# ltronchin/Gan-track

Hardware: AMD Instinct MI355X
Metric: imgs/sec at 256^2 bs32/GPU StyleGAN2-ADA training (+ sec/kimg) (higher is better)
Workload: dtype fp16+fp32 (fp16 at the 4 highest resolutions, fp32 below; f32 accumulate); 1 GPU; StyleGAN2-ADA train iteration, 256x256 1-ch, c_dim 2, cbase 16384, map 8, Gmain+Dmain / Greg every 4 / Dreg every 16, ADA geometric p=0.2; global_batch=32, batch_gpu=32, resolution=256, parallelism=dp1

## Files before the change

### gan-track_amd/csrc/upfirdn2d.hip

```cpp
#include <cstdlib>

#include "sg2_common.h"

namespace sg2 {
namespace {

constexpr int kMaxTaps = 1024;

struct UpfParams {
    const void* x;
    void* y;
    const float* f;
    int N, C, H, W;
    int OH, OW;
    int64_t xs_n, xs_c, xs_h, xs_w;
    int64_t ys_n, ys_c, ys_h, ys_w;
    int fw, fh;
    int upx, upy, downx, downy, padx0, pady0;
    int flip;
    float gain;
    const float* out_scale;
    const void* noise;
    const float* bias;
    const void* residual;
    void* aux;
    float noise_gain, alpha, egain, clamp;
    int act, aux_mode, epi;
    const int* lim;
    int xcd;
};

constexpr int kZeroBand = 32;

__device__ __forceinline__ int floordiv(int a, int b) { return (a >= 0) ? a / b : -((-a + b - 1) / b); }

__device__ __forceinline__ void axis_taps(int o, int down, int pad0, int up, int& t0, int& i0) {
    const int z = o * down - pad0;
    int r = (-z) % up;
    if (r < 0) r += up;
    t0 = r;
    i0 = floordiv(z + r, up);
}

__device__ __forceinline__ void stage_filter(float* sf, const UpfParams& p) {
    const int n = p.fw * p.fh;
    for (int i = threadIdx.x; i < n; i += blockDim.x) {
        const int ty = i / p.fw, tx = i % p.fw;
        const int sy = p.flip ? ty : p.fh - 1 - ty;
        const int sx = p.flip ? tx : p.fw - 1 - tx;
        sf[i] = p.f[sy * p.fw + sx] * p.gain;
    }
    __syncthreads();
}

template <typename T>
__global__ __launch_bounds__(256) void upfirdn_generic(UpfParams p) {
    __shared__ float sf[kMaxTaps];
    stage_filter(sf, p);
    const T* x = (const T*)p.x;
    T* y = (T*)p.y;
    const int64_t total = (int64_t)p.N * p.C * p.OH * p.OW;
    for (int64_t idx = (int64_t)blockIdx.x * blockDim.x + threadIdx.x; idx < total;
         idx += (int64_t)gridDim.x * blockDim.x) {
        int64_t r = idx;
        const int ox = (int)(r % p.OW); r /= p.OW;
        const int oy = (int)(r % p.OH); r /= p.OH;
        const int c = (int)(r % p.C); r /= p.C;
        const int n = (int)r;
        if (p.lim) {
            const int ly = p.lim[0], lx = p.lim[1];
            if (oy >= ly + kZeroBand || ox >= lx + kZeroBand) continue;
            if (oy >= ly || ox >= lx) {
                y[n * p.ys_n + c * p.ys_c + (int64_t)oy * p.ys_h + (int64_t)ox * p.ys_w] = (T)0.f;
                continue;
            }
        }
        int ty0, iy0, tx0, ix0;
        axis_taps(oy, p.downy, p.pady0, p.upy, ty0, iy0);
        axis_taps(ox, p.downx, p.padx0, p.upx, tx0, ix0);
        const T* xb = x + n * p.xs_n + c * p.xs_c;
        float acc = 0.f;
        for (int ty = ty0, iy = iy0; ty < p.fh; ty += p.upy, ++iy) {
            if (iy < 0 || iy >= p.H) continue;
            const T* xr = xb + iy * p.xs_h;
            for (int tx = tx0, ix = ix0; tx < p.fw; tx += p.upx, ++ix) {
                if (ix < 0 || ix >= p.W) continue;
                acc += (float)xr[ix * p.xs_w] * sf[ty * p.fw + tx];
            }
        }
        y[n * p.ys_n + c * p.ys_c + (int64_t)oy * p.ys_h + (int64_t)ox * p.ys_w] = (T)acc;
    }
}

template <int UP, int DOWN>
__device__ __forceinline__ void axis_taps_c(int o, int down, int pad0, int up, int& t0, int& i0) {
    if (UP == 1 && DOWN != 0) { t0 = 0; i0 = o * DOWN - pad0; }
    else if (UP == 2 && DOWN != 0) { const int z = o * DOWN - pad0; t0 = z & 1; i0 = (z + t0) >> 1; }
    else axis_taps(o, down, pad0, up, t0, i0);
}

template <typename T, bool HORIZ, int KT, int UP, int DOWN>
__global__ __launch_bounds__(256) void upfirdn_1d(UpfParams p) {
    __shared__ float sf[64];
    const int F = HORIZ ? p.fw : p.fh;
    for (int t = threadIdx.x; t < F; t += 256) sf[t] = p.f[p.flip ? t : F - 1 - t] * p.gain;
    __syncthreads();
    const int ly = p.lim ? p.lim[0] : p.OH, lx = p.lim ? p.lim[1] : p.OW;
    const int rows = min(p.OH, ly + (p.lim ? kZeroBand : 0)), cols = min(p.OW, lx + (p.lim ? kZeroBand : 0));
    const int tiles = (cols + 255) / 256;
    const int total = p.N * p.C * rows * tiles;
    const int up = HORIZ ? p.upx : p.upy, down = HORIZ ? p.downx : p.downy, L = HORIZ ? p.W : p.H;
    for (int b = blockIdx.x; b < total; b += gridDim.x) {
        const int row = b / tiles;
        const int ox = (b - row * tiles) * 256 + threadIdx.x;
        const int oy = row % rows, nc = row / rows;
        if (ox >= cols) continue;
        const int c = nc % p.C, n = nc / p.C;
        T* yp = (T*)p.y + n * p.ys_n + c * p.ys_c + (int64_t)oy * p.ys_h + (int64_t)ox * p.ys_w;
        if (oy >= ly || ox >= lx) { *yp = (T)0.f; continue; }
        const T* xb = (const T*)p.x + n * p.xs_n + c * p.xs_c;
        int t0, i0;
        if (HORIZ) axis_taps_c<UP, DOWN>(ox, down, p.padx0, up, t0, i0);
        else axis_taps_c<UP, DOWN>(oy, down, p.pady0, up, t0, i0);
        const T* xl = HORIZ ? xb + (int64_t)oy * p.xs_h : xb + (int64_t)ox * p.xs_w;
        const int64_t st = HORIZ ? p.xs_w : p.xs_h;
        const int upk = UP ? UP : up;
        float acc = 0.f;
#pragma unroll
        for (int k = 0; k < KT; ++k) {
            const int t = t0 + k * upk, i = i0 + k;
            const bool ok = t < F && i >= 0 && i < L;
            const float v = (float)xl[(int64_t)(ok ? i : 0) * st];
            acc += ok ? v * sf[t < F ? t : 0] : 0.f;
        }
        *yp = (T)acc;
    }
}

template <typename T, int UP, int DOWN, int KT, int TWD = 256>
__global__ __launch_bounds__(256) void upfirdn_1d_hlds(UpfParams p) {
    constexpr int ROWS = 256 / TWD;
    constexpr int SPAN = ((TWD - 1) * DOWN + UP - 1) / UP + KT + 1;
    __shared__ float sf[64];
    __shared__ float sx[ROWS][SPAN];
    const int F = p.fw;
    for (int t = threadIdx.x; t < KT * UP; t += 256) sf[t] = t < F ? p.f[p.flip ? t : F - 1 - t] * p.gain : 0.f;
    __syncthreads();
    float fr[KT * UP];
#pragma unroll
    for (int t = 0; t < KT * UP; ++t) fr[t] = t < F ? sf[t] : 0.f;
    const int ly = p.lim ? p.lim[0] : p.OH, lx = p.lim ? p.lim[1] : p.OW;
    const int rows = min(p.OH, ly + (p.lim ? kZeroBand : 0)), cols = min(p.OW, lx + (p.lim ? kZeroBand : 0));
    const int tiles = (cols + TWD - 1) / TWD, rgroups = (rows + ROWS - 1) / ROWS;
    const int total = p.N * p.C * rgroups * tiles;
    const int rr = threadIdx.x / TWD, col = threadIdx.x % TWD;
    for (int b = blockIdx.x; b < total; b += gridDim.x) {
        const int rg = b / tiles;
        const int ox0 = (b - rg * tiles) * TWD, ox = ox0 + col;
        const int oy0 = (rg % rgroups) * ROWS, nc = rg / rgroups;
        const int c = nc % p.C, n = nc / p.C;
        int tb, base;
        axis_taps_c<UP, DOWN>(ox0, DOWN, p.padx0, UP, tb, base);
        const T* xp = (const T*)p.x + n * p.xs_n + c * p.xs_c;
        __syncthreads();
        for (int e = threadIdx.x; e < ROWS * SPAN; e += 256) {
            const int r = e / SPAN, m = e - r * SPAN;
            const int i = base + m, y = oy0 + r;
            sx[r][m] = (i >= 0 && i < p.W && y < rows) ? (float)xp[(int64_t)y * p.xs_h + (int64_t)i * p.xs_w] : 0.f;
        }
        __syncthreads();
        const int oy = oy0 + rr;
        if (ox >= cols || oy >= rows) continue;
        T* yp = (T*)p.y + n * p.ys_n + c * p.ys_c + (int64_t)oy * p.ys_h + (int64_t)ox * p.ys_w;
        if (oy >= ly || ox >= lx) { *yp = (T)0.f; continue; }
        int t0, i0;
        axis_taps_c<UP, DOWN>(ox, DOWN, p.padx0, UP, t0, i0);
        const float* w = &sx[rr][i0 - base];
        float acc = 0.f;
#pragma unroll
        for (int k = 0; k < KT; ++k)
            acc += w[k] * (UP == 1 ? fr[k] : sf[t0 + k * UP]);
        *yp = (T)acc;
    }
}

template <int UP, int DOWN, int P>
struct VRunPat {
    static constexpr int dj(int j) { return UP == 1 ? j * DOWN : (P == 0 ? (j + 1) / 2 : j / 2); }
    static constexpr int tj(int j) { return UP == 1 ? 0 : (P == 0 ? (j & 1) : 1 - (j & 1)); }
};

template <int UP, int DOWN, int KT, int R, int SPAN, int P>
__device__ __forceinline__ void vrun_acc(const float (&win)[SPAN], const float (&fr)[KT * UP], float (&acc)[R]) {
#pragma unroll
    for (int j = 0; j < R; ++j) {
#pragma unroll
        for (int k = 0; k < KT; ++k) acc[j] += win[VRunPat<UP, DOWN, P>::dj(j) + k] * fr[VRunPat<UP, DOWN, P>::tj(j) + k * UP];
    }
}

template <typename T, int UP, int DOWN, int KT, int R>
__global__ __launch_bounds__(256) void upfirdn_1d_vrun(UpfParams p) {
    static_assert(UP == 1 || R % 2 == 0, "even runs keep the phase fixed");
    constexpr int SPAN = ((R - 1) * DOWN + UP - 1) / UP + KT;
    __shared__ float sf[64];
    const int F = p.fh;
    for (int t = threadIdx.x; t < F; t += 256) sf[t] = p.f[p.flip ? t : F - 1 - t] * p.gain;
    __syncthreads();
    float fr[KT * UP];
#pragma unroll
    for (int t = 0; t < KT * UP; ++t) fr[t] = t < F ? sf[t] : 0.f;
    const int ly = p.lim ? p.lim[0] : p.OH, lx = p.lim ? p.lim[1] : p.OW;
    const int rows = min(p.OH, ly + (p.lim ? kZeroBand : 0)), cols = min(p.OW, lx + (p.lim ? kZeroBand : 0));
    const int tiles = (cols + 255) / 256, runs = (rows + R - 1) / R;
    const int total = p.N * p.C * runs * tiles;
    for (int b = blockIdx.x; b < total; b += gridDim.x) {
        const int run = b / tiles;
        const int ox = (b - run * tiles) * 256 + threadIdx.x;
        const int oy0 = (run % runs) * R, nc = run / runs;
        if (ox >= cols) continue;
        const int c = nc % p.C, n = nc / p.C;
        const T* xb = (const T*)p.x + n * p.xs_n + c * p.xs_c + (int64_t)ox * p.xs_w;
        T* yb = (T*)p.y + n * p.ys_n + c * p.ys_c + (int64_t)ox * p.ys_w;
        const int z0 = oy0 * DOWN - p.pady0;
        const int ph = UP == 2 ? (z0 & 1) : 0;
        const int base = UP == 2 ? (z0 + ph) >> 1 : z0;
        float win[SPAN];
#pragma unroll
        for (int m = 0; m < SPAN; ++m) {
            const int i = base + m;
            const bool ok = i >= 0 && i < p.H;
            const float v = (float)xb[(int64_t)(ok ? i : 0) * p.xs_h];
            win[m] = ok ? v : 0.f;
        }
        float acc[R];
#pragma unroll
        for (int j = 0; j < R; ++j) acc[j] = 0.f;
        if (ph) vrun_acc<UP, DOWN, KT, R, SPAN, 1>(win, fr, acc);
        else vrun_acc<UP, DOWN, KT, R, SPAN, 0>(win, fr, acc);
#pragma unroll
        for (int j = 0; j < R; ++j) {
            const int oy = oy0 + j;
            if (oy >= rows) break;
            yb[(int64_t)oy * p.ys_h] = (oy >= ly || ox >= lx) ? (T)0.f : (T)acc[j];
        }
    }
}

template <typename T> struct VecN { static constexpr int N = 8; };
template <> struct VecN<float> { static constexpr int N = 4; };

template <typename T, int V, typename vecT>
__device__ __forceinline__ void store_out(const UpfParams& p, T* y, const float* acc, int n, int oy, int ox, int cv) {
    const int64_t dst = n * p.ys_n + (int64_t)oy * p.ys_h + (int64_t)ox * p.ys_w + cv * V;
    vecT o;
    if (p.epi) {
        const float nv = p.noise ? (float)((const T*)p.noise)[((int64_t)n * p.OH + oy) * p.OW + ox] * p.noise_gain : 0.f;
        vecT ax, rv;
        if (p.residual) rv = *(const vecT*)((const T*)p.residual + dst);
#pragma unroll
        for (int j = 0; j < V; ++j) {
            const int c = cv * V + j;
            float v = acc[j];
            if (p.out_scale) v *= p.out_scale[(int64_t)n * p.C + c];
            v += nv;
            if (p.bias) v += (float)(T)p.bias[c];
            if (p.act == 1) v = v > 0.f ? v : v * p.alpha;
            v *= p.egain;
            if (p.clamp >= 0.f) v = fminf(fmaxf(v, -p.clamp), p.clamp);
            ax[j] = (T)(p.aux_mode == 1 ? acc[j] : v);
            o[j] = (T)v;
            if (p.residual) o[j] = (T)((float)o[j] + (float)rv[j]);
        }
        if (p.aux_mode) *(vecT*)((T*)p.aux + dst) = ax;
    } else {
#pragma unroll
        for (int j = 0; j < V; ++j) o[j] = (T)acc[j];
    }
    *(vecT*)(y + dst) = o;
}


template <typename T, typename IDX>
__global__ __launch_bounds__(256) void upfirdn_nhwc_vec(UpfParams p) {
    constexpr int V = VecN<T>::N;
    typedef T vecT __attribute__((ext_vector_type(V)));
    __shared__ float sf[kMaxTaps];
    stage_filter(sf, p);
    const T* x = (const T*)p.x;
    T* y = (T*)p.y;
    const IDX CV = (IDX)(p.C / V), OW = (IDX)p.OW, OH = (IDX)p.OH;
    const IDX total = (IDX)((int64_t)p.N * p.OH * p.OW * (p.C / V));
    for (IDX idx = (IDX)blockIdx.x * blockDim.x + threadIdx.x; idx < total; idx += (IDX)gridDim.x * blockDim.x) {
        IDX r = idx;
        const int cv = (int)(r % CV); r /= CV;
        const int ox = (int)(r % OW); r /= OW;
        const int oy = (int)(r % OH); r /= OH;
        const int n = (int)r;
        int ty0, iy0, tx0, ix0;
        axis_taps(oy, p.downy, p.pady0, p.upy, ty0, iy0);
        axis_taps(ox, p.downx, p.padx0, p.upx, tx0, ix0);
        const T* xb = x + n * p.xs_n + cv * V;
        float acc[V];
#pragma unroll
        for (int j = 0; j < V; ++j) acc[j] = 0.f;
        for (int ty = ty0, iy = iy0; ty < p.fh; ty += p.upy, ++iy) {
            if (iy < 0 || iy >= p.H) continue;
            const T* xr = xb + iy * p.xs_h;
            for (int tx = tx0, ix = ix0; tx < p.fw; tx += p.upx, ++ix) {
                if (ix < 0 || ix >= p.W) continue;
                const float wt = sf[ty * p.fw + tx];
                const vecT v = *(const vecT*)(xr + ix * p.xs_w);
#pragma unroll
                for (int j = 0; j < V; ++j) acc[j] += (float)v[j] * wt;
            }
        }
        store_out<T, V, vecT>(p, y, acc, n, oy, ox, cv);
    }
}

__device__ __forceinline__ float fma_mix_lo(unsigned h2, float w, float acc) {
    float r;
    asm volatile("v_fma_mix_f32 %0, %1, %2, %3 op_sel_hi:[1,0,0]" : "=v"(r) : "v"(h2), "v"(w), "v"(acc));
    return r;
}
__device__ __forceinline__ float fma_mix_hi(unsigned h2, float w, float acc) {
    float r;
    asm volatile("v_fma_mix_f32 %0, %1, %2, %3 op_sel:[1,0,0] op_sel_hi:[1,0,0]" : "=v"(r) : "v"(h2), "v"(w), "v"(acc));
    return r;
}

template <typename T>
__global__ __launch_bounds__(256) void upfirdn_nhwc_up2(UpfParams p) {
    constexpr int V = VecN<T>::N;
    typedef T vecT __attribute__((ext_vector_type(V)));
    __shared__ float sf[16];
    if (threadIdx.x < 16) {
        const int ty = threadIdx.x >> 2, tx = threadIdx.x & 3;
        sf[threadIdx.x] = p.f[(p.flip ? ty : 3 - ty) * 4 + (p.flip ? tx : 3 - tx)] * p.gain;
    }
    __syncthreads();
    const unsigned CV = p.C / V, CW = (p.OW + 1) >> 1, CH = (p.OH + 1) >> 1;
    const unsigned total = (unsigned)p.N * CH * CW * CV;
    const unsigned idx = blockIdx.x * 256u + threadIdx.x;
    if (idx >= total) return;
    unsigned r = idx;
    const int cv = (int)(r % CV); r /= CV;
    const int cx = (int)(r % CW); r /= CW;
    const int cy = (int)(r % CH);
    const int n = (int)(r / CH);
    int ty[2], iy[2], tx[2], ix[2];
    axis_taps(2 * cy, 1, p.pady0, 2, ty[0], iy[0]);
    axis_taps(2 * cy + 1, 1, p.pady0, 2, ty[1], iy[1]);
    axis_taps(2 * cx, 1, p.padx0, 2, tx[0], ix[0]);
    axis_taps(2 * cx + 1, 1, p.padx0, 2, tx[1], ix[1]);
    const int y0 = min(iy[0], iy[1]), x0 = min(ix[0], ix[1]);
    const T* xb = (const T*)p.x + n * p.xs_n + cv * V;
    vecT xv[3][3];
#pragma unroll
    for (int a = 0; a < 3; ++a)
#pragma unroll
        for (int b = 0; b < 3; ++b) {
            const int yy = y0 + a, xx = x0 + b;
            const bool ok = yy >= 0 && yy < p.H && xx >= 0 && xx < p.W;
            xv[a][b] = ok ? *(const vecT*)(xb + yy * p.xs_h + xx * p.xs_w) : vecT{};
        }
#pragma unroll
    for (int py = 0; py < 2; ++py) {
        const int oy = 2 * cy + py;
        if (oy >= p.OH) continue;
        const int dy = iy[py] - y0;
#pragma unroll
        for (int px = 0; px < 2; ++px) {
            const int ox = 2 * cx + px;
            if (ox >= p.OW) continue;
            const int dx = ix[px] - x0;
            float acc[V];
#pragma unroll
            for (int j = 0; j < V; ++j) acc[j] = 0.f;
#pragma unroll
            for (int a = 0; a < 2; ++a) {
                const int t1 = ty[py] + 2 * a;
                if (t1 >= 4) continue;
#pragma unroll
                for (int b = 0; b < 2; ++b) {
                    const int t2 = tx[px] + 2 * b;
                    if (t2 >= 4) continue;
                    const float w = sf[t1 * 4 + t2];
                    const vecT v = dy ? (dx ? xv[1 + a][1 + b] : xv[1 + a][b]) : (dx ? xv[a][1 + b] : xv[a][b]);
                    if constexpr (std::is_same<T, f16_t>::value) {
                        typedef unsigned u32v __attribute__((ext_vector_type(V / 2)));
                        const u32v u = __builtin_bit_cast(u32v, v);
#pragma unroll
                        for (int q = 0; q < V / 2; ++q) {
                            acc[2 * q] = fma_mix_lo(u[q], w, acc[2 * q]);
                            acc[2 * q + 1] = fma_mix_hi(u[q], w, acc[2 * q + 1]);
                        }
                    } else {
#pragma unroll
                        for (int j = 0; j < V; ++j) acc[j] += (float)v[j] * w;
                    }
                }
            }
            store_out<T, V, vecT>(p, (T*)p.y, acc, n, oy, ox, cv);
        }
    }
}

template <typename T, int DOWN, int TW, int TH, int CG>
__global__ __launch_bounds__(256) void upfirdn_nhwc_f4(UpfParams p) {
    constexpr int V = VecN<T>::N;
    constexpr int F = 4;
    constexpr int IW = (TW - 1) * DOWN + F, IH = (TH - 1) * DOWN + F, NIN = IW * IH * CG;
    typedef T vecT __attribute__((ext_vector_type(V)));
    __shared__ float sf[F * F];
    extern __shared__ __attribute__((aligned(16))) char tile_raw[];
    vecT* tile = (vecT*)tile_raw;
    const int tid = threadIdx.x;
    if (tid < F * F) {
        const int ty = tid / F, tx = tid % F;
        sf[tid] = p.f[(p.flip ? ty : F - 1 - ty) * F + (p.flip ? tx : F - 1 - tx)] * p.gain;
    }
    const int CV = p.C / V;
    const int ngroups = (CV + CG - 1) / CG;
    const int tiles_x = (p.OW + TW - 1) / TW, tiles_y = (p.OH + TH - 1) / TH;
    int64_t b = blockIdx.x;
    const int64_t nb = gridDim.x;
    if ((nb & 7) == 0 && p.xcd) b = (b & 7) * (nb >> 3) + (b >> 3);
    const int cg = (int)(b % ngroups); b /= ngroups;
    const int tx0 = (int)(b % tiles_x) * TW; b /= tiles_x;
    const int ty0 = (int)(b % tiles_y) * TH; b /= tiles_y;
    const int n = (int)b;
    const int cv0 = cg * CG;
    const T* xb = (const T*)p.x + n * p.xs_n;
    const int iy0 = ty0 * DOWN - p.pady0, ix0 = tx0 * DOWN - p.padx0;
    for (int i = tid; i < NIN; i += 256) {
        const int c = i % CG, px = i / CG;
        const int ry = px / IW, rx = px - ry * IW;
        const int iy = iy0 + ry, ix = ix0 + rx;
        const bool ok = iy >= 0 && iy < p.H && ix >= 0 && ix < p.W && cv0 + c < CV;
        vecT v = *(const vecT*)(xb + (int64_t)(ok ? iy : 0) * p.xs_h + (int64_t)(ok ? ix : 0) * p.xs_w +
                                (ok ? cv0 + c : 0) * V);
#pragma unroll
        for (int j = 0; j < V; ++j) v[j] = ok ? v[j] : (T)0.f;
        tile[i] = v;
    }
    __syncthreads();
    const int c = tid % CG;
    if (cv0 + c >= CV) return;
#pragma unroll
    for (int pass = 0; pass < TW * TH * CG / 256; ++pass) {
        const int pix = tid / CG + pass * (256 / CG);
        const int oy = ty0 + pix / TW, ox = tx0 + pix % TW;
        if (oy >= p.OH || ox >= p.OW) continue;
        float acc[V];
#pragma unroll
        for (int j = 0; j < V; ++j) acc[j] = 0.f;
        const vecT* base = tile + ((pix / TW) * DOWN * IW + (pix % TW) * DOWN) * CG + c;
#pragma unroll
        for (int ky = 0; ky < F; ++ky)
#pragma unroll
            for (int kx = 0; kx < F; ++kx) {
                const float w = sf[ky * F + kx];
                const vecT v = base[(ky * IW + kx) * CG];
                if constexpr (std::is_same<T, f16_t>::value) {
                    typedef unsigned u32v __attribute__((ext_vector_type(V / 2)));
                    const u32v u = __builtin_bit_cast(u32v, v);
#pragma unroll
                    for (int q = 0; q < V / 2; ++q) {
                        acc[2 * q] = fma_mix_lo(u[q], w, acc[2 * q]);
                        acc[2 * q + 1] = fma_mix_hi(u[q], w, acc[2 * q + 1]);
                    }
                } else {
#pragma unroll
                    for (int j = 0; j < V; ++j) acc[j] += (float)v[j] * w;
                }
            }
        store_out<T, V, vecT>(p, (T*)p.y, acc, n, oy, ox, cv0 + c);
    }
}

template <typename T, int V, typename vecT, int TW, int TH, int CG, bool SEP, bool EPI>
__device__ __forceinline__ void fir4_strip(const UpfParams& p, const vecT* base, const float* wf, const float* fy,
                                           const float* fx, int n, int ty0, int ox, int cv) {
    constexpr int F = 4, IW = TW + F - 1, IH = TH + F - 1;
    float os[V], bj[V];
#pragma unroll
    for (int j = 0; j < V; ++j) {
        const int c = cv * V + j;
        os[j] = (p.epi && p.out_scale) ? p.out_scale[(int64_t)n * p.C + c] : 1.f;
        bj[j] = (p.epi && p.bias) ? (float)(T)p.bias[c] : 0.f;
    }
    const float slope = (p.epi && p.act == 1) ? p.alpha : 1.f;
    const float eg = p.epi ? p.egain : 1.f;
    const bool clamp_on = p.epi && p.clamp >= 0.f;
    const float cl = p.clamp;
    const bool noise = p.epi && p.noise, resid = p.epi && p.residual;
    const int aux_mode = p.epi ? p.aux_mode : 0;
    float acc[TH][V];
#pragma unroll
    for (int o = 0; o < TH; ++o)
#pragma unroll
        for (int j = 0; j < V; ++j) acc[o][j] = 0.f;
#pragma unroll
    for (int ry = 0; ry < IH; ++ry) {
        vecT v[F];
#pragma unroll
        for (int kx = 0; kx < F; ++kx) v[kx] = base[(ry * IW + kx) * CG];
        if constexpr (SEP) {
            float h[V];
            if constexpr (std::is_same<T, f16_t>::value) {
                typedef unsigned u32v __attribute__((ext_vector_type(V / 2)));
#pragma unroll
                for (int j = 0; j < V; ++j) h[j] = 0.f;
#pragma unroll
                for (int kx = 0; kx < F; ++kx) {
                    const u32v u = __builtin_bit_cast(u32v, v[kx]);
#pragma unroll
                    for (int q = 0; q < V / 2; ++q) {
                        h[2 * q] = fma_mix_lo(u[q], fx[kx], h[2 * q]);
                        h[2 * q + 1] = fma_mix_hi(u[q], fx[kx], h[2 * q + 1]);
                    }
                }
            } else {
#pragma unroll
                for (int j = 0; j < V; ++j) {
                    h[j] = 0.f;
#pragma unroll
                    for (int kx = 0; kx < F; ++kx) h[j] += (float)v[kx][j] * fx[kx];
                }
            }
#pragma unroll
            for (int ky = 0; ky < F; ++ky) {
                const int o = ry - ky;
                if (o < 0 || o >= TH) continue;
#pragma unroll
                for (int j = 0; j < V; ++j) acc[o][j] += h[j] * fy[ky];
            }
        } else {
#pragma unroll
            for (int ky = 0; ky < F; ++ky) {
                const int o = ry - ky;
                if (o < 0 || o >= TH) continue;
#pragma unroll
                for (int kx = 0; kx < F; ++kx)
#pragma unroll
                    for (int j = 0; j < V; ++j) acc[o][j] += (float)v[kx][j] * wf[ky * F + kx];
            }
        }
        const int od = ry - (F - 1);
        if (od < 0) continue;
        const int oy = ty0 + od;
        const int64_t dst = n * p.ys_n + (int64_t)oy * p.ys_h + (int64_t)ox * p.ys_w + cv * V;
        if constexpr (!EPI) {
            vecT o;
#pragma unroll
            for (int j = 0; j < V; ++j) o[j] = (T)acc[od][j];
            *(vecT*)((T*)p.y + dst) = o;
            __builtin_amdgcn_sched_barrier(0);
            continue;
        }
        const float nv = noise ? (float)((const T*)p.noise)[((int64_t)n * p.OH + oy) * p.OW + ox] * p.noise_gain : 0.f;
        vecT o, ax;
#pragma unroll
        for (int j = 0; j < V; ++j) {
            float z = acc[od][j] * os[j] + nv + bj[j];
            z = (z > 0.f ? z : z * slope) * eg;
            if (clamp_on) z = fminf(fmaxf(z, -cl), cl);
            o[j] = (T)z;
            ax[j] = (T)(aux_mode == 1 ? acc[od][j] : z);
        }
        if (resid) {
            const vecT rv = *(const vecT*)((const T*)p.residual + dst);
#pragma unroll
            for (int j = 0; j < V; ++j) o[j] = (T)((float)o[j] + (float)rv[j]);
        }
        if (aux_mode) *(vecT*)((T*)p.aux + dst) = ax;
        *(vecT*)((T*)p.y + dst) = o;
        __builtin_amdgcn_sched_barrier(0);
    }
}

template <typename T, int TW, int TH, int CG = 8>
__global__ __launch_bounds__(256, 2) void upfirdn_nhwc_f4s(UpfParams p) {
    constexpr int V = VecN<T>::N, F = 4;
    constexpr int IW = TW + F - 1, IH = TH + F - 1, NIN = IW * IH * CG;
    constexpr int NL = (NIN + 255) / 256;
    static_assert(TW * CG == 256, "one lane per (column, channel vector)");
    typedef T vecT __attribute__((ext_vector_type(V)));
    extern __shared__ __attribute__((aligned(16))) char tile_raw[];
    vecT* tile = (vecT*)tile_raw;
    const int tid = threadIdx.x;
    float wf[F * F];
#pragma unroll
    for (int t = 0; t < F * F; ++t) {
        const int ty = t / F, tx = t % F;
        wf[t] = p.f[(p.flip ? ty : F - 1 - ty) * F + (p.flip ? tx : F - 1 - tx)] * p.gain;
    }
    const int CV = p.C / V;
    const int ngroups = (CV + CG - 1) / CG;
    const int tiles_x = (p.OW + TW - 1) / TW, tiles_y = (p.OH + TH - 1) / TH;
    int64_t b = blockIdx.x;
    const int64_t nb = gridDim.x;
    if ((nb & 7) == 0) b = (b & 7) * (nb >> 3) + (b >> 3);
    const int tx0 = min((int)(b % tiles_x) * TW, p.OW - TW); b /= tiles_x;
    const int ty0 = min((int)(b % tiles_y) * TH, p.OH - TH); b /= tiles_y;
    const int cg = (int)(b % ngroups); b /= ngroups;
    const int n = (int)b;
    const int cv0 = cg * CG;
    const T* xb = (const T*)p.x + n * p.xs_n;
    const int iy0 = ty0 - p.pady0, ix0 = tx0 - p.padx0;
    vecT r[NL];
#pragma unroll
    for (int l = 0; l < NL; ++l) {
        const int i = tid + l * 256;
        const int c = i % CG, px = i / CG;
        const int ry = px / IW, rx = px - ry * IW;
        const int iy = iy0 + ry, ix = ix0 + rx;
        const bool ok = i < NIN && iy >= 0 && iy < p.H && ix >= 0 && ix < p.W && cv0 + c < CV;
        r[l] = *(const vecT*)(xb + (int64_t)(ok ? iy : 0) * p.xs_h + (int64_t)(ok ? ix : 0) * p.xs_w +
                              (ok ? cv0 + c : 0) * V);
#pragma unroll
        for (int j = 0; j < V; ++j) r[l][j] = ok ? r[l][j] : (T)0.f;
    }
#pragma unroll
    for (int l = 0; l < NL; ++l)
        if (l < NL - 1 || tid + l * 256 < NIN) tile[tid + l * 256] = r[l];
    __syncthreads();
    const int c = tid % CG, col = tid / CG;
    if (cv0 + c >= CV) return;
    float fy[F], fx[F];
    bool sep = wf[0] != 0.f;
#pragma unroll
    for (int k = 0; k < F; ++k) {
        fx[k] = wf[k];
        fy[k] = sep ? wf[k * F] / wf[0] : 0.f;
    }
#pragma unroll
    for (int t = 0; t < F * F; ++t) sep = sep && (fy[t / F] * fx[t % F] == wf[t]);
    const vecT* tb = tile + col * CG + c;
    if (sep) {
        if (p.epi) fir4_strip<T, V, vecT, TW, TH, CG, true, true>(p, tb, wf, fy, fx, n, ty0, tx0 + col, cv0 + c);
        else fir4_strip<T, V, vecT, TW, TH, CG, true, false>(p, tb, wf, fy, fx, n, ty0, tx0 + col, cv0 + c);
    } else {
        if (p.epi) fir4_strip<T, V, vecT, TW, TH, CG, false, true>(p, tb, wf, fy, fx, n, ty0, tx0 + col, cv0 + c);
        else fir4_strip<T, V, vecT, TW, TH, CG, false, false>(p, tb, wf, fy, fx, n, ty0, tx0 + col, cv0 + c);
    }
}

template <typename T>
int launch(const UpfParams& p, bool vec, hipStream_t s) {
    static const bool fir_old = getenv("SG2_FIR_OLD") != nullptr;
    if (!fir_old && vec && p.upx == 1 && p.upy == 1 && p.downx == 1 && p.downy == 1 && p.fw == 4 && p.fh == 4 &&
        p.OH >= 8 && (p.OW % 32 == 0 || p.OW >= 224) && !(p.residual && p.residual == p.y)) {
        constexpr int TW = 32, TH = 8;
        const char* e32 = getenv("SG2_FIR_C32");
        const bool c32_off = e32 && e32[0] == '0';
        if (!c32_off && p.C / VecN<T>::N == 4 && (p.OW % 64 == 0 || p.OW >= 224)) {
            constexpr int TW4 = 64, CG4 = 4;
            const int64_t blocks4 = (int64_t)p.N * cdiv(p.OH, TH) * cdiv(p.OW, TW4);
            if (blocks4 < INT32_MAX) {
                const size_t lds = (size_t)(TH + 3) * (TW4 + 3) * CG4 * 16;
                auto k = upfirdn_nhwc_f4s<T, TW4, TH, CG4>;
                static bool set4 = false;
                if (!set4) { (void)hipFuncSetAttribute((const void*)k, hipFuncAttributeMaxDynamicSharedMemorySize, (int)lds); set4 = true; }
                k<<<(unsigned)blocks4, 256, lds, s>>>(p);
                return launch_status("sg2_upfirdn2d");
            }
        }
        const int64_t blocks = (int64_t)p.N * cdiv(p.OH, TH) * cdiv(p.OW, TW) * cdiv(p.C / VecN<T>::N, 8);
        if (blocks < INT32_MAX) {
            const size_t lds = (size_t)(TH + 3) * (TW + 3) * 8 * 16;
            auto k = upfirdn_nhwc_f4s<T, TW, TH>;
            static bool set = false;
            if (!set) { (void)hipFuncSetAttribute((const void*)k, hipFuncAttributeMaxDynamicSharedMemorySize, (int)lds); set = true; }
            k<<<(unsigned)blocks, 256, lds, s>>>(p);
            return launch_status("sg2_upfirdn2d");
        }
    }
    if (vec && p.upx == 1 && p.upy == 1 && p.downx == p.downy && (p.downy == 1 || p.downy == 2) && p.fw == 4 &&
        p.fh == 4) {
        constexpr int CG = 4;
        const int d = p.downy;
        const int TW = d == 1 ? 32 : 16, TH = 8;
        const int64_t blocks = (int64_t)p.N * cdiv(p.OH, TH) * cdiv(p.OW, TW) * cdiv(p.C / VecN<T>::N, CG);
        if (blocks < INT32_MAX) {
            const size_t lds = (size_t)((TH - 1) * d + 4) * ((TW - 1) * d + 4) * CG * 16;
            if (d == 1) {
                auto k = upfirdn_nhwc_f4<T, 1, 32, 8, CG>;
                static bool set1 = false;
                if (!set1) { (void)hipFuncSetAttribute((const void*)k, hipFuncAttributeMaxDynamicSharedMemorySize, (int)lds); set1 = true; }
                k<<<(unsigned)blocks, 256, lds, s>>>(p);
            } else {
                auto k = upfirdn_nhwc_f4<T, 2, 16, 8, CG>;
                static bool set2 = false;
                if (!set2) { (void)hipFuncSetAttribute((const void*)k, hipFuncAttributeMaxDynamicSharedMemorySize, (int)lds); set2 = true; }
                k<<<(unsigned)blocks, 256, lds, s>>>(p);
            }
            return launch_status("sg2_upfirdn2d");
        }
    }
    if (vec && p.upx == 2 && p.upy == 2 && p.downx == 1 && p.downy == 1 && p.fw == 4 && p.fh == 4 &&
        !getenv("SG2_UPF_UP2_OFF")) {
        const int64_t cells = (int64_t)p.N * ((p.OH + 1) / 2) * ((p.OW + 1) / 2) * (p.C / VecN<T>::N);
        if (cells < INT32_MAX - 256) {
            upfirdn_nhwc_up2<T><<<(unsigned)cdiv(cells, 256), 256, 0, s>>>(p);
            return launch_status("sg2_upfirdn2d");
        }
    }
    if (!vec && !p.epi) {
        const bool horiz = p.fh == 1 && p.upy == 1 && p.downy == 1 && p.pady0 == 0 && p.OH == p.H && p.fw <= 64;
        const bool vert = p.fw == 1 && p.upx == 1 && p.downx == 1 && p.padx0 == 0 && p.OW == p.W && p.fh <= 64;
        const int up = horiz ? p.upx : p.upy, down = horiz ? p.downx : p.downy, F = horiz ? p.fw : p.fh;
        const int kt = (F + up - 1) / up;
        const int64_t pairs = (int64_t)p.N * p.C * p.OH * cdiv(p.OW, 256);
        if ((horiz || vert) && kt <= 16 && pairs < INT32_MAX) {
            static const int gmax = [] { const char* e = getenv("SG2_U1D_GRID"); return e ? atoi(e) : 4096; }();
            const unsigned g = (unsigned)std::min<int64_t>(pairs, gmax);
            const bool ada_up = up == 2 && down == 1 && kt == 6, ada_down = up == 1 && down == 2 && kt == 12;
            static const int vr = [] { const char* e = getenv("SG2_U1D_VRUN"); return e ? atoi(e) : 4; }();
            static const bool hl = [] { const char* e = getenv("SG2_U1D_HLDS"); return e ? atoi(e) != 0 : true; }();
            static const int htw = [] { const char* e = getenv("SG2_U1D_HTW"); return e ? atoi(e) : 128; }();
            if (vert && vr == 4 && ada_up) upfirdn_1d_vrun<T, 2, 1, 6, 4><<<g, 256, 0, s>>>(p);
            else if (vert && vr == 4 && ada_down) upfirdn_1d_vrun<T, 1, 2, 12, 4><<<g, 256, 0, s>>>(p);
            else if (vert && vr == 8 && ada_up) upfirdn_1d_vrun<T, 2, 1, 6, 8><<<g, 256, 0, s>>>(p);
            else if (vert && vr == 8 && ada_down) upfirdn_1d_vrun<T, 1, 2, 12, 8><<<g, 256, 0, s>>>(p);
            else if (horiz && hl && ada_up && htw == 128) upfirdn_1d_hlds<T, 2, 1, 6, 128><<<g, 256, 0, s>>>(p);
            else if (horiz && hl && ada_down && htw == 128) upfirdn_1d_hlds<T, 1, 2, 12, 128><<<g, 256, 0, s>>>(p);
            else if (horiz && hl && ada_up) upfirdn_1d_hlds<T, 2, 1, 6><<<g, 256, 0, s>>>(p);
            else if (horiz && hl && ada_down) upfirdn_1d_hlds<T, 1, 2, 12><<<g, 256, 0, s>>>(p);
            else if (horiz && ada_up) upfirdn_1d<T, true, 6, 2, 1><<<g, 256, 0, s>>>(p);
            else if (horiz && ada_down) upfirdn_1d<T, true, 12, 1, 2><<<g, 256, 0, s>>>(p);
            else if (ada_up) upfirdn_1d<T, false, 6, 2, 1><<<g, 256, 0, s>>>(p);
            else if (ada_down) upfirdn_1d<T, false, 12, 1, 2><<<g, 256, 0, s>>>(p);
            else {
#define U1D(KT_) { if (horiz) upfirdn_1d<T, true, KT_, 0, 0><<<g, 256, 0, s>>>(p); \
                   else upfirdn_1d<T, false, KT_, 0, 0><<<g, 256, 0, s>>>(p); }
                if (kt <= 4) U1D(4) else if (kt <= 8) U1D(8) else U1D(16)
#undef U1D
            }
            return launch_status("sg2_upfirdn2d");
        }
    }
    const int64_t work = vec ? (int64_t)p.N * p.OH * p.OW * (p.C / VecN<T>::N) : (int64_t)p.N * p.C * p.OH * p.OW;
    const int grid = (int)std::max<int64_t>(1, std::min<int64_t>(cdiv(work, 256), 256 * 32));
    if (vec && work < INT32_MAX && (int64_t)grid * 256 < INT32_MAX)
        upfirdn_nhwc_vec<T, unsigned><<<grid, 256, 0, s>>>(p);
    else if (vec)
        upfirdn_nhwc_vec<T, int64_t><<<grid, 256, 0, s>>>(p);
    else
        upfirdn_generic<T><<<grid, 256, 0, s>>>(p);
    return launch_status("sg2_upfirdn2d");
}

}
}

extern "C" int sg2_upfirdn2d_fused(void* y, const void* x, const float* f, int dtype, const int64_t* in_size,
                                   const int64_t* in_stride, const int64_t* out_size, const int64_t* out_stride,
                                   int fw, int fh, int upx, int upy, int downx, int downy, int padx0, int padx1,
                                   int pady0, int pady1, int flip, float gain, const sg2_epilogue* epi,
                                   void* stream) {
    using namespace sg2;
    SG2_CHECK(x && y && f && in_size && in_stride && out_size && out_stride, "sg2_upfirdn2d: null argument");
    SG2_CHECK(upx >= 1 && upy >= 1 && downx >= 1 && downy >= 1, "sg2_upfirdn2d: up/down must be >= 1");
    SG2_CHECK(fw >= 1 && fh >= 1 && fw * fh <= kMaxTaps, "sg2_upfirdn2d: filter too large");
    UpfParams p;
    p.x = x; p.y = y; p.f = f;
    p.N = (int)in_size[0]; p.C = (int)in_size[1]; p.H = (int)in_size[2]; p.W = (int)in_size[3];
    p.OH = (int)out_size[2]; p.OW = (int)out_size[3];
    SG2_CHECK(out_size[0] == p.N && out_size[1] == p.C, "sg2_upfirdn2d: batch/channel mismatch");
    const int64_t eh = ((int64_t)p.H * upy + pady0 + pady1 - fh + downy) / downy;
    const int64_t ew = ((int64_t)p.W * upx + padx0 + padx1 - fw + downx) / downx;
    SG2_CHECK(p.H * upy + pady0 + pady1 >= fh && p.W * upx + padx0 + padx1 >= fw,
              "sg2_upfirdn2d: upsampled buffer must be at least the size of the filter");
    SG2_CHECK(eh == p.OH && ew == p.OW, "sg2_upfirdn2d: output size mismatch");
    p.xs_n = in_stride[0]; p.xs_c = in_stride[1]; p.xs_h = in_stride[2]; p.xs_w = in_stride[3];
    p.ys_n = out_stride[0]; p.ys_c = out_stride[1]; p.ys_h = out_stride[2]; p.ys_w = out_stride[3];
    p.fw = fw; p.fh = fh; p.upx = upx; p.upy = upy; p.downx = downx; p.downy = downy;
    p.padx0 = padx0; p.pady0 = pady0; p.flip = flip; p.gain = gain; p.lim = nullptr;
    { const char* e = getenv("SG2_FIR_XCD"); p.xcd = e ? atoi(e) : 1; }
    p.out_scale = nullptr; p.noise = nullptr; p.bias = nullptr; p.residual = nullptr; p.aux = nullptr;
    p.noise_gain = 0.f; p.alpha = 0.f; p.egain = 1.f; p.clamp = -1.f; p.act = 0; p.aux_mode = 0; p.epi = 0;
    if (epi) {
        SG2_CHECK(epi->act == 0 || epi->act == 1, "sg2_upfirdn2d: epilogue act must be 0 or 1");
        SG2_CHECK(epi->aux_mode >= 0 && epi->aux_mode <= 2 && (epi->aux_mode == 0 || epi->aux),
                  "sg2_upfirdn2d: bad epilogue aux output");
        p.out_scale = epi->out_scale; p.noise = epi->noise; p.bias = epi->bias; p.residual = epi->residual;
        p.aux = epi->aux; p.noise_gain = epi->noise_gain; p.alpha = epi->alpha; p.egain = epi->gain;
        p.clamp = epi->clamp; p.act = epi->act; p.aux_mode = epi->aux_mode; p.epi = 1;
    }
    if ((int64_t)p.N * p.C * p.OH * p.OW == 0) return 0;
    hipStream_t s = as_stream(stream);
    SG2_DISPATCH(dtype, T, {
        constexpr int V = VecN<T>::N;
        const bool vec = p.xs_c == 1 && p.ys_c == 1 && p.C % V == 0 && p.C >= V &&
                         ((uintptr_t)x % 16 == 0) && ((uintptr_t)y % 16 == 0) &&
                         p.xs_w % V == 0 && p.xs_h % V == 0 && p.xs_n % V == 0 &&
                         p.ys_w % V == 0 && p.ys_h % V == 0 && p.ys_n % V == 0;
        SG2_CHECK(vec || !p.epi, "sg2_upfirdn2d: the fused epilogue needs NHWC activations with C % 8 == 0");
        return launch<T>(p, vec, s);
    });
    return 0;
}

extern "C" int sg2_upfirdn2d_lim(void* y, const void* x, const float* f, int dtype, const int64_t* in_size,
                                 const int64_t* in_stride, const int64_t* out_size, const int64_t* out_stride, int fw,
                                 int fh, int upx, int upy, int downx, int downy, int padx0, int padx1, int pady0,
                                 int pady1, int flip, float gain, const int* lim, void* stream) {
    using namespace sg2;
    SG2_CHECK(x && y && f && in_size && in_stride && out_size && out_stride, "sg2_upfirdn2d: null argument");
    SG2_CHECK(upx >= 1 && upy >= 1 && downx >= 1 && downy >= 1, "sg2_upfirdn2d: up/down must be >= 1");
    SG2_CHECK(fw >= 1 && fh >= 1 && fw * fh <= kMaxTaps, "sg2_upfirdn2d: filter too large");
    UpfParams p{};
    p.x = x; p.y = y; p.f = f; p.lim = lim;
    p.N = (int)in_size[0]; p.C = (int)in_size[1]; p.H = (int)in_size[2]; p.W = (int)in_size[3];
    p.OH = (int)out_size[2]; p.OW = (int)out_size[3];
    SG2_CHECK(out_size[0] == p.N && out_size[1] == p.C, "sg2_upfirdn2d: batch/channel mismatch");
    const int64_t eh = ((int64_t)p.H * upy + pady0 + pady1 - fh + downy) / downy;
    const int64_t ew = ((int64_t)p.W * upx + padx0 + padx1 - fw + downx) / downx;
    SG2_CHECK(eh == p.OH && ew == p.OW, "sg2_upfirdn2d: output size mismatch");
    p.xs_n = in_stride[0]; p.xs_c = in_stride[1]; p.xs_h = in_stride[2]; p.xs_w = in_stride[3];
    p.ys_n = out_stride[0]; p.ys_c = out_stride[1]; p.ys_h = out_stride[2]; p.ys_w = out_stride[3];
    p.fw = fw; p.fh = fh; p.upx = upx; p.upy = upy; p.downx = downx; p.downy = downy;
    p.padx0 = padx0; p.pady0 = pady0; p.flip = flip; p.gain = gain; p.egain = 1.f; p.clamp = -1.f;
    if ((int64_t)p.N * p.C * p.OH * p.OW == 0) return 0;
    hipStream_t s = as_stream(stream);
    SG2_DISPATCH(dtype, T, { return launch<T>(p, false, s); });
    return 0;
}

extern "C" int sg2_upfirdn2d(void* y, const void* x, const float* f, int dtype, const int64_t* in_size,
                             const int64_t* in_stride, const int64_t* out_size, const int64_t* out_stride, int fw,
                             int fh, int upx, int upy, int downx, int downy, int padx0, int padx1, int pady0,
                             int pady1, int flip, float gain, void* stream) {
    return sg2_upfirdn2d_fused(y, x, f, dtype, in_size, in_stride, out_size, out_stride, fw, fh, upx, upy, downx,
                               downy, padx0, padx1, pady0, pady1, flip, gain, nullptr, stream);
}
```

### gan-track_amd/sg2hip/__init__.py

```python
import contextlib
import ctypes
import os

import torch

_HERE = os.path.dirname(os.path.abspath(__file__))
LIB_PATH = os.environ.get('SG2HIP_LIB', os.path.join(_HERE, 'libsg2hip.so'))

F32, F16, BF16, F32S3 = 0, 1, 2, 3
_DTYPES = {torch.float32: F32, torch.float16: F16, torch.bfloat16: BF16}

_c_i64p = ctypes.POINTER(ctypes.c_int64)


class Epilogue(ctypes.Structure):
    _fields_ = [('out_scale', ctypes.c_void_p), ('noise', ctypes.c_void_p), ('bias', ctypes.c_void_p),
                ('residual', ctypes.c_void_p), ('aux', ctypes.c_void_p), ('noise_gain', ctypes.c_float),
                ('alpha', ctypes.c_float), ('gain', ctypes.c_float), ('clamp', ctypes.c_float),
                ('act', ctypes.c_int), ('aux_mode', ctypes.c_int), ('dot_src', ctypes.c_void_p),
                ('dot_out', ctypes.c_void_p)]

class AugGeomArgs(ctypes.Structure):
    _fields_ = [('draw', ctypes.c_void_p * 16), ('p', ctypes.c_void_p)] + \
        [(k, ctypes.c_float) for k in ('xflip', 'rotate90', 'xint', 'xint_max', 'scale', 'rotate', 'aniso', 'xfrac',
                                       'scale_std', 'rotate_max', 'aniso_std', 'xfrac_std', 'pad_x', 'pad_y',
                                       'inv_sx', 'inv_sy')] + \
        [(k, ctypes.c_int) for k in ('n', 'h', 'w')]


_vp = ctypes.c_void_p
_i = ctypes.c_int
_i64 = ctypes.c_int64
_f = ctypes.c_float

SIGNATURES = {
    'sg2_abi_version': [],
    'sg2_bias_act': [_vp, _vp, _vp, _vp, _vp, _vp, _i, _i64, _i64, _i64, _i, _i, _f, _f, _f, _vp],
    'sg2_upfirdn2d': [_vp, _vp, _vp, _i, _c_i64p, _c_i64p, _c_i64p, _c_i64p, _i, _i, _i, _i, _i, _i, _i, _i, _i, _i,
                      _i, _f, _vp],
    'sg2_conv2d': [_vp, _vp, _vp, _i, _i, _i, _i, _i, _i, _i, _i, _i, _i, _i, _i, _i, _i, _vp, _i64, _vp],
    'sg2_conv2d_fused': [_vp, _vp, _vp, _i, _i, _i, _i, _i, _i, _i, _i, _i, _i, _i, _i, _i, _i, _vp,
                         ctypes.POINTER(Epilogue), _vp, _i64, _vp],
    'sg2_conv3x3': [_vp, _vp, _vp, _vp, _i, _i, _i, _i, _i, _i, _vp, _vp, _vp, _f, _vp, _i, _f, _f, _f, _vp, _vp,
                    _vp],
    'sg2_set_zeroed_accumulators': [_i],
    'sg2_set_clean_workspace': [_i],
    'sg2_set_deterministic': [_vp, _i64],
    'sg2_split3': [_vp, _vp, _i64, _i, _i64, _vp, _vp],
    'sg2_conv3x3_s2': [_vp, _vp, _vp, _vp, _i, _i, _i, _i, _i, _i, _vp, _vp, _vp, _f, _vp, _i, _f, _f, _f, _vp, _i,
                       _vp, _vp, _vp],
    'sg2_conv3x3_up2': [_vp, _vp, _vp, _i, _i, _i, _i, _i, _i, _vp, _vp],
    'sg2_conv2d_wgrad': [_vp, _vp, _vp, _i, _i, _i, _i, _i, _i, _i, _i, _i, _i, _i, _i, _i, _vp, _vp, _f, _vp],
    'sg2_conv2d_wgrad_oikk': [_vp, _vp, _vp, _i, _i, _i, _i, _i, _i, _i, _i, _i, _i, _i, _i, _i, _f, _i, _vp],
    'sg2_upfirdn2d_lim': [_vp, _vp, _vp, _i, _c_i64p, _c_i64p, _c_i64p, _c_i64p, _i, _i, _i, _i, _i, _i, _i, _i, _i, _i,
                          _i, _f, _vp, _vp],
    'sg2_upfirdn2d_fused': [_vp, _vp, _vp, _i, _c_i64p, _c_i64p, _c_i64p, _c_i64p, _i, _i, _i, _i, _i, _i, _i, _i, _i,
                            _i, _i, _f, ctypes.POINTER(Epilogue), _vp],
    'sg2_layer_bwd': [_vp, _vp, _vp, _vp, _vp, _vp, _vp, _vp, _i, _i, _i, _i, _i, _f, _f, _f, _vp],
    'sg2_dot_hw': [_vp, _vp, _vp, _i, _i, _i, _i, _vp],
    'sg2_vjp_axpy': [_vp, _vp, _vp, _vp, _vp, _vp, _i, _f, _f, _f, _vp, _vp, _i, _i, _i, _i, _vp],
    'sg2_grid_sample_fwd': [_vp, _vp, _vp, _i, _c_i64p, _c_i64p, _c_i64p, _c_i64p, _vp, _vp],
    'sg2_grid_sample_bwd': [_vp, _vp, _vp, _i, _c_i64p, _c_i64p, _c_i64p, _c_i64p, _vp, _vp],
    'sg2_affine_grid_sample_fwd': [_vp, _vp, _vp, _i, _c_i64p, _c_i64p, _c_i64p, _c_i64p, _vp, _vp],
    'sg2_affine_grid_sample_bwd': [_vp, _vp, _vp, _i, _c_i64p, _c_i64p, _c_i64p, _c_i64p, _vp, _vp],
    'sg2_reflect_pad_dyn': [_vp, _vp, _vp, _i, _i, _i, _i, _i, _i, _i, _vp],
    'sg2_aug_geom': [_vp, _vp, _vp, _vp, ctypes.POINTER(AugGeomArgs), _vp],
    'sg2_moments': [_vp, _vp, _i64, _i, _vp],
    'sg2_demod_fwd': [_vp, _vp, _vp, _vp, _i, _i, _i, _i, _f, _vp],
    'sg2_demod_bwd': [_vp, _vp, _vp, _vp, _vp, _vp, _vp, _i, _i, _i, _i, _vp],
    'sg2_demod_vjp_bwd': [_vp] * 10 + [_i, _i, _i, _i, _vp],
    'sg2_adam_multi': [_vp, _vp, _vp, _i, _vp, _vp, _vp, _f, _f, _f, _f, _i, _vp],
    'sg2_lerp_multi': [_vp, _vp, _i, _f, _vp],
    'sg2_infnorm_fwd': [_vp, _vp, _vp, _i, _i, _f, _i, _vp],
    'sg2_infnorm_bwd': [_vp, _vp, _vp, _vp, _i, _i, _f, _i, _vp],
    'sg2_infnorm_vjp_bwd': [_vp, _vp, _vp, _vp, _vp, _vp, _i, _i, _f, _vp],
    'sg2_pack_weight': [_vp, _i, _vp, _i, _i, _i, _i, _i64, _i64, _i64, _i, _f, _vp],
    'sg2_pack_weight_multi': [_vp, _i, _vp],
    'sg2_knn_scratch_bytes': [_c_i64p, _i64, _i64, _i],
    'sg2_knn_radii': [_vp, _vp, _i, _i64, _i, _i, _i, _vp, _i64, _vp],
    'sg2_manifold_member': [_vp, _vp, _i64, _vp, _i64, _vp, _i, _i, _i, _vp, _i64, _vp],
    'sg2_noise_reg_scratch_bytes': [_c_i64p, _c_i64p, _i],
    'sg2_noise_reg_fwd': [_vp, _vp, _vp, _c_i64p, _i, _vp, _vp],
    'sg2_noise_reg_bwd': [_vp, _vp, _vp, _vp, _c_i64p, _i, _vp, _i, _vp],
    'sg2_noise_normalize_multi': [_vp, _c_i64p, _i, _vp],
}
ABI_VERSION = 11

_lib = None


def lib():
    global _lib
    if _lib is None:
        if not os.path.exists(LIB_PATH):
            raise RuntimeError(f'sg2hip: {LIB_PATH} not found -- build it with `python -c "import __graft_entry__ as '
                               f'g; g.build()"` (hipcc --offload-arch=gfx950); there is no CPU fallback')
        L = ctypes.CDLL(LIB_PATH)
        for name, args in SIGNATURES.items():
            fn = getattr(L, name)
            fn.argtypes = args
            fn.restype = ctypes.c_int
        L.sg2_last_error.argtypes = []
        L.sg2_last_error.restype = ctypes.c_char_p
        L.sg2_set_zeroed_accumulators.restype = None
        L.sg2_set_clean_workspace.restype = None
        L.sg2_set_deterministic.restype = None
        if L.sg2_abi_version() != ABI_VERSION:
            raise RuntimeError(f'sg2hip: ABI version mismatch ({L.sg2_abi_version()} != {ABI_VERSION})')
        _lib = L
    return _lib


@contextlib.contextmanager
def clean_workspace(on=True):
    if not on:
        yield
        return
    L = lib()
    L.sg2_set_clean_workspace(1)
    try:
        yield
    finally:
        L.sg2_set_clean_workspace(0)


_det_scratch = {}
_det_retired = []
_det_state = (0, 0)


def det_active():
    return _det_state[0] != 0


def _det_register(ptr, nbytes):
    global _det_state
    lib().sg2_set_deterministic(ctypes.c_void_p(ptr), ctypes.c_int64(nbytes))
    _det_state = (ptr, nbytes)


@contextlib.contextmanager
def deterministic(on=True, scratch_mb=2048, device=None):
    prev = _det_state
    if on:
        dev = torch.device('cuda', torch.cuda.current_device()) if device is None else torch.device(device)
        buf = _det_scratch.get(dev)
        if buf is None or buf.numel() * 4 < scratch_mb << 20:
            if buf is not None:
                _det_retired.append(buf)
            buf = _det_scratch[dev] = torch.empty([scratch_mb << 18], dtype=torch.float32, device=dev)
        _det_register(buf.data_ptr(), buf.numel() * 4)
    else:
        _det_register(0, 0)
    try:
        yield
    finally:
        _det_register(*prev)


@contextlib.contextmanager
def zeroed_accumulators(on=True):
    if not on:
        yield
        return
    L = lib()
    L.sg2_set_zeroed_accumulators(1)
    try:
        yield
    finally:
        L.sg2_set_zeroed_accumulators(0)


def check(rc, what):
    if rc != 0:
        msg = lib().sg2_last_error().decode(errors='replace')
        raise RuntimeError(f'{what} failed ({rc}): {msg}')


def dtype_code(t):
    try:
        return _DTYPES[t.dtype]
    except KeyError:
        raise RuntimeError(f'sg2hip: unsupported dtype {t.dtype}') from None


def require_device(*tensors):
    for t in tensors:
        if t is not None and (not isinstance(t, torch.Tensor) or t.device.type != 'cuda'):
            raise RuntimeError('sg2hip ops run only on ROCm device tensors (no CPU fallback); got '
                               f'{type(t).__name__} on {getattr(t, "device", None)}')


def stream_ptr(device=None):
    return ctypes.c_void_p(torch.cuda.current_stream(device).cuda_stream)


def ptr(t):
    return ctypes.c_void_p(t.data_ptr()) if t is not None else ctypes.c_void_p(0)


def i64arr(vals):
    return (ctypes.c_int64 * len(vals))(*[int(v) for v in vals])
```

### gan-track_amd/torch_utils/ops/modconv.py

```python
import os

import torch

from . import bias_act as _ba
from . import conv2d_gradfix as _cg
from . import staged_sum as _ss
from . import upfirdn2d as _up

_CL = torch.channels_last
enabled = True
prezero = os.environ.get('SG2_PREZERO', '1') != '0'
det_assign = os.environ.get('SG2_DET_ASSIGN', '1') != '0'
fast_backward = True
fused_vjp = os.environ.get('SG2_FUSED_VJP', '1') != '0'
tap_enabled = os.environ.get('SG2_TORGB_TAP', '1') != '0'
_ACT = {0: 'linear', 1: 'lrelu'}


def supported(x, weight, up):
    n, cin, h, w = x.shape
    cout, _, kh, kw = weight.shape
    return (enabled and up == 1 and kh == 3 and kw == 3 and x.dtype in (torch.float16, torch.bfloat16) and x.is_cuda and
            cin % 8 == 0 and cout % 8 == 0 and h >= 16 and w >= 16)


def supported_generic(x, weight):
    return enabled and x.is_cuda


def _halo(x, kh, kw, stride, pad):
    n, cin, h, w = x.shape
    return (kh == 3 and kw == 3 and stride == 1 and pad == 1 and x.dtype in (torch.float16, torch.bfloat16) and
            cin % 8 == 0 and h >= 16 and w >= 16)


def _f32(t):
    return t.float().contiguous() if t is not None else None


def _sum_hw(t):
    return _ss.staged_sum(t, (2, 3), dtype=torch.float32)


def _sum_nhw(t):
    return _ss.staged_sum(t, (0, 2, 3), dtype=torch.float32)


def _mul(a, s):
    return a * s if s is not None else a


class FusedConv(torch.autograd.Function):
    @staticmethod
    def forward(ctx, x, styles, weight, dcoefs, noise, bias, residual, stride, pad, act, alpha, gain, clamp, wgain):
        x_in = x
        x = _cg._nhwc(x)
        n, cin, h, w = x.shape
        cout, _, kh, kw = weight.shape
        oh = (h + 2 * pad - kh) // stride + 1
        ow = (w + 2 * pad - kw) // stride + 1
        dt = x.dtype
        nz = noise.to(dt).reshape(n, oh, ow).contiguous() if noise is not None else None
        any_grad = any(ctx.needs_input_grad[:7])
        want_c = any_grad and dcoefs is not None
        want_z = any_grad and residual is not None
        assert not (want_c and want_z), 'demodulation and a residual in one layer are not supported'
        b32 = _f32(bias) if bias is not None else None
        if _halo(x, kh, kw, stride, pad) and residual is None:
            y, aux = _cg.conv3x3_fused(x, _cg._pack_conv(weight, dt, scale=wgain), cout, in_scale=_f32(styles), out_scale=_f32(dcoefs),
                                       noise=nz, noise_gain=1.0, bias=b32, act=act, alpha=alpha, gain=gain,
                                       clamp=clamp, want_raw=want_c)
        elif _cg._halo_s2_ok(x, kh, kw, stride, pad, cout=cout, scaled=styles is not None or noise is not None):
            y, aux = _cg.conv3x3_fused(x, _cg._pack_conv(weight, dt, scale=wgain), cout, in_scale=_f32(styles),
                                       out_scale=_f32(dcoefs), noise=nz, noise_gain=1.0, bias=b32, act=act,
                                       alpha=alpha, gain=gain, clamp=clamp, want_raw=want_c or want_z, stride=2,
                                       residual=residual, raw_act=want_z)
        else:
            y, aux = _cg.conv_fused(x, _cg._pack_conv(weight, dt, scale=wgain), cout, oh, ow, kh, kw, stride, (pad, pad),
                                    in_scale=_f32(styles), out_scale=_f32(dcoefs), noise=nz, noise_gain=1.0,
                                    bias=b32, act=act, alpha=alpha, gain=gain, clamp=clamp, residual=residual,
                                    aux_mode=1 if want_c else (2 if want_z else 0))
        ctx.save_for_backward(x_in, styles, weight, dcoefs, noise, bias, y, aux)
        ctx.cfg = (stride, pad, act, alpha, gain, clamp, residual is not None, wgain)
        return y

    @staticmethod
    def backward(ctx, dy):
        need = ctx.needs_input_grad
        g = _fused_conv_grads(ctx, need, dy)
        return g + (dy if need[6] else None, None, None, None, None, None, None, None)


def _fused_conv_grads(ctx, need, dy, dx_residual=None):
    x, styles, weight, dcoefs, noise, bias, y, aux = ctx.saved_tensors
    stride, pad, act, alpha, gain, clamp, has_res, wgain = ctx.cfg
    zsrc = aux if has_res else y
    c = aux if (dcoefs is not None and not has_res) else None
    if not torch.is_grad_enabled() and fast_backward:
        return _fast_backward(need, dy, _cg._nhwc(x), styles, weight, dcoefs, noise, bias, zsrc, c, stride, pad, act,
                              alpha, gain, clamp, wgain, dx_residual=dx_residual)
    if fused_vjp and _cg.weight_gradients_disabled and not has_res and (dcoefs is None or c is not None):
        dx, ds, dd = _LayerVJP.apply(dy, x, styles, weight, dcoefs, zsrc, c, need[0], need[1], need[3],
                                     stride, pad, act, alpha, gain, clamp, wgain)
        g = (dx, ds, None, dd, None, None)
    else:
        g = _composed_backward(need, dy, x, styles, weight, dcoefs, noise, bias, zsrc, c, stride, pad, act, alpha,
                               gain, clamp, wgain)
    if dx_residual is not None and g[0] is not None:
        g = (g[0].to(dx_residual.dtype) + dx_residual,) + tuple(g[1:])
    return g


class FusedConvTap(torch.autograd.Function):

    @staticmethod
    def forward(ctx, x, styles, weight, bias, pad, clamp):
        y = FusedConv.forward(ctx, x, styles, weight, None, None, bias, None, 1, pad, 0, 0.2, 1.0, clamp, 1.0)
        return x.view_as(x), y

    @staticmethod
    def backward(ctx, g_pass, dy):
        n = ctx.needs_input_grad
        need = (n[0], n[1], n[2], False, False, n[3], False)
        if dy is None:
            return g_pass, None, None, None, None, None
        res = None
        if g_pass is not None and n[0]:
            res = _cg._nhwc(g_pass.to(ctx.saved_tensors[0].dtype))
        dx, ds, dw, _, _, db = _fused_conv_grads(ctx, need, dy, dx_residual=res)
        if dx is None and res is not None:
            dx = res
        return dx, ds, dw, db, None, None


def fused_conv_tap(x, weight, styles, bias, padding, clamp):
    return FusedConvTap.apply(x, styles, weight, bias, int(padding), float(clamp if clamp is not None else -1.0))


def _scaled_input_grads(dc, x, styles, weight, need_x, need_s, need_w, stride, pad, wgain=1.0, acc_ds=None,
                        acc_dw=None, dx_residual=None):
    n, cin, h, w = x.shape
    cout, _, kh, kw = weight.shape
    dt = x.dtype
    dx = ds = dw = None
    s32 = _f32(styles)
    want_ds = need_s and styles is not None
    dso = acc_ds.view(n, cin) if (want_ds and acc_ds is not None) else None
    if need_x or want_ds:
        if dx_residual is not None and not need_x:
            dx_residual = None
        if _halo(dc, kh, kw, stride, pad) and dx_residual is None:
            wT = _cg._pack_convT(weight, dt, flip=True, scale=wgain)
            if want_ds:
                dx, _, ds = _cg.conv3x3_fused(dc, wT, cin, out_scale=s32, dot_src=x, dot_out=dso)
            else:
                dx, _ = _cg.conv3x3_fused(dc, wT, cin, out_scale=s32)
        else:
            if want_ds:
                dx, _, ds = _cg.conv_fused(dc, _cg._pack_convT(weight, dt, scale=wgain), cin, h, w, kh, kw, stride,
                                           (pad, pad), transpose=True, out_scale=s32, dot_src=x, dot_out=dso,
                                           residual=dx_residual)
            else:
                dx, _ = _cg.conv_fused(dc, _cg._pack_convT(weight, dt, scale=wgain), cin, h, w, kh, kw, stride,
                                       (pad, pad), transpose=True, out_scale=s32, residual=dx_residual)
        ds = ds.to(styles.dtype) if want_ds else None
        dx = dx if need_x else None
    if need_w and not _cg.weight_gradients_disabled:
        dw = _cg._wgrad_raw(dc, x, kh, kw, stride, (pad, pad), x_scale=s32, alpha=wgain, out=acc_dw,
                            param_layout=True).to(weight.dtype)
    return dx, ds, dw


class _ScaledConvT(torch.autograd.Function):

    @staticmethod
    def forward(ctx, dz, d, weight, stride, pad, out_hw):
        dzk = _cg._nhwc(dz)
        cin, kh, kw = weight.shape[1], weight.shape[2], weight.shape[3]
        dt = dz.dtype
        if _halo(dzk, kh, kw, stride, pad):
            y, _ = _cg.conv3x3_fused(dzk, _cg._pack_convT(weight, dt, flip=True), cin, in_scale=_f32(d))
        else:
            y, _ = _cg.conv_fused(dzk, _cg._pack_convT(weight, dt), cin, out_hw[0], out_hw[1], kh, kw, stride,
                                  (pad, pad), transpose=True, in_scale=_f32(d))
        ctx.save_for_backward(dz, d, weight)
        ctx.cfg = (stride, pad, tuple(out_hw))
        return y

    @staticmethod
    def backward(ctx, g):
        dz, d, weight = ctx.saved_tensors
        stride, pad, out_hw = ctx.cfg
        need = ctx.needs_input_grad
        dt = dz.dtype
        n, cout, oh, ow = dz.shape
        kh, kw = weight.shape[2], weight.shape[3]
        if torch.is_grad_enabled():
            ins = [t for t, nd in zip((dz, d, weight), need[:3]) if nd]
            y = _cg._ConvT2d.apply(dz * d.to(dt).reshape(n, -1, 1, 1), weight.to(dt), stride, (pad, pad), out_hw)
            gs = iter(torch.autograd.grad(y, ins, g, create_graph=True, allow_unused=True))
            return tuple(next(gs) if nd else None for nd in need[:3]) + (None, None, None)
        g = _cg._nhwc(g.to(dt))
        dz = _cg._nhwc(dz)
        d32 = _f32(d)
        gdz = gd = gw = None
        if need[0] or need[1]:
            src = dz if need[1] else None
            if _halo(g, kh, kw, stride, pad):
                res = _cg.conv3x3_fused(g, _cg._pack_conv(weight, dt), cout, out_scale=d32, dot_src=src)
            else:
                res = _cg.conv_fused(g, _cg._pack_conv(weight, dt), cout, oh, ow, kh, kw, stride, (pad, pad),
                                     out_scale=d32, dot_src=src)
            gdz = res[0] if need[0] else None
            gd = res[2].to(d.dtype) if need[1] else None
        if need[2] and not _cg.weight_gradients_disabled:
            gw = _cg._wgrad_raw(dz, g, kh, kw, stride, (pad, pad), g_scale=d32).to(weight.dtype)
        return gdz, gd, gw, None, None, None


class _SavedRaw(torch.autograd.Function):

    @staticmethod
    def forward(ctx, x, styles, weight, c, stride, pad):
        ctx.save_for_backward(x, styles, weight)
        ctx.cfg = (stride, pad)
        return c.view_as(c)

    @staticmethod
    def backward(ctx, dc):
        x, styles, weight = ctx.saved_tensors
        stride, pad = ctx.cfg
        need = ctx.needs_input_grad
        if torch.is_grad_enabled():
            dt = x.dtype
            n = x.shape[0]
            oh, ow = dc.shape[2], dc.shape[3]
            ins = [t for t, nd in zip((x, styles, weight), need[:3]) if nd]
            cc = _cg._Conv2d.apply(_mul(x, styles.to(dt).reshape(n, -1, 1, 1)), weight.to(dt), stride, (pad, pad),
                                   (oh, ow))
            gs = iter(torch.autograd.grad(cc, ins, dc, create_graph=True, allow_unused=True))
            return tuple(next(gs) if nd else None for nd in need[:3]) + (None, None, None)
        dx, ds, dw = _scaled_input_grads(_cg._nhwc(dc.to(x.dtype)), _cg._nhwc(x), styles,
                                         weight, need[0], need[1], need[2], stride, pad)
        return dx, ds, dw, None, None, None


def _conv_any(x, weight, cout, oh, ow, stride, pad, transpose, wgain, **epi):
    kh, kw = weight.shape[2], weight.shape[3]
    dt = x.dtype
    want_raw = epi.pop('want_raw', False)
    dot_src = epi.get('dot_src')
    if _halo(x, kh, kw, stride, pad):
        wp = _cg._pack_convT(weight, dt, flip=True, scale=wgain) if transpose else _cg._pack_conv(weight, dt, scale=wgain)
        res = _cg.conv3x3_fused(x, wp, cout, want_raw=want_raw, **epi)
    else:
        wp = _cg._pack_convT(weight, dt, scale=wgain) if transpose else _cg._pack_conv(weight, dt, scale=wgain)
        res = _cg.conv_fused(x, wp, cout, oh, ow, kh, kw, stride, (pad, pad), transpose=transpose,
                             aux_mode=1 if want_raw else 0, **epi)
    return res[0], res[1], (res[2] if dot_src is not None else None)


class _LayerVJP(torch.autograd.Function):

    @staticmethod
    def forward(ctx, dy, x, styles, weight, dcoefs, zsrc, c, need_x, need_s, need_d, stride, pad, act, alpha, gain,
                clamp, wgain):
        xk = _cg._nhwc(x)
        n, cin, h, w = xk.shape
        cout = weight.shape[0]
        dt = xk.dtype
        d32, s32 = _f32(dcoefs), _f32(styles)
        want_dd = need_d and d32 is not None
        want_ds = need_s and s32 is not None
        if zsrc.shape[1] % 8 == 0:
            dc, _, dd, _ = _cg.layer_bwd(dy.to(dt), zsrc, c if want_dd else None, d32, act=act, alpha=alpha, gain=gain,
                                         clamp=clamp, want_db=False, want_dd=want_dd, want_dnoise=False)
        else:
            dz = _ba.bias_act_grad(dy.to(dt), zsrc, act=_ACT[act], alpha=alpha, gain=gain, clamp=clamp)
            dd = _sum_hw(dz * c) if want_dd else None
            dc = _cg._nhwc(dz * dcoefs.to(dt).reshape(n, -1, 1, 1) if d32 is not None else dz)
        dx, dxs, ds = _conv_any(dc, weight, cin, h, w, stride, pad, True, wgain, out_scale=s32,
                                dot_src=xk if want_ds else None, want_raw=s32 is not None)
        if dxs is None:
            dxs = dx
        ctx.save_for_backward(xk, styles, weight, dcoefs, zsrc, c, dc, dxs)
        ctx.cfg = (stride, pad, act, alpha, gain, clamp, wgain)
        return (dx if need_x else None, ds.to(styles.dtype) if want_ds else None,
                dd.to(dcoefs.dtype) if want_dd else None)

    @staticmethod
    def backward(ctx, g_dx, g_ds, g_dd):
        if torch.is_grad_enabled():
            raise RuntimeError('_LayerVJP: third-order gradients are not supported (set modconv.fused_vjp = False)')
        x, styles, weight, dcoefs, zsrc, c, dc, dxs = ctx.saved_tensors
        stride, pad, act, alpha, gain, clamp, wgain = ctx.cfg
        need = ctx.needs_input_grad
        n, cin, h, w = x.shape
        cout, _, kh, kw = weight.shape
        oh, ow = dc.shape[2], dc.shape[3]
        dt = x.dtype
        d32, s32 = _f32(dcoefs), _f32(styles)
        g_dy = g_x = g_s = g_w = g_d = None
        g_ds = g_ds if s32 is not None else None
        gds32 = _f32(g_ds)
        G = None
        if g_dx is not None and s32 is None:
            G = _cg._nhwc(g_dx.to(dt))
        elif g_dx is not None:
            G, g_s = _cg.vjp_axpy(g_dx.to(dt), s32, x if g_ds is not None else None, gds32,
                                  e=dxs if need[2] else None)
        elif g_ds is not None:
            G, _ = _cg.vjp_axpy(x, gds32)
        hscale = (g_dd.float() / d32).contiguous() if (g_dd is not None and d32 is not None) else None
        if G is not None and (need[0] or need[4]):
            A_d, _, dot = _conv_any(G, weight, cout, oh, ow, stride, pad, False, wgain, out_scale=d32,
                                    dot_src=dc if (need[4] and d32 is not None) else None)
            if need[4] and d32 is not None:
                g_d = (dot / d32).to(dcoefs.dtype)
            if need[0]:
                g_dy, _ = _cg.vjp_axpy(A_d, None, c if hscale is not None else None, _f32(g_dd) if hscale is not None
                                       else None, y=zsrc, act=act, alpha=alpha, gain=gain, clamp=clamp)
        elif need[0] and hscale is not None:
            g_dy, _ = _cg.vjp_axpy(c, _f32(g_dd), y=zsrc, act=act, alpha=alpha, gain=gain, clamp=clamp)
        if need[1] or need[2]:
            gxc = gsc = None
            if hscale is not None:
                gxc, _, gsc = _conv_any(dc, weight, cin, h, w, stride, pad, True, wgain, in_scale=hscale,
                                        out_scale=s32, dot_src=x if (need[2] and s32 is not None) else None)
            if need[1]:
                if g_ds is not None:
                    g_x, _ = (_cg.vjp_axpy(gxc, None, dxs, gds32) if gxc is not None else _cg.vjp_axpy(dxs, gds32))
                else:
                    g_x = gxc
            if gsc is not None:
                g_s = gsc if g_s is None else g_s + gsc
        if need[3] and (G is not None or hscale is not None):
            acc = torch.zeros([cout * kh * kw * cin], dtype=torch.float32, device=x.device)
            if G is not None:
                g_w = _cg._wgrad_raw(dc, G, kh, kw, stride, (pad, pad), alpha=wgain, out=acc, param_layout=True)
            if hscale is not None:
                g_w = _cg._wgrad_raw(dc, x, kh, kw, stride, (pad, pad), x_scale=s32, g_scale=hscale, alpha=wgain,
                                     out=acc, param_layout=True)
            g_w = g_w.to(weight.dtype)
        g_s = g_s.to(styles.dtype) if g_s is not None else None
        return (g_dy, g_x, g_s, g_w, g_d) + (None,) * 12


def _fast_backward(need, dy, x, styles, weight, dcoefs, noise, bias, zsrc, c, stride, pad, act, alpha, gain, clamp,
                   wgain=1.0, dx_residual=None):
    n, cin, h, w = x.shape
    cout, _, kh, kw = weight.shape
    dt = x.dtype
    d32 = _f32(dcoefs)
    want_dd = need[3] and d32 is not None
    want_db, want_dn = need[5] and bias is not None, need[4] and noise is not None
    wide = zsrc.shape[1] % 8 == 0
    want_ds = need[1] and styles is not None and (need[0] or need[1])
    want_dw = need[2] and not _cg.weight_gradients_disabled
    sizes = [cout if (wide and want_db) else 0, n * cout if (wide and want_dd) else 0, n * cin if want_ds else 0,
             cout * kh * kw * cin if want_dw else 0]
    if not prezero or (det_assign and _cg._hip.det_active()):
        sizes = [0, 0, 0, 0]
    acc = torch.zeros([sum(sizes)], dtype=torch.float32, device=dy.device) if sum(sizes) else None
    parts, o = [], 0
    for k in sizes:
        parts.append(acc[o:o + k] if k else None)
        o += k
    if wide:
        lb = acc[:sizes[0] + sizes[1]] if sizes[0] + sizes[1] else None
        dc, db, dd, dn = _cg.layer_bwd(dy.to(dt), zsrc, c if want_dd else None, d32, act=act, alpha=alpha, gain=gain,
                                       clamp=clamp, want_db=want_db, want_dd=want_dd, want_dnoise=want_dn, acc=lb)
    else:
        dz = _ba.bias_act_grad(dy, zsrc, act=_ACT[act], alpha=alpha, gain=gain, clamp=clamp)
        db = _sum_nhw(dz) if want_db else None
        dd = _sum_hw(dz * c) if want_dd else None
        dn = dz.sum(1, keepdim=True, dtype=torch.float32) if want_dn else None
        dc = _cg._nhwc(dz * dcoefs.to(dt).reshape(n, -1, 1, 1) if dcoefs is not None else dz)
    dx, ds, dw = _scaled_input_grads(dc, x, styles, weight, need[0], need[1], need[2], stride, pad, wgain,
                                     acc_ds=parts[2], acc_dw=parts[3], dx_residual=dx_residual)
    db = db.to(bias.dtype) if db is not None else None
    dd = dd.to(dcoefs.dtype) if dd is not None else None
    dn = dn.to(noise.dtype) if dn is not None else None
    return dx, ds, dw, dd, dn, db


def _composed_backward(need, dy, x, styles, weight, dcoefs, noise, bias, zsrc, c, stride, pad, act, alpha, gain,
                       clamp, wgain=1.0):
    if wgain != 1.0:
        weight = weight * wgain
    n, cin, h, w = x.shape
    cout, _, kh, kw = weight.shape
    oh, ow = zsrc.shape[2], zsrc.shape[3]
    dt = x.dtype
    dz = _ba.bias_act_grad(dy, zsrc, act=_ACT[act], alpha=alpha, gain=gain, clamp=clamp)
    dx = ds = dw = dd = dnoise = db = None
    param_grads = not _cg.weight_gradients_disabled
    if need[5] and bias is not None and param_grads:
        db = _sum_nhw(dz).to(bias.dtype)
    if need[4] and noise is not None and param_grads:
        dnoise = dz.sum(1, keepdim=True, dtype=torch.float32).to(noise.dtype)
    s_ = styles.to(dt).reshape(n, -1, 1, 1) if styles is not None else None
    if need[3] and dcoefs is not None:
        if torch.is_grad_enabled() and c is not None and styles is not None:
            c_ = _SavedRaw.apply(x, styles, weight, c, stride, pad)
        elif torch.is_grad_enabled():
            c_ = _cg._Conv2d.apply(_mul(x, s_), weight.to(dt), stride, (pad, pad), (oh, ow))
        else:
            c_ = c
        dd = _cg.dot_hw(dz, c_).to(dcoefs.dtype)
    want_dw = need[2] and not _cg.weight_gradients_disabled
    scaled_t = dcoefs is not None and not want_dw
    dc = dz * dcoefs.to(dt).reshape(n, -1, 1, 1) if dcoefs is not None and not scaled_t else dz
    if need[0] or need[1]:
        if scaled_t:
            dxs = _ScaledConvT.apply(dz, dcoefs, weight, stride, pad, (h, w))
        else:
            dxs = _cg._ConvT2d.apply(dc, weight.to(dt), stride, (pad, pad), (h, w))
        if need[0]:
            dx = _mul(dxs, s_)
        if need[1] and styles is not None:
            ds = _cg.dot_hw(dxs, x).to(styles.dtype)
    if need[2] and not _cg.weight_gradients_disabled:
        dw = _cg._WGrad.apply(dc, _mul(x, s_), (kh, kw), stride, (pad, pad))
        dw = (dw * wgain if wgain != 1.0 else dw).to(weight.dtype)
    return dx, ds, dw, dd, dnoise, db


def fused_conv(x, weight, styles=None, dcoefs=None, noise=None, bias=None, residual=None, stride=1, padding=0,
               act='linear', alpha=0.2, gain=1.0, clamp=None, wgain=1.0):
    return FusedConv.apply(x, styles, weight, dcoefs, noise, bias, residual, int(stride), int(padding),
                           1 if act == 'lrelu' else 0, float(alpha), float(gain),
                           float(clamp if clamp is not None else -1.0), float(wgain))


def modconv_layer(x, styles, weight, dcoefs, noise, bias, alpha, gain, clamp):
    return fused_conv(x, weight, styles=styles, dcoefs=dcoefs, noise=noise, bias=bias, padding=1, act='lrelu',
                      alpha=alpha, gain=gain, clamp=clamp)


def _up_geometry(h, w, kh, kw, f):
    from . import conv2d_resample as _cr
    x0, x1, y0, y1 = _cr._frame_padding(kw // 2, f, 2, 1)
    x0, x1 = x0 - (kw - 1), x1 - (kw - 2)
    y0, y1 = y0 - (kh - 1), y1 - (kh - 2)
    cx = max(-max(x0, x1), 0)
    cy = max(-max(y0, y1), 0)
    th, tw = (h - 1) * 2 - 2 * cy + kh, (w - 1) * 2 - 2 * cx + kw
    return (cy, cx), (th, tw), [x0 + cx, x1 + cx, y0 + cy, y1 + cy]


def supported_up(x, weight, f):
    n, cin, h, w = x.shape
    cout = weight.shape[0]
    vec = 8 if x.dtype != torch.float32 else 4
    return enabled and x.is_cuda and f is not None and f.ndim == 2 and cout % vec == 0 and cout % 8 == 0


class UpModConv(torch.autograd.Function):

    @staticmethod
    def forward(ctx, x, styles, weight, dcoefs, noise, bias, f, alpha, gain, clamp):
        x = _cg._nhwc(x)
        n, cin, h, w = x.shape
        cout, _, kh, kw = weight.shape
        dt = x.dtype
        tpad, (th, tw), fpad = _up_geometry(h, w, kh, kw, f)
        t, _ = _cg.conv_fused(x, _cg._pack_conv(weight, dt), cout, th, tw, kh, kw, 2, tpad, transpose=True,
                              in_scale=_f32(styles))
        oh, ow = th + fpad[2] + fpad[3] - f.shape[0] + 1, tw + fpad[0] + fpad[1] - f.shape[1] + 1
        nz = noise.to(dt).reshape(n, oh, ow).contiguous() if noise is not None else None
        want_c = any(ctx.needs_input_grad[:6]) and dcoefs is not None
        b32 = _f32(bias) if bias is not None else None
        y, c = _up.fir_fused(t, f, fpad, gain=4.0, out_scale=_f32(dcoefs), noise=nz, bias=b32, act=1, alpha=alpha,
                             act_gain=gain, clamp=clamp, aux_mode=1 if want_c else 0)
        ctx.save_for_backward(x, styles, weight, dcoefs, noise, bias, f, y, c)
        ctx.cfg = (alpha, gain, clamp, tpad, (th, tw), fpad)
        return y

    @staticmethod
    def backward(ctx, dy):
        x, styles, weight, dcoefs, noise, bias, f, y, c = ctx.saved_tensors
        alpha, gain, clamp, tpad, (th, tw), fpad = ctx.cfg
        need = ctx.needs_input_grad
        n, cin, h, w = x.shape
        cout, _, kh, kw = weight.shape
        dt = x.dtype
        oh, ow = y.shape[2], y.shape[3]
        aup, adown, apad, aflip = _up.adjoint_params(f, (th, tw), (oh, ow), 1, 1, fpad, False)
        dx = ds = dw = dd = dn = db = None
        if torch.is_grad_enabled() and fused_vjp and _cg.weight_gradients_disabled and c is not None:
            dx, ds, dd = _UpLayerVJP.apply(dy, x, styles, weight, dcoefs, y, c, f, need[0], need[1], need[3],
                                           alpha, gain, clamp, tpad, (th, tw), fpad)
            return (dx, ds, None, dd, None, None, None, None, None, None)
        if not torch.is_grad_enabled() and fast_backward:
            d32, s32 = _f32(dcoefs), _f32(styles)
            want_dd = need[3] and d32 is not None
            dc, db, dd, dn = _cg.layer_bwd(dy.to(dt), y, c if want_dd else None, d32, act=1, alpha=alpha, gain=gain,
                                           clamp=clamp, want_db=need[5] and bias is not None, want_dd=want_dd,
                                           want_dnoise=need[4] and noise is not None)
            dt_ = _up.upfirdn2d(dc, f, up=aup, down=adown, padding=apad, flip_filter=aflip, gain=4)
            if (need[0] or need[1]) and _cg._halo_s2_ok(dt_, kh, kw, 2, tpad, dot=need[1]):
                res = _cg.conv3x3_fused(dt_, _cg._pack_conv(weight.transpose(0, 1), dt), cin, out_scale=s32,
                                        dot_src=x if need[1] else None, stride=2)
                dx = res[0] if need[0] else None
                ds = res[2] if need[1] else None
            elif need[0] or need[1]:
                if need[1]:
                    dx, _, ds = _cg.conv_fused(dt_, _cg._pack_conv(weight.transpose(0, 1), dt), cin, h, w, kh, kw, 2, tpad, out_scale=s32,
                                               dot_src=x)
                else:
                    dx, _ = _cg.conv_fused(dt_, _cg._pack_conv(weight.transpose(0, 1), dt), cin, h, w, kh, kw, 2, tpad, out_scale=s32)
                dx = dx if need[0] else None
            if need[2] and not _cg.weight_gradients_disabled:
                dw = _cg._wgrad_raw(x, dt_, kh, kw, 2, tpad, g_scale=s32, param_layout='swap').transpose(0, 1) \
                    .to(weight.dtype)
        else:
            wt = weight.to(dt).transpose(0, 1)
            dz = _ba.bias_act_grad(dy, y, act='lrelu', alpha=alpha, gain=gain, clamp=clamp)
            param_grads = not _cg.weight_gradients_disabled
            if need[5] and bias is not None and param_grads:
                db = _sum_nhw(dz)
            if need[4] and noise is not None and param_grads:
                dn = dz.sum(1, keepdim=True, dtype=torch.float32)
            s_ = styles.to(dt).reshape(n, -1, 1, 1)
            xs = x * s_
            if need[3] and dcoefs is not None:
                t_ = _cg._ConvT2d.apply(xs, wt, 2, tpad, (th, tw))
                c_ = _up.upfirdn2d(t_, f, padding=fpad, gain=4)
                dd = _cg.dot_hw(dz, c_)
            dc = dz * dcoefs.to(dt).reshape(n, -1, 1, 1)
            dt_ = _up.upfirdn2d(dc, f, up=aup, down=adown, padding=apad, flip_filter=aflip, gain=4)
            if need[0] or need[1]:
                dxs = _cg._Conv2d.apply(dt_, wt, 2, tpad, (h, w))
                if need[0]:
                    dx = dxs * s_
                if need[1]:
                    ds = _cg.dot_hw(dxs, x)
            if need[2] and not _cg.weight_gradients_disabled:
                dw = _cg._WGrad.apply(xs, dt_, (kh, kw), 2, tpad).transpose(0, 1)
        cast = lambda g, ref: g.to(ref.dtype) if (g is not None and ref is not None) else g
        return (dx, cast(ds, styles), cast(dw, weight), cast(dd, dcoefs), cast(dn, noise), cast(db, bias),
                None, None, None, None)


class _UpLayerVJP(torch.autograd.Function):

    @staticmethod
    def forward(ctx, dy, x, styles, weight, dcoefs, y, c, f, need_x, need_s, need_d, alpha, gain, clamp, tpad,
                t_hw, fpad):
        n, cin, h, w = x.shape
        kh, kw = weight.shape[2], weight.shape[3]
        dt = x.dtype
        d32, s32 = _f32(dcoefs), _f32(styles)
        oh, ow = y.shape[2], y.shape[3]
        aup, adown, apad, aflip = _up.adjoint_params(f, t_hw, (oh, ow), 1, 1, fpad, False)
        dc, _, dd, _ = _cg.layer_bwd(dy.to(dt), y, c if need_d else None, d32, act=1, alpha=alpha, gain=gain,
                                     clamp=clamp, want_db=False, want_dd=need_d, want_dnoise=False)
        u = _up.upfirdn2d(dc, f, up=aup, down=adown, padding=apad, flip_filter=aflip, gain=4)
        wT = _cg._pack_conv(weight.transpose(0, 1), dt)
        if _cg._halo_s2_ok(u, kh, kw, 2, tpad, dot=need_s):
            dx, dxs, ds = _cg.conv3x3_fused(u, wT, cin, out_scale=s32, dot_src=x if need_s else None, stride=2,
                                            want_raw=True) + ((None,) if not need_s else ())
        else:
            res = _cg.conv_fused(u, wT, cin, h, w, kh, kw, 2, tpad, out_scale=s32, dot_src=x if need_s else None,
                                 aux_mode=1)
            dx, dxs, ds = res if need_s else res + (None,)
        ctx.save_for_backward(x, styles, weight, dcoefs, y, c, f, dc, u, dxs)
        ctx.cfg = (alpha, gain, clamp, tpad, t_hw, fpad)
        return (dx if need_x else None, ds.to(styles.dtype) if need_s else None,
                dd.to(dcoefs.dtype) if need_d else None)

    @staticmethod
    def backward(ctx, g_dx, g_ds, g_dd):
        if torch.is_grad_enabled():
            raise RuntimeError('_UpLayerVJP: third-order gradients are not supported (set modconv.fused_vjp = False)')
        x, styles, weight, dcoefs, y, c, f, dc, u, dxs = ctx.saved_tensors
        alpha, gain, clamp, tpad, (th, tw), fpad = ctx.cfg
        need = ctx.needs_input_grad
        n, cin, h, w = x.shape
        cout, _, kh, kw = weight.shape
        dt = x.dtype
        d32, s32 = _f32(dcoefs), _f32(styles)
        g_dy = g_x = g_s = g_w = g_d = None
        gds32 = _f32(g_ds)
        G = None
        if g_dx is not None:
            G, g_s = _cg.vjp_axpy(g_dx.to(dt), s32, x if g_ds is not None else None, gds32,
                                  e=dxs if need[2] else None)
        elif g_ds is not None:
            G, _ = _cg.vjp_axpy(x, gds32)
        hscale = (g_dd.float() / d32).contiguous() if g_dd is not None else None
        if G is not None and (need[0] or need[4]):
            tG, _ = _cg.conv_fused(G, _cg._pack_conv(weight, dt), cout, th, tw, kh, kw, 2, tpad, transpose=True)
            A_d, _ = _up.fir_fused(tG, f, fpad, gain=4.0, out_scale=d32)
            if need[4]:
                g_d = (_cg.dot_hw(A_d, dc) / (d32 * d32)).to(dcoefs.dtype)
            if need[0]:
                g_dy, _ = _cg.vjp_axpy(A_d, None, c if hscale is not None else None, _f32(g_dd) if hscale is not None
                                       else None, y=y, act=1, alpha=alpha, gain=gain, clamp=clamp)
        elif need[0] and hscale is not None:
            g_dy, _ = _cg.vjp_axpy(c, _f32(g_dd), y=y, act=1, alpha=alpha, gain=gain, clamp=clamp)
        if need[1] or need[2]:
            gxc = None
            if hscale is not None:
                wT = _cg._pack_conv(weight.transpose(0, 1), dt)
                dot_src = x if need[2] else None
                if _cg._halo_s2_ok(u, kh, kw, 2, tpad, dot=need[2]):
                    res = _cg.conv3x3_fused(u, wT, cin, in_scale=hscale, out_scale=s32, dot_src=dot_src, stride=2)
                else:
                    res = _cg.conv_fused(u, wT, cin, h, w, kh, kw, 2, tpad, in_scale=hscale, out_scale=s32,
                                         dot_src=dot_src)
                gxc = res[0]
                if need[2]:
                    g_s = res[2] if g_s is None else g_s + res[2]
            if need[1]:
                if g_ds is not None:
                    g_x, _ = (_cg.vjp_axpy(gxc, None, dxs, gds32) if gxc is not None else _cg.vjp_axpy(dxs, gds32))
                else:
                    g_x = gxc
        if need[3] and (G is not None or hscale is not None):
            acc = torch.zeros([cin * kh * kw * cout], dtype=torch.float32, device=x.device)
            if G is not None:
                g_w = _cg._wgrad_raw(G, u, kh, kw, 2, tpad, out=acc, param_layout='swap')
            if hscale is not None:
                g_w = _cg._wgrad_raw(x, u, kh, kw, 2, tpad, g_scale=s32, x_scale=hscale, out=acc, param_layout='swap')
            g_w = g_w.transpose(0, 1).to(weight.dtype)
        g_s = g_s.to(styles.dtype) if g_s is not None else None
        return (g_dy, g_x, g_s, g_w, g_d) + (None,) * 12


def up_modconv_layer(x, styles, weight, dcoefs, noise, bias, f, alpha, gain, clamp):
    return UpModConv.apply(x, styles, weight, dcoefs, noise, bias, f, float(alpha), float(gain),
                           float(clamp if clamp is not None else -1.0))
```

### gan-track_amd/torch_utils/ops/upfirdn2d.py

```python
import ctypes

import numpy as np
import torch

import sg2hip as _hip


def _parse_scaling(scaling):
    if isinstance(scaling, int):
        scaling = [scaling, scaling]
    assert isinstance(scaling, (list, tuple)) and all(isinstance(v, int) for v in scaling)
    sx, sy = scaling
    assert sx >= 1 and sy >= 1
    return sx, sy


def _parse_padding(padding):
    if isinstance(padding, int):
        padding = [padding, padding]
    assert isinstance(padding, (list, tuple)) and all(isinstance(v, int) for v in padding)
    if len(padding) == 2:
        px, py = padding
        padding = [px, px, py, py]
    px0, px1, py0, py1 = padding
    return px0, px1, py0, py1


def _get_filter_size(f):
    if f is None:
        return 1, 1
    assert isinstance(f, torch.Tensor) and f.ndim in [1, 2]
    fw = int(f.shape[-1])
    fh = int(f.shape[0])
    assert fw >= 1 and fh >= 1
    return fw, fh


def setup_filter(f, device=torch.device('cpu'), normalize=True, flip_filter=False, gain=1, separable=None):
    if f is None:
        f = 1
    f = torch.as_tensor(f, dtype=torch.float32)
    assert f.ndim in [0, 1, 2] and f.numel() > 0
    if f.ndim == 0:
        f = f[np.newaxis]
    if separable is None:
        separable = (f.ndim == 1 and f.numel() >= 8)
    if f.ndim == 1 and not separable:
        f = f.ger(f)
    assert f.ndim == (1 if separable else 2)
    if normalize:
        f /= f.sum()
    if flip_filter:
        f = f.flip(list(range(f.ndim)))
    f = f * (gain ** (f.ndim / 2))
    return f.to(device=device)


def _raw(x, f2, upx, upy, downx, downy, px0, px1, py0, py1, flip, gain):
    n, c, h, w = x.shape
    fh, fw = f2.shape
    oh = (h * upy + py0 + py1 - fh + downy) // downy
    ow = (w * upx + px0 + px1 - fw + downx) // downx
    assert oh >= 1 and ow >= 1, 'upfirdn2d: output would be empty'
    fmt = torch.channels_last if (x.stride(1) == 1 and c > 1) else torch.contiguous_format
    y = torch.empty([n, c, oh, ow], dtype=x.dtype, device=x.device, memory_format=fmt)
    _hip.check(_hip.lib().sg2_upfirdn2d(
        _hip.ptr(y), _hip.ptr(x), _hip.ptr(f2), _hip.dtype_code(x), _hip.i64arr(x.shape), _hip.i64arr(x.stride()),
        _hip.i64arr(y.shape), _hip.i64arr(y.stride()), fw, fh, upx, upy, downx, downy, px0, px1, py0, py1,
        int(bool(flip)), float(gain), _hip.stream_ptr(x.device)), 'sg2_upfirdn2d')
    return y


def _raw_lim(x, f2, upx, upy, downx, downy, px0, px1, py0, py1, flip, gain, lim):
    n, c, h, w = x.shape
    fh, fw = f2.shape
    oh = (h * upy + py0 + py1 - fh + downy) // downy
    ow = (w * upx + px0 + px1 - fw + downx) // downx
    y = torch.empty([n, c, oh, ow], dtype=x.dtype, device=x.device)
    _hip.check(_hip.lib().sg2_upfirdn2d_lim(
        _hip.ptr(y), _hip.ptr(x), _hip.ptr(f2), _hip.dtype_code(x), _hip.i64arr(x.shape), _hip.i64arr(x.stride()),
        _hip.i64arr(y.shape), _hip.i64arr(y.stride()), fw, fh, upx, upy, downx, downy, px0, px1, py0, py1,
        int(bool(flip)), float(gain), _hip.ptr(lim), _hip.stream_ptr(x.device)), 'sg2_upfirdn2d_lim')
    return y


class _SepLimited(torch.autograd.Function):

    @staticmethod
    def forward(ctx, x, f, up, down, padding, flip_filter, gain, lims):
        upx, upy = up
        downx, downy = down
        px0, px1, py0, py1 = padding
        x = x.contiguous()
        y = _raw_lim(x, f.unsqueeze(0), upx, 1, downx, 1, px0, px1, 0, 0, flip_filter, 1.0, lims[0])
        y = _raw_lim(y, f.unsqueeze(1), 1, upy, 1, downy, 0, 0, py0, py1, flip_filter, gain, lims[1])
        ctx.save_for_backward(f)
        ctx.cfg = (up, down, padding, flip_filter, gain, lims, x.shape)
        return y

    @staticmethod
    def backward(ctx, dy):
        f, = ctx.saved_tensors
        up, down, padding, flip_filter, gain, lims, xs = ctx.cfg
        aup, adown, p, aflip = adjoint_params(f, (xs[2], xs[3]), (dy.shape[2], dy.shape[3]), list(up), list(down),
                                              list(padding), flip_filter)
        dx = _SepLimited.apply(dy, f, tuple(aup), tuple(adown), tuple(p), aflip, gain,
                               (lims[2], lims[3], lims[0], lims[1]))
        return dx, None, None, None, None, None, None, None


def upsample2d_limited(x, f, lims, up=2, gain=1):
    _hip.require_device(x)
    assert f.ndim == 1 and x.dtype == torch.float32
    fw = f.shape[0]
    p = [(fw + up - 1) // 2, (fw - up) // 2] * 2
    return _SepLimited.apply(x, f.to(device=x.device, dtype=torch.float32).contiguous(), (up, up), (1, 1),
                             tuple(p), False, float(gain * up * up), tuple(lims))


def fir_fused(x, f2, padding, gain=1.0, flip_filter=False, out_scale=None, noise=None, noise_gain=1.0, bias=None,
              act=0, alpha=0.2, act_gain=1.0, clamp=-1.0, aux_mode=0):
    px0, px1, py0, py1 = _parse_padding(padding)
    n, c, h, w = x.shape
    fh, fw = f2.shape
    oh, ow = h + py0 + py1 - fh + 1, w + px0 + px1 - fw + 1
    y = torch.empty([n, c, oh, ow], dtype=x.dtype, device=x.device, memory_format=torch.channels_last)
    aux = torch.empty_like(y) if aux_mode else None
    epi = _hip.Epilogue(_hip.ptr(out_scale), _hip.ptr(noise), _hip.ptr(bias), None, _hip.ptr(aux), float(noise_gain),
                        float(alpha), float(act_gain), float(clamp), int(act), int(aux_mode))
    _hip.check(_hip.lib().sg2_upfirdn2d_fused(
        _hip.ptr(y), _hip.ptr(x), _hip.ptr(f2), _hip.dtype_code(x), _hip.i64arr(x.shape), _hip.i64arr(x.stride()),
        _hip.i64arr(y.shape), _hip.i64arr(y.stride()), fw, fh, 1, 1, 1, 1, px0, px1, py0, py1, int(bool(flip_filter)),
        float(gain), ctypes.byref(epi), _hip.stream_ptr(x.device)), 'sg2_upfirdn2d_fused')
    return y, aux


class _ForkFIR(torch.autograd.Function):

    @staticmethod
    def forward(ctx, x, f, down, padding):
        px0, px1, py0, py1 = padding
        y = _raw(x, f, 1, 1, down, down, px0, px1, py0, py1, False, 1.0)
        ctx.save_for_backward(f)
        ctx.cfg = (down, padding, x.shape)
        return x.view_as(x), y

    @staticmethod
    def backward(ctx, gx, gy):
        f, = ctx.saved_tensors
        down, padding, xs = ctx.cfg
        if gy is None:
            return gx, None, None, None
        aup, adown, p, aflip = adjoint_params(f, (xs[2], xs[3]), (gy.shape[2], gy.shape[3]), [1, 1], [down, down],
                                              list(padding), False)
        if torch.is_grad_enabled() or gx is None:
            dx = _upfirdn2d_fn(up=aup, down=adown, padding=p, flip_filter=aflip).apply(gy, f)
            return (dx + gx if gx is not None else dx), None, None, None
        cl = torch.channels_last
        gy = gy.contiguous(memory_format=cl)
        gx = gx.to(gy.dtype).contiguous(memory_format=cl)
        dx = torch.empty_like(gx)
        epi = _hip.Epilogue(None, None, None, _hip.ptr(gx), None, 1.0, 0.2, 1.0, -1.0, 0, 0)
        fh, fw = f.shape
        _hip.check(_hip.lib().sg2_upfirdn2d_fused(
            _hip.ptr(dx), _hip.ptr(gy), _hip.ptr(f), _hip.dtype_code(gy), _hip.i64arr(gy.shape),
            _hip.i64arr(gy.stride()), _hip.i64arr(dx.shape), _hip.i64arr(dx.stride()), fw, fh, aup[0], aup[1],
            adown[0], adown[1], p[0], p[1], p[2], p[3], int(bool(aflip)), 1.0, ctypes.byref(epi),
            _hip.stream_ptr(gy.device)), 'sg2_upfirdn2d_fused')
        return dx, None, None, None


def fork_fir(x, f, down, padding):
    _hip.require_device(x)
    px0, px1, py0, py1 = _parse_padding(padding)
    f = f.to(device=x.device, dtype=torch.float32).contiguous()
    return _ForkFIR.apply(x, f, int(down), (px0, px1, py0, py1))


def fork_fir_ok(x, f):
    v = 8 if x.dtype in (torch.float16, torch.bfloat16) else 4
    return (x.is_cuda and f is not None and f.ndim == 2 and x.ndim == 4 and x.shape[1] % v == 0 and
            x.is_contiguous(memory_format=torch.channels_last))


def adjoint_params(f, x_hw, y_hw, up, down, padding, flip_filter):
    upx, upy = _parse_scaling(up)
    downx, downy = _parse_scaling(down)
    px0, px1, py0, py1 = _parse_padding(padding)
    fw, fh = _get_filter_size(f)
    ih, iw = x_hw
    oh, ow = y_hw
    p = [fw - px0 - 1, iw * upx - ow * downx + px0 - upx + 1, fh - py0 - 1, ih * upy - oh * downy + py0 - upy + 1]
    return [downx, downy], [upx, upy], p, not flip_filter


_cache = {}


def _upfirdn2d_fn(up=1, down=1, padding=0, flip_filter=False, gain=1):
    upx, upy = _parse_scaling(up)
    downx, downy = _parse_scaling(down)
    px0, px1, py0, py1 = _parse_padding(padding)
    key = (upx, upy, downx, downy, px0, px1, py0, py1, flip_filter, gain)
    if key in _cache:
        return _cache[key]

    class Upfirdn2d(torch.autograd.Function):
        @staticmethod
        def forward(ctx, x, f):
            assert x.ndim == 4
            if f is None:
                f = torch.ones([1, 1], dtype=torch.float32, device=x.device)
            if f.ndim == 1 and f.shape[0] == 1:
                f = f.square().unsqueeze(0)
            f = f.to(device=x.device, dtype=torch.float32).contiguous()
            if f.ndim == 2:
                y = _raw(x, f, upx, upy, downx, downy, px0, px1, py0, py1, flip_filter, gain)
            else:
                y = _raw(x, f.unsqueeze(0), upx, 1, downx, 1, px0, px1, 0, 0, flip_filter, 1.0)
                y = _raw(y, f.unsqueeze(1), 1, upy, 1, downy, 0, 0, py0, py1, flip_filter, gain)
            ctx.save_for_backward(f)
            ctx.x_shape = x.shape
            return y

        @staticmethod
        def backward(ctx, dy):
            f, = ctx.saved_tensors
            _, _, ih, iw = ctx.x_shape
            _, _, oh, ow = dy.shape
            aup, adown, p, aflip = adjoint_params(f, (ih, iw), (oh, ow), [upx, upy], [downx, downy],
                                                  [px0, px1, py0, py1], flip_filter)
            dx = None
            if ctx.needs_input_grad[0]:
                dx = _upfirdn2d_fn(up=aup, down=adown, padding=p, flip_filter=aflip, gain=gain).apply(dy, f)
            assert not ctx.needs_input_grad[1]
            return dx, None

    _cache[key] = Upfirdn2d
    return Upfirdn2d


def upfirdn2d(x, f, up=1, down=1, padding=0, flip_filter=False, gain=1, impl='cuda'):
    assert isinstance(x, torch.Tensor)
    _hip.require_device(x)
    return _upfirdn2d_fn(up=up, down=down, padding=padding, flip_filter=flip_filter, gain=gain).apply(x, f)


def filter2d(x, f, padding=0, flip_filter=False, gain=1, impl='cuda'):
    px0, px1, py0, py1 = _parse_padding(padding)
    fw, fh = _get_filter_size(f)
    p = [px0 + fw // 2, px1 + (fw - 1) // 2, py0 + fh // 2, py1 + (fh - 1) // 2]
    return upfirdn2d(x, f, padding=p, flip_filter=flip_filter, gain=gain, impl=impl)


def upsample2d(x, f, up=2, padding=0, flip_filter=False, gain=1, impl='cuda'):
    upx, upy = _parse_scaling(up)
    px0, px1, py0, py1 = _parse_padding(padding)
    fw, fh = _get_filter_size(f)
    p = [px0 + (fw + upx - 1) // 2, px1 + (fw - upx) // 2, py0 + (fh + upy - 1) // 2, py1 + (fh - upy) // 2]
    return upfirdn2d(x, f, up=up, padding=p, flip_filter=flip_filter, gain=gain * upx * upy, impl=impl)


def downsample2d(x, f, down=2, padding=0, flip_filter=False, gain=1, impl='cuda'):
    downx, downy = _parse_scaling(down)
    px0, px1, py0, py1 = _parse_padding(padding)
    fw, fh = _get_filter_size(f)
    p = [px0 + (fw - downx + 1) // 2, px1 + (fw - downx) // 2, py0 + (fh - downy + 1) // 2, py1 + (fh - downy) // 2]
    return upfirdn2d(x, f, down=down, padding=p, flip_filter=flip_filter, gain=gain, impl=impl)
```

### gan-track_amd/training/networks_stylegan2.py

```python
import numpy as np
import torch

import sg2hip as _hip
from torch_utils import misc
from torch_utils import persistence
from torch_utils.ops import bias_act
from torch_utils.ops import conv2d_gradfix
from torch_utils.ops import conv2d_resample
from torch_utils.ops import fma
from torch_utils.ops import modconv
from torch_utils.ops import staged_sum
from torch_utils.ops import upfirdn2d

_CL = torch.channels_last


def normalize_2nd_moment(x, dim=1, eps=1e-8):
    return x * (x.square().mean(dim=dim, keepdim=True) + eps).rsqrt()


class _InfNorm(torch.autograd.Function):

    @staticmethod
    def forward(ctx, t_in, c, mode):
        t = t_in.contiguous()
        rows, L = t.shape
        y = torch.empty_like(t)
        nrm = torch.empty([rows], dtype=torch.float32, device=t.device)
        _hip.check(_hip.lib().sg2_infnorm_fwd(_hip.ptr(y), _hip.ptr(nrm), _hip.ptr(t), rows, L, float(c), mode,
                                              _hip.stream_ptr(t.device)), 'sg2_infnorm_fwd')
        ctx.save_for_backward(t_in, nrm)
        ctx.c, ctx.mode = c, mode
        return y

    @staticmethod
    def backward(ctx, dy):
        t, nrm = ctx.saved_tensors
        if not ctx.needs_input_grad[0]:
            return None, None, None
        if torch.is_grad_enabled():
            return _InfNormVJP.apply(dy, t, nrm, ctx.c if ctx.mode == 0 else 1.0, ctx.mode), None, None
        dy, t = dy.contiguous(), t.contiguous()
        dt = torch.empty_like(t)
        _hip.check(_hip.lib().sg2_infnorm_bwd(_hip.ptr(dt), _hip.ptr(dy), _hip.ptr(t), _hip.ptr(nrm), t.shape[0],
                                              t.shape[1], float(ctx.c), ctx.mode, _hip.stream_ptr(t.device)),
                   'sg2_infnorm_bwd')
        return dt, None, None


class _InfNormVJP(torch.autograd.Function):

    @staticmethod
    def forward(ctx, dy, t, nrm, c, mode):
        dy, t = dy.contiguous(), t.contiguous()
        dt = torch.empty_like(t)
        _hip.check(_hip.lib().sg2_infnorm_bwd(_hip.ptr(dt), _hip.ptr(dy), _hip.ptr(t), _hip.ptr(nrm), t.shape[0],
                                              t.shape[1], float(c), mode, _hip.stream_ptr(t.device)), 'sg2_infnorm_bwd')
        ctx.save_for_backward(dy, t, nrm)
        ctx.c = c
        return dt

    @staticmethod
    def backward(ctx, g):
        dy, t, nrm = ctx.saved_tensors
        g = g.float().contiguous()
        g_dy = torch.empty_like(dy) if ctx.needs_input_grad[0] else None
        g_t = torch.empty_like(t) if ctx.needs_input_grad[1] else None
        _hip.check(_hip.lib().sg2_infnorm_vjp_bwd(_hip.ptr(g_dy), _hip.ptr(g_t), _hip.ptr(g), _hip.ptr(dy),
                                                  _hip.ptr(t), _hip.ptr(nrm), t.shape[0], t.shape[1], float(ctx.c),
                                                  _hip.stream_ptr(t.device)), 'sg2_infnorm_vjp_bwd')
        return g_dy, g_t, None, None, None


def _prenorm(weight, styles):
    o, i, kh, kw = weight.shape
    if weight.dtype != torch.float32 or styles.dtype != torch.float32:
        return (weight * (1 / np.sqrt(i * kh * kw) / weight.norm(float('inf'), dim=[1, 2, 3], keepdim=True)),
                styles / styles.norm(float('inf'), dim=1, keepdim=True))
    w = _InfNorm.apply(weight.reshape(o, -1), float(np.float32(1 / np.sqrt(i * kh * kw))), 0).reshape(o, i, kh, kw)
    return w, _InfNorm.apply(styles, 1.0, 1)


class _Demod(torch.autograd.Function):

    @staticmethod
    def forward(ctx, weight, styles):
        w = weight.float().contiguous()
        s = styles.float().contiguous()
        n, o, i, kk = s.shape[0], w.shape[0], w.shape[1], w.shape[2] * w.shape[3]
        d = torch.empty([n, o], dtype=torch.float32, device=s.device)
        wsq = torch.empty([o, i], dtype=torch.float32, device=s.device)
        _hip.check(_hip.lib().sg2_demod_fwd(_hip.ptr(d), _hip.ptr(wsq), _hip.ptr(s), _hip.ptr(w), n, o, i, kk, 1e-8,
                                            _hip.stream_ptr(s.device)), 'sg2_demod_fwd')
        ctx.save_for_backward(w, s, d, wsq)
        return d

    @staticmethod
    def backward(ctx, dd):
        w, s, d, wsq = ctx.saved_tensors
        need_w, need_s = ctx.needs_input_grad[0], ctx.needs_input_grad[1]
        if torch.is_grad_enabled():
            need_w = need_w and not conv2d_gradfix.weight_gradients_disabled
            if need_s and not need_w:
                return None, _DemodVJP.apply(dd, d, w, s, wsq)
            gu = dd * d.pow(3) * -0.5
            gs = 2 * s * (gu @ w.square().sum([2, 3])) if need_s else None
            gw = 2 * w * (gu.t() @ s.square())[:, :, None, None] if need_w else None
            return gw, gs
        dd = dd.float().contiguous()
        n, o, i, kk = s.shape[0], w.shape[0], w.shape[1], w.shape[2] * w.shape[3]
        gw = torch.empty_like(w) if need_w else None
        gs = torch.empty_like(s) if need_s else None
        _hip.check(_hip.lib().sg2_demod_bwd(_hip.ptr(gs), _hip.ptr(gw), _hip.ptr(dd), _hip.ptr(d), _hip.ptr(s),
                                            _hip.ptr(w), _hip.ptr(wsq), n, o, i, kk, _hip.stream_ptr(s.device)),
                   'sg2_demod_bwd')
        return gw, gs


class _DemodVJP(torch.autograd.Function):

    @staticmethod
    def forward(ctx, dd, d, w, s, wsq):
        dd = dd.float().contiguous()
        n, o, i, kk = s.shape[0], w.shape[0], w.shape[1], w.shape[2] * w.shape[3]
        gs = torch.empty_like(s)
        _hip.check(_hip.lib().sg2_demod_bwd(_hip.ptr(gs), _hip.ptr(None), _hip.ptr(dd), _hip.ptr(d), _hip.ptr(s), _hip.ptr(w),
                                            _hip.ptr(wsq), n, o, i, kk, _hip.stream_ptr(s.device)), 'sg2_demod_bwd')
        ctx.save_for_backward(dd, d, w, s, wsq)
        return gs

    @staticmethod
    def backward(ctx, g):
        dd, d, w, s, wsq = ctx.saved_tensors
        g = g.float().contiguous()
        need = ctx.needs_input_grad
        g_dd = torch.empty_like(dd) if need[0] else None
        g_d = torch.empty_like(d) if need[1] else None
        g_w = torch.empty_like(w) if need[2] else None
        g_s = torch.empty_like(s) if need[3] else None
        n, o, i, kk = s.shape[0], w.shape[0], w.shape[1], w.shape[2] * w.shape[3]
        _hip.check(_hip.lib().sg2_demod_vjp_bwd(_hip.ptr(g_dd), _hip.ptr(g_d), _hip.ptr(g_w), _hip.ptr(g_s),
                                                _hip.ptr(g), _hip.ptr(dd), _hip.ptr(d), _hip.ptr(s), _hip.ptr(w),
                                                _hip.ptr(wsq), n, o, i, kk, _hip.stream_ptr(s.device)),
                   'sg2_demod_vjp_bwd')
        return g_dd, g_d, g_w, g_s, None


def _demod(weight, styles):
    if weight.shape[1] <= 1024 and weight.shape[0] <= 1024 and styles.shape[0] <= 1024:
        return _Demod.apply(weight, styles)
    wsq = weight.float().square().sum(dim=[2, 3])
    return (styles.float().square() @ wsq.t() + 1e-8).rsqrt()


def modulated_conv2d(x, weight, styles, noise=None, up=1, down=1, padding=0, resample_filter=None,
                     demodulate=True, flip_weight=True, fused_modconv=True):
    n = x.shape[0]
    out_ch, in_ch, kh, kw = weight.shape
    misc.assert_shape(weight, [out_ch, in_ch, kh, kw])
    misc.assert_shape(x, [n, in_ch, None, None])
    misc.assert_shape(styles, [n, in_ch])
    if x.dtype == torch.float16 and demodulate:
        weight, styles = _prenorm(weight, styles)
    dcoefs = _demod(weight, styles) if demodulate else None
    x = x * styles.to(x.dtype).reshape(n, -1, 1, 1)
    x = conv2d_resample.conv2d_resample(x=x, w=weight.to(x.dtype), f=resample_filter, up=up, down=down,
                                        padding=padding, flip_weight=flip_weight)
    if demodulate and noise is not None:
        return fma.fma(x, dcoefs.to(x.dtype).reshape(n, -1, 1, 1), noise.to(x.dtype))
    if demodulate:
        return x * dcoefs.to(x.dtype).reshape(n, -1, 1, 1)
    if noise is not None:
        return x + noise.to(x.dtype)
    return x


class _Addmm(torch.autograd.Function):

    @staticmethod
    def forward(ctx, b, x, w, beta, alpha):
        ctx.save_for_backward(x, w)
        ctx.beta, ctx.alpha = beta, alpha
        return torch.addmm(b, x, w.t(), beta=beta, alpha=alpha)

    @staticmethod
    def backward(ctx, dy):
        x, w = ctx.saved_tensors
        beta, alpha = ctx.beta, ctx.alpha
        nb, nx, nw = ctx.needs_input_grad[:3]
        if torch.is_grad_enabled():
            pg = not conv2d_gradfix.weight_gradients_disabled
            return ((dy.sum(0) * beta) if nb and pg else None, (dy @ w) * alpha if nx else None,
                    (dy.t() @ x) * alpha if nw and pg else None, None, None)
        z = _zero_scalar(dy)
        db = None
        if nb:
            db = torch.addmv(_zero_vec(dy, dy.shape[1]), dy.t(), _ones(dy, dy.shape[0]), beta=0, alpha=beta) \
                if beta != 1 else dy.sum(0)
        dx = torch.addmm(z, dy, w, beta=0, alpha=alpha) if nx else None
        dw = torch.addmm(z, dy.t(), x, beta=0, alpha=alpha) if nw else None
        return db, dx, dw, None, None


def _zero_scalar(t):
    return torch.empty((), dtype=t.dtype, device=t.device)


def _zero_vec(t, n):
    return torch.empty((n,), dtype=t.dtype, device=t.device)


_ONES = {}


def _ones(t, n):
    key = (n, t.dtype, t.device)
    v = _ONES.get(key)
    if v is None:
        v = _ONES[key] = torch.ones(n, dtype=t.dtype, device=t.device)
    return v


@persistence.persistent_class
class FullyConnectedLayer(torch.nn.Module):

    def __init__(self, in_features, out_features, bias=True, activation='linear', lr_multiplier=1, bias_init=0):
        super().__init__()
        self.in_features, self.out_features, self.activation = in_features, out_features, activation
        self.weight = torch.nn.Parameter(torch.randn([out_features, in_features]) / lr_multiplier)
        self.bias = torch.nn.Parameter(torch.full([out_features], np.float32(bias_init))) if bias else None
        self.weight_gain = lr_multiplier / np.sqrt(in_features)
        self.bias_gain = lr_multiplier

    def forward(self, x, out_gain=1):
        w = self.weight if self.weight.dtype == x.dtype else self.weight.to(x.dtype)
        b = self.bias
        if b is not None:
            b = b if b.dtype == x.dtype else b.to(x.dtype)
            if self.activation == 'linear':
                return _Addmm.apply(b, x, w, float(self.bias_gain * out_gain), float(self.weight_gain * out_gain))
            y = _Addmm.apply(b, x, w, float(self.bias_gain), float(self.weight_gain))
            return bias_act.bias_act(y, None, act=self.activation)
        y = x.matmul((w * (self.weight_gain * out_gain)).t())
        return bias_act.bias_act(y, None, act=self.activation) if self.activation != 'linear' else y

    def extra_repr(self):
        return f'in_features={self.in_features:d}, out_features={self.out_features:d}, activation={self.activation:s}'


grouped_affine = True
_PLAN_CACHE = {}


def _style_plan(layers, n, num_ws, device):
    key = (tuple((int(a.out_features), float(a.weight_gain), float(a.bias_gain), int(k), float(g)) for a, k, g in layers),
           n, num_ws, str(device))
    plan = _PLAN_CACHE.get(key)
    if plan is not None:
        return plan
    tot = sum(a.out_features for a, _, _ in layers)
    idx, bidx, alpha, beta, spans = [], [], [], [], []
    col, off = 0, 0
    for a, k, g in layers:
        c = a.out_features
        rows = np.arange(n)[:, None] * num_ws + k
        cols = col + np.arange(c)[None, :]
        idx.append((rows * tot + cols).reshape(-1))
        bidx.append((np.arange(n)[:, None] * tot + cols).reshape(-1))
        alpha.append(np.full(n * c, np.float32(a.weight_gain * g), np.float32))
        beta.append(np.full(c, np.float32(a.bias_gain * g), np.float32))
        spans.append((off, c))
        col += c
        off += n * c
    T = lambda v, dt: torch.as_tensor(np.concatenate(v), dtype=dt, device=device)
    plan = (T(idx, torch.int64), T(bidx, torch.int64), T(alpha, torch.float32), T(beta, torch.float32),
            torch.ones([n, 1], dtype=torch.float32, device=device), spans)
    _PLAN_CACHE[key] = plan
    return plan


def grouped_styles(ws, layers):
    n, num_ws, d = ws.shape
    W = torch.cat([a.weight for a, _, _ in layers])
    b = torch.cat([a.bias for a, _, _ in layers])
    S = torch.mm(ws.reshape(n * num_ws, d), W.t())
    idx, bidx, alpha, beta, ones, spans = _style_plan(layers, n, num_ws, ws.device)
    B = torch.mm(ones, (b * beta).view(1, -1))
    out = torch.addcmul(B.take(bidx), S.take(idx), alpha)
    return [t.view(n, c) for t, (_, c) in zip(out.split([n * c for _, c in spans]), spans)]


@persistence.persistent_class
class Conv2dLayer(torch.nn.Module):

    def __init__(self, in_channels, out_channels, kernel_size, bias=True, activation='linear', up=1, down=1,
                 resample_filter=[1, 3, 3, 1], conv_clamp=None, channels_last=False, trainable=True):
        super().__init__()
        self.in_channels, self.out_channels, self.activation = in_channels, out_channels, activation
        self.up, self.down, self.conv_clamp = up, down, conv_clamp
        self.register_buffer('resample_filter', upfirdn2d.setup_filter(resample_filter))
        self.padding = kernel_size // 2
        self.weight_gain = 1 / np.sqrt(in_channels * (kernel_size ** 2))
        self.act_gain = bias_act.activation_funcs[activation].def_gain
        weight = torch.randn([out_channels, in_channels, kernel_size, kernel_size])
        bias = torch.zeros([out_channels]) if bias else None
        if trainable:
            self.weight = torch.nn.Parameter(weight)
            self.bias = torch.nn.Parameter(bias) if bias is not None else None
        else:
            self.register_buffer('weight', weight)
            if bias is not None:
                self.register_buffer('bias', bias)
            else:
                self.bias = None

    def forward(self, x, gain=1, residual=None, prefiltered=False):
        clamp = self.conv_clamp * gain if self.conv_clamp is not None else None
        kh = self.weight.shape[2]
        if self.activation in ('lrelu', 'linear') and self.up == 1 and modconv.supported_generic(x, self.weight):
            stride, pad = 1, self.padding
            if self.down > 1:
                x0, x1, y0, y1 = conv2d_resample._frame_padding(self.padding, self.resample_filter, 1, self.down)
                if kh == 1:
                    if not prefiltered:
                        x = upfirdn2d.upfirdn2d(x, self.resample_filter, down=self.down, padding=[x0, x1, y0, y1])
                else:
                    x = upfirdn2d.upfirdn2d(x, self.resample_filter, padding=[x0, x1, y0, y1])
                    stride = self.down
                pad = 0
            return modconv.fused_conv(x, self.weight, bias=self.bias, residual=residual, stride=stride, padding=pad,
                                      act=self.activation, alpha=bias_act.activation_funcs[self.activation].def_alpha or 0.2,
                                      gain=self.act_gain * gain, clamp=clamp, wgain=self.weight_gain)
        w = self.weight * self.weight_gain
        b = self.bias.to(x.dtype) if self.bias is not None else None
        pre = prefiltered and self.down > 1 and kh == 1
        x = conv2d_resample.conv2d_resample(x=x, w=w.to(x.dtype), f=None if pre else self.resample_filter, up=self.up,
                                            down=1 if pre else self.down, padding=self.padding,
                                            flip_weight=(self.up == 1))
        x = bias_act.bias_act(x, b, act=self.activation, gain=self.act_gain * gain, clamp=clamp)
        return x if residual is None else residual.add_(x)

    def extra_repr(self):
        return (f'in_channels={self.in_channels:d}, out_channels={self.out_channels:d}, '
                f'activation={self.activation:s}, up={self.up}, down={self.down}')


@persistence.persistent_class
class MappingNetwork(torch.nn.Module):

    def __init__(self, z_dim, c_dim, w_dim, num_ws, num_layers=8, embed_features=None, layer_features=None,
                 activation='lrelu', lr_multiplier=0.01, w_avg_beta=0.998):
        super().__init__()
        self.z_dim, self.c_dim, self.w_dim, self.num_ws = z_dim, c_dim, w_dim, num_ws
        self.num_layers, self.w_avg_beta = num_layers, w_avg_beta
        if embed_features is None:
            embed_features = w_dim
        if c_dim == 0:
            embed_features = 0
        if layer_features is None:
            layer_features = w_dim
        feats = [z_dim + embed_features] + [layer_features] * (num_layers - 1) + [w_dim]
        if c_dim > 0:
            self.embed = FullyConnectedLayer(c_dim, embed_features)
        for idx in range(num_layers):
            setattr(self, f'fc{idx}', FullyConnectedLayer(feats[idx], feats[idx + 1], activation=activation,
                                                          lr_multiplier=lr_multiplier))
        if num_ws is not None and w_avg_beta is not None:
            self.register_buffer('w_avg', torch.zeros([w_dim]))

    def forward(self, z, c, truncation_psi=1, truncation_cutoff=None, update_emas=False):
        x = None
        if self.z_dim > 0:
            misc.assert_shape(z, [None, self.z_dim])
            x = normalize_2nd_moment(z.to(torch.float32))
        if self.c_dim > 0:
            misc.assert_shape(c, [None, self.c_dim])
            y = normalize_2nd_moment(self.embed(c.to(torch.float32)))
            x = torch.cat([x, y], dim=1) if x is not None else y
        for idx in range(self.num_layers):
            x = getattr(self, f'fc{idx}')(x)
        if update_emas and self.w_avg_beta is not None:
            self.w_avg.copy_(x.detach().mean(dim=0).lerp(self.w_avg, self.w_avg_beta))
        if self.num_ws is not None:
            x = x.unsqueeze(1).repeat([1, self.num_ws, 1])
        if truncation_psi != 1:
            assert self.w_avg_beta is not None
            if self.num_ws is None or truncation_cutoff is None:
                x = self.w_avg.lerp(x, truncation_psi)
            else:
                x[:, :truncation_cutoff] = self.w_avg.lerp(x[:, :truncation_cutoff], truncation_psi)
        return x

    def extra_repr(self):
        return f'z_dim={self.z_dim:d}, c_dim={self.c_dim:d}, w_dim={self.w_dim:d}, num_ws={self.num_ws}'


@persistence.persistent_class
class SynthesisLayer(torch.nn.Module):

    def __init__(self, in_channels, out_channels, w_dim, resolution, kernel_size=3, up=1, use_noise=True,
                 activation='lrelu', resample_filter=[1, 3, 3, 1], conv_clamp=None, channels_last=False):
        super().__init__()
        self.in_channels, self.out_channels, self.w_dim = in_channels, out_channels, w_dim
        self.resolution, self.up, self.use_noise = resolution, up, use_noise
        self.activation, self.conv_clamp = activation, conv_clamp
        self.register_buffer('resample_filter', upfirdn2d.setup_filter(resample_filter))
        self.padding = kernel_size // 2
        self.act_gain = bias_act.activation_funcs[activation].def_gain
        self.affine = FullyConnectedLayer(w_dim, in_channels, bias_init=1)
        self.weight = torch.nn.Parameter(torch.randn([out_channels, in_channels, kernel_size, kernel_size]))
        if use_noise:
            self.register_buffer('noise_const', torch.randn([resolution, resolution]))
            self.noise_strength = torch.nn.Parameter(torch.zeros([]))
        self.bias = torch.nn.Parameter(torch.zeros([out_channels]))

    def forward(self, x, w, noise_mode='random', fused_modconv=True, gain=1, styles=None):
        assert noise_mode in ['random', 'const', 'none']
        misc.assert_shape(x, [None, self.in_channels, self.resolution // self.up, self.resolution // self.up])
        if styles is None:
            styles = self.affine(w)
        noise = None
        if self.use_noise and noise_mode == 'random':
            noise = staged_sum.scale_by_scalar(torch.randn([x.shape[0], 1, self.resolution, self.resolution],
                                                           device=x.device), self.noise_strength)
        if self.use_noise and noise_mode == 'const':
            noise = staged_sum.scale_by_scalar(self.noise_const, self.noise_strength)
        up_fused = self.up == 2 and modconv.supported_up(x, self.weight, self.resample_filter)
        if self.activation == 'lrelu' and (up_fused or (self.up == 1 and modconv.supported_generic(x, self.weight))):
            weight = self.weight
            if x.dtype == torch.float16:
                weight, styles = _prenorm(weight, styles)
            if noise is not None and noise.ndim == 2:
                noise = noise.reshape(1, 1, *noise.shape).expand(x.shape[0], 1, -1, -1)
            clamp = self.conv_clamp * gain if self.conv_clamp is not None else None
            if up_fused:
                return modconv.up_modconv_layer(x, styles, weight, _demod(weight, styles), noise, self.bias,
                                                self.resample_filter,
                                                alpha=bias_act.activation_funcs[self.activation].def_alpha,
                                                gain=self.act_gain * gain, clamp=clamp)
            return modconv.modconv_layer(x, styles, weight, _demod(weight, styles), noise, self.bias,
                                         alpha=bias_act.activation_funcs[self.activation].def_alpha,
                                         gain=self.act_gain * gain, clamp=clamp)
        x = modulated_conv2d(x=x, weight=self.weight, styles=styles, noise=noise, up=self.up, padding=self.padding,
                             resample_filter=self.resample_filter, flip_weight=(self.up == 1),
                             fused_modconv=fused_modconv)
        clamp = self.conv_clamp * gain if self.conv_clamp is not None else None
        return bias_act.bias_act(x, self.bias.to(x.dtype), act=self.activation, gain=self.act_gain * gain, clamp=clamp)

    def extra_repr(self):
        return (f'in_channels={self.in_channels:d}, out_channels={self.out_channels:d}, w_dim={self.w_dim:d}, '
                f'resolution={self.resolution:d}, up={self.up}, activation={self.activation:s}')


@persistence.persistent_class
class ToRGBLayer(torch.nn.Module):

    def __init__(self, in_channels, out_channels, w_dim, kernel_size=1, conv_clamp=None, channels_last=False):
        super().__init__()
        self.in_channels, self.out_channels, self.w_dim = in_channels, out_channels, w_dim
        self.conv_clamp = conv_clamp
        self.affine = FullyConnectedLayer(w_dim, in_channels, bias_init=1)
        self.weight = torch.nn.Parameter(torch.randn([out_channels, in_channels, kernel_size, kernel_size]))
        self.bias = torch.nn.Parameter(torch.zeros([out_channels]))
        self.weight_gain = 1 / np.sqrt(in_channels * (kernel_size ** 2))

    def forward(self, x, w, fused_modconv=True, styles=None):
        if styles is None:
            styles = self.affine(w, out_gain=self.weight_gain)
        if modconv.supported_generic(x, self.weight):
            return modconv.fused_conv(x, self.weight, styles=styles, bias=self.bias,
                                      padding=self.weight.shape[-1] // 2, clamp=self.conv_clamp)
        x = modulated_conv2d(x=x, weight=self.weight, styles=styles, demodulate=False, fused_modconv=fused_modconv)
        return bias_act.bias_act(x, self.bias.to(x.dtype), clamp=self.conv_clamp)

    def forward_tap(self, x, w, fused_modconv=True, styles=None):
        if styles is None:
            styles = self.affine(w, out_gain=self.weight_gain)
        if modconv.tap_enabled and modconv.supported_generic(x, self.weight):
            return modconv.fused_conv_tap(x, self.weight, styles, self.bias, self.weight.shape[-1] // 2,
                                          self.conv_clamp)
        return x, self.forward(x, w, fused_modconv=fused_modconv, styles=styles)

    def extra_repr(self):
        return f'in_channels={self.in_channels:d}, out_channels={self.out_channels:d}, w_dim={self.w_dim:d}'


@persistence.persistent_class
class SynthesisBlock(torch.nn.Module):

    def __init__(self, in_channels, out_channels, w_dim, resolution, img_channels, is_last, architecture='skip',
                 resample_filter=[1, 3, 3, 1], conv_clamp=256, use_fp16=False, fp16_channels_last=False,
                 fused_modconv_default=True, fp16_dtype=torch.float16, **layer_kwargs):
        assert architecture in ['orig', 'skip', 'resnet']
        super().__init__()
        self.in_channels, self.w_dim, self.resolution = in_channels, w_dim, resolution
        self.img_channels, self.is_last, self.architecture = img_channels, is_last, architecture
        self.use_fp16, self.fp16_dtype = use_fp16, fp16_dtype
        self.channels_last = True
        self.fused_modconv_default = fused_modconv_default
        self.register_buffer('resample_filter', upfirdn2d.setup_filter(resample_filter))
        self.num_conv = 0
        self.num_torgb = 0
        if in_channels == 0:
            self.const = torch.nn.Parameter(torch.randn([out_channels, resolution, resolution]))
        if in_channels != 0:
            self.conv0 = SynthesisLayer(in_channels, out_channels, w_dim=w_dim, resolution=resolution, up=2,
                                        resample_filter=resample_filter, conv_clamp=conv_clamp, **layer_kwargs)
            self.num_conv += 1
        self.conv1 = SynthesisLayer(out_channels, out_channels, w_dim=w_dim, resolution=resolution,
                                    conv_clamp=conv_clamp, **layer_kwargs)
        self.num_conv += 1
        if is_last or architecture == 'skip':
            self.torgb = ToRGBLayer(out_channels, img_channels, w_dim=w_dim, conv_clamp=conv_clamp)
            self.num_torgb += 1
        if in_channels != 0 and architecture == 'resnet':
            self.skip = Conv2dLayer(in_channels, out_channels, kernel_size=1, bias=False, up=2,
                                    resample_filter=resample_filter)

    def style_layers(self):
        out, k = [], 0
        if self.in_channels != 0:
            out.append((self.conv0.affine, k, 1.0))
            k += 1
        out.append((self.conv1.affine, k, 1.0))
        k += 1
        if self.is_last or self.architecture == 'skip':
            out.append((self.torgb.affine, k, float(self.torgb.weight_gain)))
        return out

    def forward(self, x, img, ws, force_fp32=False, fused_modconv=None, update_emas=False, styles=None,
                **layer_kwargs):
        misc.assert_shape(ws, [None, self.num_conv + self.num_torgb, self.w_dim])
        if styles is not None:
            s_iter = iter(styles)
            w_iter = iter([None] * len(styles))
        else:
            s_iter = iter([None] * (self.num_conv + self.num_torgb))
            w_iter = iter(ws.unbind(dim=1))
        dtype = self.fp16_dtype if self.use_fp16 and not force_fp32 else torch.float32
        if fused_modconv is None:
            fused_modconv = self.fused_modconv_default
        if fused_modconv == 'inference_only':
            fused_modconv = not self.training
        if self.in_channels == 0:
            x = self.const.to(dtype=dtype).unsqueeze(0).repeat([ws.shape[0], 1, 1, 1])
            x = x.contiguous(memory_format=_CL)
        else:
            misc.assert_shape(x, [None, self.in_channels, self.resolution // 2, self.resolution // 2])
            x = x.to(dtype=dtype, memory_format=_CL)
        if self.in_channels == 0:
            x = self.conv1(x, next(w_iter), fused_modconv=fused_modconv, styles=next(s_iter), **layer_kwargs)
        elif self.architecture == 'resnet':
            y = self.skip(x, gain=np.sqrt(0.5))
            x = self.conv0(x, next(w_iter), fused_modconv=fused_modconv, styles=next(s_iter), **layer_kwargs)
            x = self.conv1(x, next(w_iter), fused_modconv=fused_modconv, gain=np.sqrt(0.5), styles=next(s_iter),
                           **layer_kwargs)
            x = y.add_(x)
        else:
            x = self.conv0(x, next(w_iter), fused_modconv=fused_modconv, styles=next(s_iter), **layer_kwargs)
            x = self.conv1(x, next(w_iter), fused_modconv=fused_modconv, styles=next(s_iter), **layer_kwargs)
        if img is not None:
            misc.assert_shape(img, [None, self.img_channels, self.resolution // 2, self.resolution // 2])
            img = upfirdn2d.upsample2d(img, self.resample_filter)
        if self.is_last or self.architecture == 'skip':
            if self.is_last:
                y = self.torgb(x, next(w_iter), fused_modconv=fused_modconv, styles=next(s_iter))
            else:
                x, y = self.torgb.forward_tap(x, next(w_iter), fused_modconv=fused_modconv, styles=next(s_iter))
            y = y.to(dtype=torch.float32, memory_format=torch.contiguous_format)
            img = img.add_(y) if img is not None else y
        assert x.dtype == dtype
        assert img is None or img.dtype == torch.float32
        return x, img

    def extra_repr(self):
        return f'resolution={self.resolution:d}, architecture={self.architecture:s}'


@persistence.persistent_class
class SynthesisNetwork(torch.nn.Module):

    def __init__(self, w_dim, img_resolution, img_channels, channel_base=32768, channel_max=512, num_fp16_res=4,
                 **block_kwargs):
        assert img_resolution >= 4 and img_resolution & (img_resolution - 1) == 0
        super().__init__()
        self.w_dim, self.img_resolution, self.img_channels = w_dim, img_resolution, img_channels
        self.img_resolution_log2 = int(np.log2(img_resolution))
        self.num_fp16_res = num_fp16_res
        self.block_resolutions = [2 ** i for i in range(2, self.img_resolution_log2 + 1)]
        channels = {r: min(channel_base // r, channel_max) for r in self.block_resolutions}
        fp16_resolution = max(2 ** (self.img_resolution_log2 + 1 - num_fp16_res), 8)
        self.num_ws = 0
        for r in self.block_resolutions:
            block = SynthesisBlock(channels[r // 2] if r > 4 else 0, channels[r], w_dim=w_dim, resolution=r,
                                   img_channels=img_channels, is_last=(r == img_resolution),
                                   use_fp16=(r >= fp16_resolution), **block_kwargs)
            self.num_ws += block.num_conv
            if r == img_resolution:
                self.num_ws += block.num_torgb
            setattr(self, f'b{r}', block)

    def forward(self, ws, **block_kwargs):
        misc.assert_shape(ws, [None, self.num_ws, self.w_dim])
        ws = ws.to(torch.float32)
        x = img = None
        styles = None
        if grouped_affine and ws.is_cuda:
            plan, w_idx = [], 0
            for r in self.block_resolutions:
                block = getattr(self, f'b{r}')
                plan += [(a, w_idx + k, g) for a, k, g in block.style_layers()]
                w_idx += block.num_conv
            styles = iter(grouped_styles(ws, plan))
        w_idx = 0
        for r in self.block_resolutions:
            block = getattr(self, f'b{r}')
            cur = ws.narrow(1, w_idx, block.num_conv + block.num_torgb)
            w_idx += block.num_conv
            bs = [next(styles) for _ in block.style_layers()] if styles is not None else None
            x, img = block(x, img, cur, styles=bs, **block_kwargs)
        return img

    def extra_repr(self):
        return (f'w_dim={self.w_dim:d}, num_ws={self.num_ws:d}, img_resolution={self.img_resolution:d}, '
                f'img_channels={self.img_channels:d}, num_fp16_res={self.num_fp16_res:d}')


@persistence.persistent_class
class Generator(torch.nn.Module):

    def __init__(self, z_dim, c_dim, w_dim, img_resolution, img_channels, mapping_kwargs={}, **synthesis_kwargs):
        super().__init__()
        self.z_dim, self.c_dim, self.w_dim = z_dim, c_dim, w_dim
        self.img_resolution, self.img_channels = img_resolution, img_channels
        self.synthesis = SynthesisNetwork(w_dim=w_dim, img_resolution=img_resolution, img_channels=img_channels,
                                          **synthesis_kwargs)
        self.num_ws = self.synthesis.num_ws
        self.mapping = MappingNetwork(z_dim=z_dim, c_dim=c_dim, w_dim=w_dim, num_ws=self.num_ws, **mapping_kwargs)

    def forward(self, z, c, truncation_psi=1, truncation_cutoff=None, update_emas=False, **synthesis_kwargs):
        ws = self.mapping(z, c, truncation_psi=truncation_psi, truncation_cutoff=truncation_cutoff,
                          update_emas=update_emas)
        return self.synthesis(ws, update_emas=update_emas, **synthesis_kwargs)


@persistence.persistent_class
class DiscriminatorBlock(torch.nn.Module):

    def __init__(self, in_channels, tmp_channels, out_channels, resolution, img_channels, first_layer_idx,
                 architecture='resnet', activation='lrelu', resample_filter=[1, 3, 3, 1], conv_clamp=None,
                 use_fp16=False, fp16_channels_last=False, freeze_layers=0, fp16_dtype=torch.float16):
        assert in_channels in [0, tmp_channels]
        assert architecture in ['orig', 'skip', 'resnet']
        super().__init__()
        self.in_channels, self.resolution, self.img_channels = in_channels, resolution, img_channels
        self.first_layer_idx, self.architecture = first_layer_idx, architecture
        self.use_fp16, self.fp16_dtype = use_fp16, fp16_dtype
        self.channels_last = True
        self.register_buffer('resample_filter', upfirdn2d.setup_filter(resample_filter))
        self.num_layers = 0

        def next_trainable():
            layer_idx = self.first_layer_idx + self.num_layers
            self.num_layers += 1
            return layer_idx >= freeze_layers

        if in_channels == 0 or architecture == 'skip':
            self.fromrgb = Conv2dLayer(img_channels, tmp_channels, kernel_size=1, activation=activation,
                                       trainable=next_trainable(), conv_clamp=conv_clamp)
        self.conv0 = Conv2dLayer(tmp_channels, tmp_channels, kernel_size=3, activation=activation,
                                 trainable=next_trainable(), conv_clamp=conv_clamp)
        self.conv1 = Conv2dLayer(tmp_channels, out_channels, kernel_size=3, activation=activation, down=2,
                                 trainable=next_trainable(), resample_filter=resample_filter, conv_clamp=conv_clamp)
        if architecture == 'resnet':
            self.skip = Conv2dLayer(tmp_channels, out_channels, kernel_size=1, bias=False, down=2,
                                    trainable=next_trainable(), resample_filter=resample_filter)

    def forward(self, x, img, force_fp32=False):
        dtype = self.fp16_dtype if self.use_fp16 and not force_fp32 else torch.float32
        if x is not None:
            misc.assert_shape(x, [None, self.in_channels, self.resolution, self.resolution])
            x = x.to(dtype=dtype, memory_format=_CL)
        if self.in_channels == 0 or self.architecture == 'skip':
            misc.assert_shape(img, [None, self.img_channels, self.resolution, self.resolution])
            img = img.to(dtype=dtype, memory_format=_CL)
            y = self.fromrgb(img)
            x = x + y if x is not None else y
            img = upfirdn2d.downsample2d(img, self.resample_filter) if self.architecture == 'skip' else None
        if self.architecture == 'resnet':
            sk = self.skip
            if sk.down > 1 and sk.weight.shape[2] == 1 and upfirdn2d.fork_fir_ok(x, sk.resample_filter):
                pad = conv2d_resample._frame_padding(sk.padding, sk.resample_filter, 1, sk.down)
                x, xd = upfirdn2d.fork_fir(x, sk.resample_filter, sk.down, pad)
                y = sk(xd, gain=np.sqrt(0.5), prefiltered=True)
            else:
                y = self.skip(x, gain=np.sqrt(0.5))
            x = self.conv0(x)
            x = self.conv1(x, gain=np.sqrt(0.5), residual=y)
        else:
            x = self.conv0(x)
            x = self.conv1(x)
        assert x.dtype == dtype
        return x, img

    def extra_repr(self):
        return f'resolution={self.resolution:d}, architecture={self.architecture:s}'


@persistence.persistent_class
class MinibatchStdLayer(torch.nn.Module):

    def __init__(self, group_size, num_channels=1):
        super().__init__()
        self.group_size, self.num_channels = group_size, num_channels
        self.segments = None

    def forward(self, x):
        seg = getattr(self, 'segments', None)
        if seg is not None and len(seg) > 1:
            return torch.cat([self._forward(part) for part in x.split(list(seg))])
        return self._forward(x)

    def _forward(self, x):
        N, C, H, W = x.shape
        G = min(self.group_size, N) if self.group_size is not None else N
        F = self.num_channels
        c = C // F
        y = x.reshape(G, -1, F, c, H, W)
        y = y - y.mean(dim=0)
        y = y.square().mean(dim=0)
        y = (y + 1e-8).sqrt()
        y = y.mean(dim=[2, 3, 4])
        y = y.reshape(-1, F, 1, 1).repeat(G, 1, H, W)
        return torch.cat([x, y], dim=1)

    def extra_repr(self):
        return f'group_size={self.group_size}, num_channels={self.num_channels:d}'


@persistence.persistent_class
class DiscriminatorEpilogue(torch.nn.Module):

    def __init__(self, in_channels, cmap_dim, resolution, img_channels, architecture='resnet', mbstd_group_size=4,
                 mbstd_num_channels=1, activation='lrelu', conv_clamp=None):
        assert architecture in ['orig', 'skip', 'resnet']
        super().__init__()
        self.in_channels, self.cmap_dim, self.resolution = in_channels, cmap_dim, resolution
        self.img_channels, self.architecture = img_channels, architecture
        if architecture == 'skip':
            self.fromrgb = Conv2dLayer(img_channels, in_channels, kernel_size=1, activation=activation)
        self.mbstd = MinibatchStdLayer(group_size=mbstd_group_size, num_channels=mbstd_num_channels) \
            if mbstd_num_channels > 0 else None
        self.conv = Conv2dLayer(in_channels + mbstd_num_channels, in_channels, kernel_size=3, activation=activation,
                                conv_clamp=conv_clamp)
        self.fc = FullyConnectedLayer(in_channels * (resolution ** 2), in_channels, activation=activation)
        self.out = FullyConnectedLayer(in_channels, 1 if cmap_dim == 0 else cmap_dim)

    def forward(self, x, img, cmap, force_fp32=False):
        misc.assert_shape(x, [None, self.in_channels, self.resolution, self.resolution])
        x = x.to(dtype=torch.float32, memory_format=torch.contiguous_format)
        if self.architecture == 'skip':
            img = img.to(dtype=torch.float32, memory_format=torch.contiguous_format)
            x = x + self.fromrgb(img)
        if self.mbstd is not None:
            x = self.mbstd(x)
        x = self.conv(x)
        x = self.fc(x.contiguous().flatten(1))
        x = self.out(x)
        if self.cmap_dim > 0:
            misc.assert_shape(cmap, [None, self.cmap_dim])
            x = (x * cmap).sum(dim=1, keepdim=True) * (1 / np.sqrt(self.cmap_dim))
        assert x.dtype == torch.float32
        return x

    def extra_repr(self):
        return f'resolution={self.resolution:d}, architecture={self.architecture:s}'


@persistence.persistent_class
class Discriminator(torch.nn.Module):

    def __init__(self, c_dim, img_resolution, img_channels, architecture='resnet', channel_base=32768,
                 channel_max=512, num_fp16_res=4, conv_clamp=256, cmap_dim=None, block_kwargs={}, mapping_kwargs={},
                 epilogue_kwargs={}):
        super().__init__()
        self.c_dim, self.img_resolution, self.img_channels = c_dim, img_resolution, img_channels
        self.img_resolution_log2 = int(np.log2(img_resolution))
        self.block_resolutions = [2 ** i for i in range(self.img_resolution_log2, 2, -1)]
        channels = {r: min(channel_base // r, channel_max) for r in self.block_resolutions + [4]}
        fp16_resolution = max(2 ** (self.img_resolution_log2 + 1 - num_fp16_res), 8)
        if cmap_dim is None:
            cmap_dim = channels[4]
        if c_dim == 0:
            cmap_dim = 0
        common = dict(img_channels=img_channels, architecture=architecture, conv_clamp=conv_clamp)
        layer_idx = 0
        for r in self.block_resolutions:
            block = DiscriminatorBlock(channels[r] if r < img_resolution else 0, channels[r], channels[r // 2],
                                       resolution=r, first_layer_idx=layer_idx, use_fp16=(r >= fp16_resolution),
                                       **block_kwargs, **common)
            setattr(self, f'b{r}', block)
            layer_idx += block.num_layers
        if c_dim > 0:
            self.mapping = MappingNetwork(z_dim=0, c_dim=c_dim, w_dim=cmap_dim, num_ws=None, w_avg_beta=None,
                                          **mapping_kwargs)
        self.b4 = DiscriminatorEpilogue(channels[4], cmap_dim=cmap_dim, resolution=4, **epilogue_kwargs, **common)

    def forward(self, img, c, update_emas=False, **block_kwargs):
        x = None
        for r in self.block_resolutions:
            x, img = getattr(self, f'b{r}')(x, img, **block_kwargs)
        cmap = self.mapping(None, c) if self.c_dim > 0 else None
        return self.b4(x, img, cmap)

    def extra_repr(self):
        return f'c_dim={self.c_dim:d}, img_resolution={self.img_resolution:d}, img_channels={self.img_channels:d}'
```

### include/sg2hip.h

```cpp
#ifndef SG2HIP_H
#define SG2HIP_H

#include <stdint.h>

#ifdef __cplusplus
extern "C" {
#endif

#define SG2_ABI_VERSION 11

enum sg2_dtype { SG2_F32 = 0, SG2_F16 = 1, SG2_BF16 = 2, SG2_F32S3 = 3 };

int sg2_split3(void* planes, const float* x, int64_t n, int C, int64_t pix_per_n, const float* scale, void* stream);

int sg2_abi_version(void);

const char* sg2_last_error(void);

int sg2_bias_act(void* y, const void* x, const void* b, const void* xref, const void* yref, const void* dy,
                 int dtype, int64_t numel, int64_t size_b, int64_t step_b, int grad, int act, float alpha,
                 float gain, float clamp, void* stream);

int sg2_upfirdn2d(void* y, const void* x, const float* f, int dtype, const int64_t* in_size,
                  const int64_t* in_stride, const int64_t* out_size, const int64_t* out_stride, int fw, int fh,
                  int upx, int upy, int downx, int downy, int padx0, int padx1, int pady0, int pady1, int flip,
                  float gain, void* stream);

int sg2_upfirdn2d_lim(void* y, const void* x, const float* f, int dtype, const int64_t* in_size,
                      const int64_t* in_stride, const int64_t* out_size, const int64_t* out_stride, int fw, int fh,
                      int upx, int upy, int downx, int downy, int padx0, int padx1, int pady0, int pady1, int flip,
                      float gain, const int* lim, void* stream);

typedef struct sg2_epilogue sg2_epilogue;
int sg2_upfirdn2d_fused(void* y, const void* x, const float* f, int dtype, const int64_t* in_size,
                        const int64_t* in_stride, const int64_t* out_size, const int64_t* out_stride, int fw, int fh,
                        int upx, int upy, int downx, int downy, int padx0, int padx1, int pady0, int pady1, int flip,
                        float gain, const sg2_epilogue* epi, void* stream);

int sg2_conv2d(void* y, const void* x, const void* w, int dtype, int N, int Cin, int H, int W, int Cout,
               int OH, int OW, int KH, int KW, int stride, int pad_y, int pad_x, int transpose,
               float* workspace, int64_t workspace_elems, void* stream);

struct sg2_epilogue {
    const float* out_scale;
    const void* noise;
    const float* bias;
    const void* residual;
    void* aux;
    float noise_gain, alpha, gain, clamp;
    int act;
    int aux_mode;
    const void* dot_src;
    float* dot_out;
};

int sg2_conv2d_fused(void* y, const void* x, const void* w, int dtype, int N, int Cin, int H, int W, int Cout,
                     int OH, int OW, int KH, int KW, int stride, int pad_y, int pad_x, int transpose,
                     const float* in_scale, const sg2_epilogue* epi, float* workspace, int64_t workspace_elems,
                     void* stream);

int sg2_conv3x3(void* y, void* y_raw, const void* x, const void* w, int dtype, int N, int Cin, int H, int W,
                int Cout, const float* in_scale, const float* out_scale, const void* noise, float noise_gain,
                const float* bias, int act, float alpha, float gain, float clamp, const void* dot_src,
                float* dot_out, void* stream);

void sg2_set_zeroed_accumulators(int on);

void sg2_set_clean_workspace(int on);

void sg2_set_deterministic(void* scratch, int64_t bytes);

int sg2_conv3x3_s2(void* y, void* y_raw, const void* x, const void* w, int dtype, int N, int Cin, int H, int W,
                   int Cout, const float* in_scale, const float* out_scale, const void* noise, float noise_gain,
                   const float* bias, int act, float alpha, float gain, float clamp, const void* residual,
                   int raw_act, const void* dot_src, float* dot_out, void* stream);

int sg2_conv3x3_up2(void* y, const void* x, const void* w, int dtype, int N, int Cin, int H, int W, int Cout,
                    const float* in_scale, void* stream);

int sg2_conv2d_wgrad(float* dw, const void* g, const void* x, int dtype, int N, int A, int OH, int OW, int B,
                     int H, int W, int KH, int KW, int stride, int pad_y, int pad_x, const float* g_scale,
                     const float* x_scale, float alpha, void* stream);

int sg2_conv2d_wgrad_oikk(float* dw, const void* g, const void* x, int dtype, int N, int A, int OH, int OW, int B,
                          int H, int W, int KH, int KW, int stride, int pad_y, int pad_x, float alpha, int swap_ab,
                          void* stream);

int sg2_layer_bwd(void* dc, float* db, float* dd, float* dnoise, const void* dy, const void* y, const void* c,
                  const float* d, int dtype, int N, int HW, int C, int act, float alpha, float gain, float clamp,
                  void* stream);

int sg2_vjp_axpy(void* out, const void* a, const float* sa, const void* b, const float* sb, const void* y, int act,
                 float alpha, float gain, float clamp, const void* e, float* dot, int dtype, int N, int HW, int C,
                 void* stream);

int sg2_dot_hw(float* out, const void* a, const void* b, int dtype, int N, int HW, int C, void* stream);

int sg2_grid_sample_fwd(void* out, const void* in, const float* grid, int dtype, const int64_t* in_size,
                        const int64_t* in_stride, const int64_t* out_size, const int64_t* out_stride,
                        const int* dyn_hw, void* stream);

int sg2_grid_sample_bwd(float* gin, const void* gout, const float* grid, int dtype, const int64_t* in_size,
                        const int64_t* in_stride, const int64_t* out_size, const int64_t* out_stride,
                        const int* dyn_hw, void* stream);

int sg2_affine_grid_sample_fwd(void* out, const void* in, const float* theta, int dtype, const int64_t* in_size,
                               const int64_t* in_stride, const int64_t* out_size, const int64_t* out_stride,
                               const int* dyn_hw, void* stream);
int sg2_affine_grid_sample_bwd(float* gin, const void* gout, const float* theta, int dtype, const int64_t* in_size,
                               const int64_t* in_stride, const int64_t* out_size, const int64_t* out_stride,
                               const int* dyn_hw, void* stream);


int sg2_reflect_pad_dyn(float* y, const float* x, const int* margins, int N, int C, int H, int W, int Hs, int Ws,
                        int adjoint, void* stream);

typedef struct sg2_aug_geom_args {
    const float* draw[16];
    const float* p;
    float xflip, rotate90, xint, xint_max, scale, rotate, aniso, xfrac;
    float scale_std, rotate_max, aniso_std, xfrac_std;
    float pad_x, pad_y, inv_sx, inv_sy;
    int n, h, w;
} sg2_aug_geom_args;
int sg2_aug_geom(float* theta, int* margins, int* lims, int* dyn_hw, const sg2_aug_geom_args* args, void* stream);

int sg2_moments(double* row, const float* v, int64_t n, int mode, void* stream);

int sg2_demod_fwd(float* d, float* wsq, const float* s, const float* w, int N, int O, int I, int KK, float eps,
                  void* stream);

int sg2_demod_bwd(float* gs, float* gw, const float* dd, const float* d, const float* s, const float* w,
                  const float* wsq, int N, int O, int I, int KK, void* stream);

int sg2_demod_vjp_bwd(float* g_dd, float* g_d, float* g_w, float* g_s, const float* g, const float* dd,
                      const float* d, const float* s, const float* w, const float* wsq, int N, int O, int I, int KK,
                      void* stream);

int sg2_pack_weight(void* out, int out_dtype, const void* in, int in_dtype, int A, int B, int K, int64_t sa,
                    int64_t sb, int64_t sk, int flip, float scale, void* stream);

typedef struct sg2_pack_desc {
    void* out;
    const void* in;
    int64_t sa, sb, sk;
    int out_dtype, in_dtype, A, B, K, flip;
    float scale;
    int block0;
} sg2_pack_desc;
int sg2_pack_weight_multi(const sg2_pack_desc* descs, int n, void* stream);

int sg2_infnorm_fwd(float* y, float* nrm, const float* t, int rows, int L, float c, int mode, void* stream);

int sg2_infnorm_bwd(float* dt, const float* dy, const float* t, const float* nrm, int rows, int L, float c, int mode,
                    void* stream);

int sg2_infnorm_vjp_bwd(float* g_dy, float* g_t, const float* g, const float* dy, const float* t, const float* nrm,
                        int rows, int L, float c, void* stream);


int sg2_adam_multi(const int64_t* seg, const float* coef, const int64_t* blocks, int nblocks, float* grad,
                   float* exp_avg, float* exp_avg_sq, float beta1, float beta2, float eps, float grad_scale,
                   int write_grad, void* stream);

int sg2_lerp_multi(const int64_t* seg, const int64_t* blocks, int nblocks, float beta, void* stream);

int sg2_knn_scratch_bytes(int64_t* bytes, int64_t rows, int64_t cols, int k);
int sg2_knn_radii(float* radii, const void* x, int dtype, int64_t n, int d, int k, int round16, void* scratch,
                  int64_t scratch_bytes, void* stream);
int sg2_manifold_member(uint8_t* hit, const void* probes, int64_t p, const void* manifold, int64_t n,
                        const float* radii, int dtype, int d, int round16, void* scratch, int64_t scratch_bytes,
                        void* stream);

int sg2_noise_reg_scratch_bytes(int64_t* bytes, const int64_t* table, int nbuf);
int sg2_noise_reg_fwd(float* reg, float* means, const float* flat, const int64_t* table, int nbuf, void* scratch,
                      void* stream);
int sg2_noise_reg_bwd(float* gflat, const float* greg, const float* means, const float* flat, const int64_t* table,
                      int nbuf, const void* scratch, int accumulate, void* stream);
int sg2_noise_normalize_multi(float* flat, const int64_t* table, int nbuf, void* stream);

#ifdef __cplusplus
}
#endif

#endif
```

Before: 788.3 imgs/s.

## Fuse FIR upfirdn with activation gradient and bias reduction; fork discriminator skip downsample

Adds an activation-gradient mode to the upfirdn2d kernels. The FIR backward output is combined in place with the leaky-ReLU/clamp gradient mask, and per-block partial bias-gradient sums are written, which removes separate bias_act backward and reduction passes. In the discriminator, the conv0 output is pre-filtered for the strided conv1, and the next block's skip downsample is forked out of the current block's conv1. This cuts separate FIR launches and extra reads of activations. It adds more complex kernel paths, extra template instantiations and bigger LDS use in the AG variants.

```diff
diff --git a/gan-track_amd/csrc/upfirdn2d.hip b/gan-track_amd/csrc/upfirdn2d.hip
--- a/gan-track_amd/csrc/upfirdn2d.hip
+++ b/gan-track_amd/csrc/upfirdn2d.hip
@@ -28,6 +28,11 @@
     int act, aux_mode, epi;
     const int* lim;
     int xcd;
+    const void* ag_ys;
+    void* ag_dc;
+    float* ag_db;
+    float ag_gain, ag_alpha, ag_clamp;
+    int ag_act, ag_store_v;
 };
 
 constexpr int kZeroBand = 32;
@@ -251,7 +256,32 @@
 template <> struct VecN<float> { static constexpr int N = 4; };
 
 template <typename T, int V, typename vecT>
-__device__ __forceinline__ void store_out(const UpfParams& p, T* y, const float* acc, int n, int oy, int ox, int cv) {
+__device__ __forceinline__ void actgrad_vec(const UpfParams& p, const vecT& o, const vecT& yv, int64_t q, bool own,
+                                            float* adb) {
+    vecT d;
+#pragma unroll
+    for (int j = 0; j < V; ++j) {
+        const float yy = (float)yv[j];
+        float dz = (float)o[j] * p.ag_gain;
+        if (p.ag_act == 1 && !(yy > 0.f)) dz *= p.ag_alpha;
+        if (p.ag_clamp >= 0.f && !(yy > -p.ag_clamp && yy < p.ag_clamp)) dz = 0.f;
+        adb[j] += own ? dz : 0.f;
+        d[j] = (T)dz;
+    }
+    *(vecT*)((T*)p.ag_dc + q) = d;
+}
+
+__device__ __forceinline__ void actgrad_slot(const UpfParams& p, float* part, const float* adb) {
+    const int CV = p.C / 8;
+    det_rows_store(part, p.C, threadIdx.x / CV, (threadIdx.x % CV) * 8, adb);
+    __syncthreads();
+    for (int i = threadIdx.x; i < p.C; i += 256)
+        p.ag_db[(int64_t)blockIdx.x * p.C + i] = det_rows_sum(part, p.C, 256 / CV, i);
+}
+
+template <typename T, int V, typename vecT, bool AG = false>
+__device__ __forceinline__ void store_out(const UpfParams& p, T* y, const float* acc, int n, int oy, int ox, int cv,
+                                          float* adb = nullptr) {
     const int64_t dst = n * p.ys_n + (int64_t)oy * p.ys_h + (int64_t)ox * p.ys_w + cv * V;
     vecT o;
     if (p.epi) {
@@ -277,16 +307,22 @@
 #pragma unroll
         for (int j = 0; j < V; ++j) o[j] = (T)acc[j];
     }
+    if constexpr (AG) {
+        const int64_t q = (((int64_t)n * p.OH + oy) * p.OW + ox) * p.C + cv * V;
+        actgrad_vec<T, V, vecT>(p, o, *(const vecT*)((const T*)p.ag_ys + q), q, true, adb);
+        if (!p.ag_store_v) return;
+    }
     *(vecT*)(y + dst) = o;
 }
 
 
-template <typename T, typename IDX>
+template <typename T, typename IDX, bool AG = false>
 __global__ __launch_bounds__(256) void upfirdn_nhwc_vec(UpfParams p) {
     constexpr int V = VecN<T>::N;
     typedef T vecT __attribute__((ext_vector_type(V)));
-    __shared__ float sf[kMaxTaps];
+    __shared__ float sf[AG ? 2048 : kMaxTaps];
     stage_filter(sf, p);
+    float adb[8] = {0.f, 0.f, 0.f, 0.f, 0.f, 0.f, 0.f, 0.f};
     const T* x = (const T*)p.x;
     T* y = (T*)p.y;
     const IDX CV = (IDX)(p.C / V), OW = (IDX)p.OW, OH = (IDX)p.OH;
@@ -315,7 +351,12 @@
                 for (int j = 0; j < V; ++j) acc[j] += (float)v[j] * wt;
             }
         }
-        store_out<T, V, vecT>(p, y, acc, n, oy, ox, cv);
+        store_out<T, V, vecT, AG>(p, y, acc, n, oy, ox, cv, adb);
+    }
+    if constexpr (AG) {
+        if (!p.ag_db) return;
+        __syncthreads();
+        actgrad_slot(p, sf, adb);
     }
 }
 
@@ -330,16 +371,10 @@
     return r;
 }
 
-template <typename T>
-__global__ __launch_bounds__(256) void upfirdn_nhwc_up2(UpfParams p) {
+template <typename T, bool AG>
+__device__ __forceinline__ void up2_cell(const UpfParams& p, const float* sf, float* adb) {
     constexpr int V = VecN<T>::N;
     typedef T vecT __attribute__((ext_vector_type(V)));
-    __shared__ float sf[16];
-    if (threadIdx.x < 16) {
-        const int ty = threadIdx.x >> 2, tx = threadIdx.x & 3;
-        sf[threadIdx.x] = p.f[(p.flip ? ty : 3 - ty) * 4 + (p.flip ? tx : 3 - tx)] * p.gain;
-    }
-    __syncthreads();
     const unsigned CV = p.C / V, CW = (p.OW + 1) >> 1, CH = (p.OH + 1) >> 1;
     const unsigned total = (unsigned)p.N * CH * CW * CV;
     const unsigned idx = blockIdx.x * 256u + threadIdx.x;
@@ -402,9 +437,106 @@
                     }
                 }
             }
-            store_out<T, V, vecT>(p, (T*)p.y, acc, n, oy, ox, cv);
-        }
-    }
+            store_out<T, V, vecT, AG>(p, (T*)p.y, acc, n, oy, ox, cv, adb);
+        }
+    }
+}
+
+template <typename T, bool AG = false>
+__global__ __launch_bounds__(256) void upfirdn_nhwc_up2(UpfParams p) {
+    __shared__ float sf[AG ? 2048 : 16];
+    if (threadIdx.x < 16) {
+        const int ty = threadIdx.x >> 2, tx = threadIdx.x & 3;
+        sf[threadIdx.x] = p.f[(p.flip ? ty : 3 - ty) * 4 + (p.flip ? tx : 3 - tx)] * p.gain;
+    }
+    __syncthreads();
+    float adb[8] = {0.f, 0.f, 0.f, 0.f, 0.f, 0.f, 0.f, 0.f};
+    up2_cell<T, AG>(p, sf, adb);
+    if constexpr (AG) {
+        if (!p.ag_db) return;
+        __syncthreads();
+        actgrad_slot(p, sf, adb);
+    }
+}
+
+template <typename T>
+__global__ __launch_bounds__(256) void upfirdn_up2_lbo(UpfParams p, int ppb) {
+    constexpr int V = 8;
+    typedef T vecT __attribute__((ext_vector_type(V)));
+    extern __shared__ __attribute__((aligned(16))) float lbo_part[];
+    __shared__ float sf[16];
+    if (threadIdx.x < 16) {
+        const int ty = threadIdx.x >> 2, tx = threadIdx.x & 3;
+        sf[threadIdx.x] = p.f[(p.flip ? ty : 3 - ty) * 4 + (p.flip ? tx : 3 - tx)] * p.gain;
+    }
+    __syncthreads();
+    const int LP = p.C / V, PPP = 256 / LP;
+    const int HW = p.OH * p.OW, n = blockIdx.y;
+    const int p0 = blockIdx.x * ppb, p1 = min(HW, p0 + ppb);
+    const int cv = threadIdx.x % LP, pl = threadIdx.x / LP;
+    const T* xb = (const T*)p.x + n * p.xs_n + cv * V;
+    float adb[V];
+#pragma unroll
+    for (int j = 0; j < V; ++j) adb[j] = 0.f;
+    constexpr int U = 4;
+    for (int pb = p0 + pl; pb < p1; pb += PPP * U) {
+        vecT xv[U][2][2];
+        int tyu[U], txu[U];
+#pragma unroll
+        for (int u = 0; u < U; ++u) {
+            const int px = pb + u * PPP;
+            const int oy = px / p.OW, ox = px - oy * p.OW;
+            int iy, ix;
+            axis_taps(oy, 1, p.pady0, 2, tyu[u], iy);
+            axis_taps(ox, 1, p.padx0, 2, txu[u], ix);
+#pragma unroll
+            for (int a = 0; a < 2; ++a)
+#pragma unroll
+                for (int b = 0; b < 2; ++b) {
+                    const int yy = iy + a, xx = ix + b;
+                    const bool ok = px < p1 && yy >= 0 && yy < p.H && xx >= 0 && xx < p.W;
+                    xv[u][a][b] = ok ? *(const vecT*)(xb + yy * p.xs_h + xx * p.xs_w) : vecT{};
+                }
+        }
+#pragma unroll
+        for (int u = 0; u < U; ++u) {
+            const int px = pb + u * PPP;
+            if (px >= p1) break;
+            const int oy = px / p.OW, ox = px - oy * p.OW;
+            float acc[V];
+#pragma unroll
+            for (int j = 0; j < V; ++j) acc[j] = 0.f;
+#pragma unroll
+            for (int a = 0; a < 2; ++a) {
+                const int t1 = tyu[u] + 2 * a;
+                if (t1 >= 4) continue;
+#pragma unroll
+                for (int b = 0; b < 2; ++b) {
+                    const int t2 = txu[u] + 2 * b;
+                    if (t2 >= 4) continue;
+                    const float w = sf[t1 * 4 + t2];
+                    const vecT v = xv[u][a][b];
+                    if constexpr (std::is_same<T, f16_t>::value) {
+                        typedef unsigned u32v __attribute__((ext_vector_type(V / 2)));
+                        const u32v uu = __builtin_bit_cast(u32v, v);
+#pragma unroll
+                        for (int q = 0; q < V / 2; ++q) {
+                            acc[2 * q] = fma_mix_lo(uu[q], w, acc[2 * q]);
+                            acc[2 * q + 1] = fma_mix_hi(uu[q], w, acc[2 * q + 1]);
+                        }
+                    } else {
+#pragma unroll
+                        for (int j = 0; j < V; ++j) acc[j] += (float)v[j] * w;
+                    }
+                }
+            }
+            store_out<T, V, vecT, true>(p, (T*)p.y, acc, n, oy, ox, cv, adb);
+        }
+    }
+    det_rows_store(lbo_part, p.C, pl, cv * V, adb);
+    __syncthreads();
+    const int slot = blockIdx.y * gridDim.x + blockIdx.x;
+    for (int i = threadIdx.x; i < p.C; i += 256) p.ag_db[(int64_t)slot * p.C + i] = det_rows_sum(lbo_part, p.C, PPP, i);
 }
 
 template <typename T, int DOWN, int TW, int TH, int CG>
@@ -480,9 +612,11 @@
     }
 }
 
-template <typename T, int V, typename vecT, int TW, int TH, int CG, bool SEP, bool EPI>
+template <typename T, int V, typename vecT, int TW, int TH, int CG, bool SEP, bool EPI, bool AG = false>
 __device__ __forceinline__ void fir4_strip(const UpfParams& p, const vecT* base, const float* wf, const float* fy,
-                                           const float* fx, int n, int ty0, int ox, int cv) {
+                                           const float* fx, int n, int ty0, int ox, int cv,
+                                           const vecT* ysv = nullptr, int own_r0 = 0, bool own_c = true,
+                                           float* adb = nullptr) {
     constexpr int F = 4, IW = TW + F - 1, IH = TH + F - 1;
     float os[V], bj[V];
 #pragma unroll
@@ -556,7 +690,13 @@
             vecT o;
 #pragma unroll
             for (int j = 0; j < V; ++j) o[j] = (T)acc[od][j];
-            *(vecT*)((T*)p.y + dst) = o;
+            if constexpr (AG) {
+                const int64_t q = (((int64_t)n * p.OH + oy) * p.OW + ox) * p.C + cv * V;
+                actgrad_vec<T, V, vecT>(p, o, ysv[od], q, own_c && od >= own_r0, adb);
+                if (p.ag_store_v) *(vecT*)((T*)p.y + dst) = o;
+            } else {
+                *(vecT*)((T*)p.y + dst) = o;
+            }
             __builtin_amdgcn_sched_barrier(0);
             continue;
         }
@@ -581,7 +721,7 @@
     }
 }
 
-template <typename T, int TW, int TH, int CG = 8>
+template <typename T, int TW, int TH, int CG = 8, bool AG = false>
 __global__ __launch_bounds__(256, 2) void upfirdn_nhwc_f4s(UpfParams p) {
     constexpr int V = VecN<T>::N, F = 4;
     constexpr int IW = TW + F - 1, IH = TH + F - 1, NIN = IW * IH * CG;
@@ -603,8 +743,9 @@
     int64_t b = blockIdx.x;
     const int64_t nb = gridDim.x;
     if ((nb & 7) == 0) b = (b & 7) * (nb >> 3) + (b >> 3);
-    const int tx0 = min((int)(b % tiles_x) * TW, p.OW - TW); b /= tiles_x;
-    const int ty0 = min((int)(b % tiles_y) * TH, p.OH - TH); b /= tiles_y;
+    const int tix = (int)(b % tiles_x); b /= tiles_x;
+    const int tiy = (int)(b % tiles_y); b /= tiles_y;
+    const int tx0 = min(tix * TW, p.OW - TW), ty0 = min(tiy * TH, p.OH - TH);
     const int cg = (int)(b % ngroups); b /= ngroups;
     const int n = (int)b;
     const int cv0 = cg * CG;
@@ -623,12 +764,22 @@
 #pragma unroll
         for (int j = 0; j < V; ++j) r[l][j] = ok ? r[l][j] : (T)0.f;
     }
+    const int c = tid % CG, col = tid / CG;
+    const bool live = cv0 + c < CV;
+    vecT ysv[AG ? TH : 1];
+    if constexpr (AG) {
+#pragma unroll
+        for (int o = 0; o < TH; ++o)
+            ysv[o] = *(const vecT*)((const T*)p.ag_ys + (((int64_t)n * p.OH + ty0 + o) * p.OW + tx0 + col) * p.C +
+                                    (live ? cv0 + c : 0) * V);
+    }
 #pragma unroll
     for (int l = 0; l < NL; ++l)
         if (l < NL - 1 || tid + l * 256 < NIN) tile[tid + l * 256] = r[l];
     __syncthreads();
-    const int c = tid % CG, col = tid / CG;
-    if (cv0 + c >= CV) return;
+    if constexpr (!AG) {
+        if (!live) return;
+    }
     float fy[F], fx[F];
     bool sep = wf[0] != 0.f;
 #pragma unroll
@@ -639,6 +790,31 @@
 #pragma unroll
     for (int t = 0; t < F * F; ++t) sep = sep && (fy[t / F] * fx[t % F] == wf[t]);
     const vecT* tb = tile + col * CG + c;
+    if constexpr (AG) {
+        float adb[V];
+#pragma unroll
+        for (int j = 0; j < V; ++j) adb[j] = 0.f;
+        if (live) {
+            const int own_r0 = tiy * TH - ty0;
+            const bool own_c = col >= tix * TW - tx0;
+            if (sep) fir4_strip<T, V, vecT, TW, TH, CG, true, false, true>(p, tb, wf, fy, fx, n, ty0, tx0 + col, cv0 + c,
+                                                                           ysv, own_r0, own_c, adb);
+            else fir4_strip<T, V, vecT, TW, TH, CG, false, false, true>(p, tb, wf, fy, fx, n, ty0, tx0 + col, cv0 + c,
+                                                                        ysv, own_r0, own_c, adb);
+        }
+        if (!p.ag_db) return;
+        __syncthreads();
+        float* part = (float*)tile_raw;
+#pragma unroll
+        for (int j = 0; j < V; ++j) part[col * (CG * V) + c * V + j] = adb[j];
+        __syncthreads();
+        if (tid < CG * V && cv0 * V + tid < p.C) {
+            float sum = 0.f;
+            for (int k = 0; k < TW; ++k) sum += part[k * (CG * V) + tid];
+            p.ag_db[(((int64_t)n * tiles_y + tiy) * tiles_x + tix) * p.C + cv0 * V + tid] = sum;
+        }
+        return;
+    }
     if (sep) {
         if (p.epi) fir4_strip<T, V, vecT, TW, TH, CG, true, true>(p, tb, wf, fy, fx, n, ty0, tx0 + col, cv0 + c);
         else fir4_strip<T, V, vecT, TW, TH, CG, true, false>(p, tb, wf, fy, fx, n, ty0, tx0 + col, cv0 + c);
@@ -649,9 +825,11 @@
 }
 
 template <typename T>
-int launch(const UpfParams& p, bool vec, hipStream_t s) {
+int launch(const UpfParams& p, bool vec, hipStream_t s, int64_t* plan = nullptr) {
     static const bool fir_old = getenv("SG2_FIR_OLD") != nullptr;
-    if (!fir_old && vec && p.upx == 1 && p.upy == 1 && p.downx == 1 && p.downy == 1 && p.fw == 4 && p.fh == 4 &&
+    constexpr bool AGT = sizeof(T) == 2;
+    const bool ag = p.ag_dc != nullptr;
+    if ((!fir_old || ag) && !(ag && p.epi) && vec && p.upx == 1 && p.upy == 1 && p.downx == 1 && p.downy == 1 && p.fw == 4 && p.fh == 4 &&
         p.OH >= 8 && (p.OW % 32 == 0 || p.OW >= 224) && !(p.residual && p.residual == p.y)) {
         constexpr int TW = 32, TH = 8;
         const char* e32 = getenv("SG2_FIR_C32");
@@ -661,6 +839,16 @@
             const int64_t blocks4 = (int64_t)p.N * cdiv(p.OH, TH) * cdiv(p.OW, TW4);
             if (blocks4 < INT32_MAX) {
                 const size_t lds = (size_t)(TH + 3) * (TW4 + 3) * CG4 * 16;
+                if (plan) { *plan = blocks4; return 0; }
+                if constexpr (AGT) {
+                    if (ag) {
+                        auto ka = upfirdn_nhwc_f4s<T, TW4, TH, CG4, true>;
+                        static bool seta4 = false;
+                        if (!seta4) { (void)hipFuncSetAttribute((const void*)ka, hipFuncAttributeMaxDynamicSharedMemorySize, (int)lds); seta4 = true; }
+                        ka<<<(unsigned)blocks4, 256, lds, s>>>(p);
+                        return launch_status("sg2_upfirdn2d_actgrad");
+                    }
+                }
                 auto k = upfirdn_nhwc_f4s<T, TW4, TH, CG4>;
                 static bool set4 = false;
                 if (!set4) { (void)hipFuncSetAttribute((const void*)k, hipFuncAttributeMaxDynamicSharedMemorySize, (int)lds); set4 = true; }
@@ -671,6 +859,16 @@
         const int64_t blocks = (int64_t)p.N * cdiv(p.OH, TH) * cdiv(p.OW, TW) * cdiv(p.C / VecN<T>::N, 8);
         if (blocks < INT32_MAX) {
             const size_t lds = (size_t)(TH + 3) * (TW + 3) * 8 * 16;
+            if (plan) { *plan = (int64_t)p.N * cdiv(p.OH, TH) * cdiv(p.OW, TW); return 0; }
+            if constexpr (AGT) {
+                if (ag) {
+                    auto ka = upfirdn_nhwc_f4s<T, TW, TH, 8, true>;
+                    static bool seta = false;
+                    if (!seta) { (void)hipFuncSetAttribute((const void*)ka, hipFuncAttributeMaxDynamicSharedMemorySize, (int)lds); seta = true; }
+                    ka<<<(unsigned)blocks, 256, lds, s>>>(p);
+                    return launch_status("sg2_upfirdn2d_actgrad");
+                }
+            }
             auto k = upfirdn_nhwc_f4s<T, TW, TH>;
             static bool set = false;
             if (!set) { (void)hipFuncSetAttribute((const void*)k, hipFuncAttributeMaxDynamicSharedMemorySize, (int)lds); set = true; }
@@ -678,7 +876,7 @@
             return launch_status("sg2_upfirdn2d");
         }
     }
-    if (vec && p.upx == 1 && p.upy == 1 && p.downx == p.downy && (p.downy == 1 || p.downy == 2) && p.fw == 4 &&
+    if (!ag && vec && p.upx == 1 && p.upy == 1 && p.downx == p.downy && (p.downy == 1 || p.downy == 2) && p.fw == 4 &&
         p.fh == 4) {
         constexpr int CG = 4;
         const int d = p.downy;
@@ -704,6 +902,13 @@
         !getenv("SG2_UPF_UP2_OFF")) {
         const int64_t cells = (int64_t)p.N * ((p.OH + 1) / 2) * ((p.OW + 1) / 2) * (p.C / VecN<T>::N);
         if (cells < INT32_MAX - 256) {
+            if (plan) { *plan = cdiv(cells, 256); return 0; }
+            if constexpr (AGT) {
+                if (ag) {
+                    upfirdn_nhwc_up2<T, true><<<(unsigned)cdiv(cells, 256), 256, 0, s>>>(p);
+                    return launch_status("sg2_upfirdn2d_actgrad");
+                }
+            }
             upfirdn_nhwc_up2<T><<<(unsigned)cdiv(cells, 256), 256, 0, s>>>(p);
             return launch_status("sg2_upfirdn2d");
         }
@@ -744,6 +949,12 @@
     }
     const int64_t work = vec ? (int64_t)p.N * p.OH * p.OW * (p.C / VecN<T>::N) : (int64_t)p.N * p.C * p.OH * p.OW;
     const int grid = (int)std::max<int64_t>(1, std::min<int64_t>(cdiv(work, 256), 256 * 32));
+    if (ag) {
+        SG2_CHECK(vec && work < INT32_MAX, "sg2_upfirdn2d_actgrad: tensor too large");
+        if (plan) { *plan = grid; return 0; }
+        if constexpr (AGT) upfirdn_nhwc_vec<T, unsigned, true><<<grid, 256, 0, s>>>(p);
+        return launch_status("sg2_upfirdn2d_actgrad");
+    }
     if (vec && work < INT32_MAX && (int64_t)grid * 256 < INT32_MAX)
         upfirdn_nhwc_vec<T, unsigned><<<grid, 256, 0, s>>>(p);
     else if (vec)
@@ -782,6 +993,8 @@
     { const char* e = getenv("SG2_FIR_XCD"); p.xcd = e ? atoi(e) : 1; }
     p.out_scale = nullptr; p.noise = nullptr; p.bias = nullptr; p.residual = nullptr; p.aux = nullptr;
     p.noise_gain = 0.f; p.alpha = 0.f; p.egain = 1.f; p.clamp = -1.f; p.act = 0; p.aux_mode = 0; p.epi = 0;
+    p.ag_ys = nullptr; p.ag_dc = nullptr; p.ag_db = nullptr; p.ag_gain = 1.f; p.ag_alpha = 0.f; p.ag_clamp = -1.f;
+    p.ag_act = 0; p.ag_store_v = 0;
     if (epi) {
         SG2_CHECK(epi->act == 0 || epi->act == 1, "sg2_upfirdn2d: epilogue act must be 0 or 1");
         SG2_CHECK(epi->aux_mode >= 0 && epi->aux_mode <= 2 && (epi->aux_mode == 0 || epi->aux),
@@ -837,3 +1050,79 @@
     return sg2_upfirdn2d_fused(y, x, f, dtype, in_size, in_stride, out_size, out_stride, fw, fh, upx, upy, downx,
                                downy, padx0, padx1, pady0, pady1, flip, gain, nullptr, stream);
 }
+
+extern "C" int sg2_upfirdn2d_actgrad(void* dc, float* db, void* v, const void* x, const void* ys, const void* residual,
+                                     const float* f, int dtype, const int64_t* in_size, const int64_t* in_stride,
+                                     const int64_t* out_size, int fw, int fh, int upx, int upy, int downx, int downy,
+                                     int padx0, int padx1, int pady0, int pady1, int flip, float fgain, int act,
+                                     float alpha, float gain, float clamp, void* stream) {
+    using namespace sg2;
+    SG2_CHECK(dc && x && ys && f && in_size && in_stride && out_size, "sg2_upfirdn2d_actgrad: null argument");
+    SG2_CHECK(dtype == SG2_F16 || dtype == SG2_BF16, "sg2_upfirdn2d_actgrad: f16/bf16 only");
+    SG2_CHECK(act == 0 || act == 1, "sg2_upfirdn2d_actgrad: act must be linear or lrelu");
+    SG2_CHECK(upx >= 1 && upy >= 1 && downx >= 1 && downy >= 1, "sg2_upfirdn2d_actgrad: up/down must be >= 1");
+    SG2_CHECK(fw >= 1 && fh >= 1 && fw * fh <= kMaxTaps, "sg2_upfirdn2d_actgrad: filter too large");
+    SG2_CHECK(!residual || v, "sg2_upfirdn2d_actgrad: a residual needs the v output");
+    SG2_CHECK(!db || det_on(), "sg2_upfirdn2d_actgrad: db needs the deterministic mode's scratch (sg2_set_deterministic)");
+    UpfParams p{};
+    p.x = x; p.y = v; p.f = f;
+    p.N = (int)in_size[0]; p.C = (int)in_size[1]; p.H = (int)in_size[2]; p.W = (int)in_size[3];
+    p.OH = (int)out_size[2]; p.OW = (int)out_size[3];
+    SG2_CHECK(out_size[0] == p.N && out_size[1] == p.C, "sg2_upfirdn2d_actgrad: batch/channel mismatch");
+    SG2_CHECK(p.C % 8 == 0 && p.C >= 8 && 256 % (p.C / 8) == 0,
+              "sg2_upfirdn2d_actgrad: C / 8 must divide 256");
+    const int64_t eh = ((int64_t)p.H * upy + pady0 + pady1 - fh + downy) / downy;
+    const int64_t ew = ((int64_t)p.W * upx + padx0 + padx1 - fw + downx) / downx;
+    SG2_CHECK(p.H * upy + pady0 + pady1 >= fh && p.W * upx + padx0 + padx1 >= fw,
+              "sg2_upfirdn2d_actgrad: upsampled buffer must be at least the size of the filter");
+    SG2_CHECK(eh == p.OH && ew == p.OW, "sg2_upfirdn2d_actgrad: output size mismatch");
+    p.xs_n = in_stride[0]; p.xs_c = in_stride[1]; p.xs_h = in_stride[2]; p.xs_w = in_stride[3];
+    p.ys_c = 1; p.ys_w = p.C; p.ys_h = (int64_t)p.OW * p.C; p.ys_n = (int64_t)p.OH * p.OW * p.C;
+    p.fw = fw; p.fh = fh; p.upx = upx; p.upy = upy; p.downx = downx; p.downy = downy;
+    p.padx0 = padx0; p.pady0 = pady0; p.flip = flip; p.gain = fgain; p.xcd = 1;
+    p.egain = 1.f; p.clamp = -1.f; p.alpha = 0.2f;
+    p.residual = residual; p.epi = residual ? 1 : 0;
+    p.ag_ys = ys; p.ag_dc = dc; p.ag_gain = gain; p.ag_alpha = alpha; p.ag_clamp = clamp; p.ag_act = act;
+    p.ag_store_v = v ? 1 : 0;
+    if ((int64_t)p.N * p.C * p.OH * p.OW == 0) return 0;
+    const bool vec = p.xs_c == 1 && p.xs_w % 8 == 0 && p.xs_h % 8 == 0 && p.xs_n % 8 == 0 &&
+                     ((uintptr_t)x | (uintptr_t)ys | (uintptr_t)dc | (uintptr_t)v | (uintptr_t)residual) % 16 == 0;
+    SG2_CHECK(vec, "sg2_upfirdn2d_actgrad: needs 16-byte aligned NHWC tensors");
+    hipStream_t s = as_stream(stream);
+    int64_t slots = 0;
+    DetArena arena;
+    const int64_t hw = (int64_t)p.OH * p.OW;
+    if (db && residual && upx == 2 && upy == 2 && downx == 1 && downy == 1 && fw == 4 && fh == 4 &&
+        !getenv("SG2_UPF_UP2_OFF") && hw * p.C < INT32_MAX && p.N <= 65535) {
+        hipError_t e = zero_acc(db, p.C * sizeof(float), s);
+        if (e) { set_error("sg2_upfirdn2d_actgrad: memset failed"); return e; }
+        const int PPP = 256 / (p.C / 8);
+        const int ppb = (int)std::min<int64_t>(hw, PPP * 16);
+        dim3 grid((unsigned)cdiv(hw, ppb), (unsigned)p.N);
+        slots = (int64_t)grid.x * p.N;
+        SG2_DET_GET(p.ag_db, arena, slots * p.C, "sg2_upfirdn2d_actgrad");
+        const size_t lds = (size_t)PPP * p.C * sizeof(float);
+        if (dtype == SG2_F16) upfirdn_up2_lbo<f16_t><<<grid, 256, lds, s>>>(p, ppb);
+        else upfirdn_up2_lbo<bf16_t><<<grid, 256, lds, s>>>(p, ppb);
+        int rc = launch_status("sg2_upfirdn2d_actgrad");
+        if (rc) return rc;
+        DetSumJob job{db, 0, p.ag_db, 0, p.C, 1, slots, p.C, det_assign()};
+        e = det_sum_multi(&job, 1, arena, s);
+        if (e) { set_error("sg2_upfirdn2d_actgrad: det_sum"); return e; }
+        return 0;
+    }
+    if (db) {
+        hipError_t e = zero_acc(db, p.C * sizeof(float), s);
+        if (e) { set_error("sg2_upfirdn2d_actgrad: memset failed"); return e; }
+        int rc = -1;
+        if (dtype == SG2_F16) rc = launch<f16_t>(p, true, s, &slots);
+        else rc = launch<bf16_t>(p, true, s, &slots);
+        if (rc) return rc;
+        SG2_DET_GET(p.ag_db, arena, slots * p.C, "sg2_upfirdn2d_actgrad");
+    }
+    int rc = dtype == SG2_F16 ? launch<f16_t>(p, true, s) : launch<bf16_t>(p, true, s);
+    if (rc || !db) return rc;
+    hipError_t err = det_sum(db, 0, p.ag_db, 0, p.C, 1, slots, p.C, arena, s, det_assign());
+    if (err) { set_error("sg2_upfirdn2d_actgrad: det_sum"); return err; }
+    return 0;
+}
diff --git a/gan-track_amd/sg2hip/__init__.py b/gan-track_amd/sg2hip/__init__.py
--- a/gan-track_amd/sg2hip/__init__.py
+++ b/gan-track_amd/sg2hip/__init__.py
@@ -56,6 +56,8 @@
                           _i, _f, _vp, _vp],
     'sg2_upfirdn2d_fused': [_vp, _vp, _vp, _i, _c_i64p, _c_i64p, _c_i64p, _c_i64p, _i, _i, _i, _i, _i, _i, _i, _i, _i,
                             _i, _i, _f, ctypes.POINTER(Epilogue), _vp],
+    'sg2_upfirdn2d_actgrad': [_vp, _vp, _vp, _vp, _vp, _vp, _vp, _i, _c_i64p, _c_i64p, _c_i64p, _i, _i, _i, _i, _i, _i, _i,
+                              _i, _i, _i, _i, _f, _i, _f, _f, _f, _vp],
     'sg2_layer_bwd': [_vp, _vp, _vp, _vp, _vp, _vp, _vp, _vp, _i, _i, _i, _i, _i, _f, _f, _f, _vp],
     'sg2_dot_hw': [_vp, _vp, _vp, _i, _i, _i, _i, _vp],
     'sg2_vjp_axpy': [_vp, _vp, _vp, _vp, _vp, _vp, _i, _f, _f, _f, _vp, _vp, _i, _i, _i, _i, _vp],
diff --git a/gan-track_amd/torch_utils/ops/modconv.py b/gan-track_amd/torch_utils/ops/modconv.py
--- a/gan-track_amd/torch_utils/ops/modconv.py
+++ b/gan-track_amd/torch_utils/ops/modconv.py
@@ -135,6 +135,89 @@
 
 def fused_conv_tap(x, weight, styles, bias, padding, clamp):
     return FusedConvTap.apply(x, styles, weight, bias, int(padding), float(clamp if clamp is not None else -1.0))
+
+
+def _wants_db(ctx, need):
+    return bool(need[5]) and ctx.saved_tensors[5] is not None
+
+
+def _actgrad_backward(ctx, need, g, ys, f, fir, residual=None):
+    x, _, weight, _, _, bias, _, _ = ctx.saved_tensors
+    stride, pad, act, alpha, gain, clamp, _, wgain = ctx.cfg
+    aup, adown, p, aflip = fir
+    want_db = need[5] and bias is not None
+    dc, db, v = _up.fir_actgrad(g, f, ys, up=aup, down=adown, padding=p, flip_filter=aflip, act=act, alpha=alpha,
+                                gain=gain, clamp=clamp, residual=residual, want_db=want_db)
+    dx, _, dw = _scaled_input_grads(dc, _cg._nhwc(x), None, weight, need[0], False, need[2], stride, pad, wgain)
+    return dx, dw, (db.to(bias.dtype) if db is not None else None), v
+
+
+class FusedConvFIR(torch.autograd.Function):
+
+    @staticmethod
+    def forward(ctx, x, weight, bias, f, fpad, pad, act, alpha, gain, clamp, wgain):
+        y = FusedConv.forward(ctx, x, None, weight, None, None, bias, None, 1, pad, act, alpha, gain, clamp, wgain)
+        ctx.fir = (f, fpad, y.shape)
+        return _up._raw(y, f, 1, 1, 1, 1, fpad[0], fpad[1], fpad[2], fpad[3], False, 1.0)
+
+    @staticmethod
+    def backward(ctx, dt):
+        n = ctx.needs_input_grad
+        need = (n[0], False, n[1], False, False, n[2], False)
+        f, fpad, ys = ctx.fir
+        y = ctx.saved_tensors[6]
+        fir = _up.adjoint_params(f, (ys[2], ys[3]), (dt.shape[2], dt.shape[3]), [1, 1], [1, 1], list(fpad), False)
+        if not torch.is_grad_enabled() and fast_backward and _up.fir_actgrad_ok(y, _wants_db(ctx, need)):
+            dx, dw, db, _ = _actgrad_backward(ctx, need, dt, y, f, fir)
+        else:
+            dy = _up._upfirdn2d_fn(up=fir[0], down=fir[1], padding=fir[2], flip_filter=fir[3]).apply(dt, f)
+            dx, _, dw, _, _, db = _fused_conv_grads(ctx, need, dy)
+        return (dx, dw, db) + (None,) * 8
+
+
+def fused_conv_fir(x, weight, bias, f, fir_padding, padding, act, alpha, gain, clamp, wgain):
+    f = f.to(device=x.device, dtype=torch.float32).contiguous()
+    return FusedConvFIR.apply(x, weight, bias, f, tuple(int(v) for v in fir_padding), int(padding),
+                              1 if act == 'lrelu' else 0, float(alpha), float(gain),
+                              float(clamp if clamp is not None else -1.0), float(wgain))
+
+
+class FusedConvFork(torch.autograd.Function):
+
+    @staticmethod
+    def forward(ctx, x, weight, bias, residual, f, down, fpad, stride, pad, act, alpha, gain, clamp, wgain):
+        y = FusedConv.forward(ctx, x, None, weight, None, None, bias, residual, stride, pad, act, alpha, gain, clamp,
+                              wgain)
+        ctx.fir = (f, down, fpad)
+        yd = _up._raw(y, f, 1, 1, down, down, fpad[0], fpad[1], fpad[2], fpad[3], False, 1.0)
+        return y, yd
+
+    @staticmethod
+    def backward(ctx, g_y, g_yd):
+        n = ctx.needs_input_grad
+        need = (n[0], False, n[1], False, False, n[2], False)
+        f, down, fpad = ctx.fir
+        y, aux = ctx.saved_tensors[6], ctx.saved_tensors[7]
+        zsrc = aux if ctx.cfg[6] else y
+        if g_yd is None:
+            dy = g_y
+        elif g_y is not None and not torch.is_grad_enabled() and fast_backward and \
+                _up.fir_actgrad_ok(zsrc, _wants_db(ctx, need), fork=(f, down)):
+            fir = _up.adjoint_params(f, (y.shape[2], y.shape[3]), (g_yd.shape[2], g_yd.shape[3]), [1, 1],
+                                     [down, down], list(fpad), False)
+            dx, dw, db, dy = _actgrad_backward(ctx, need, g_yd, zsrc, f, fir, residual=g_y)
+            return (dx, dw, db, dy if n[3] else None) + (None,) * 10
+        else:
+            dy = _up.fork_adjoint(g_y, g_yd, f, down, fpad, y.shape)
+        dx, _, dw, _, _, db = _fused_conv_grads(ctx, need, dy)
+        return (dx, dw, db, dy if n[3] else None) + (None,) * 10
+
+
+def fused_conv_fork(x, weight, bias, residual, f, down, fir_padding, stride, padding, act, alpha, gain, clamp, wgain):
+    f = f.to(device=x.device, dtype=torch.float32).contiguous()
+    return FusedConvFork.apply(x, weight, bias, residual, f, int(down), tuple(int(v) for v in fir_padding),
+                               int(stride), int(padding), 1 if act == 'lrelu' else 0, float(alpha), float(gain),
+                               float(clamp if clamp is not None else -1.0), float(wgain))
 
 
 def _scaled_input_grads(dc, x, styles, weight, need_x, need_s, need_w, stride, pad, wgain=1.0, acc_ds=None,
diff --git a/gan-track_amd/torch_utils/ops/upfirdn2d.py b/gan-track_amd/torch_utils/ops/upfirdn2d.py
--- a/gan-track_amd/torch_utils/ops/upfirdn2d.py
+++ b/gan-track_amd/torch_utils/ops/upfirdn2d.py
@@ -1,4 +1,5 @@
 import ctypes
+import os
 
 import numpy as np
 import torch
@@ -151,23 +152,60 @@
         down, padding, xs = ctx.cfg
         if gy is None:
             return gx, None, None, None
-        aup, adown, p, aflip = adjoint_params(f, (xs[2], xs[3]), (gy.shape[2], gy.shape[3]), [1, 1], [down, down],
-                                              list(padding), False)
-        if torch.is_grad_enabled() or gx is None:
-            dx = _upfirdn2d_fn(up=aup, down=adown, padding=p, flip_filter=aflip).apply(gy, f)
-            return (dx + gx if gx is not None else dx), None, None, None
-        cl = torch.channels_last
-        gy = gy.contiguous(memory_format=cl)
-        gx = gx.to(gy.dtype).contiguous(memory_format=cl)
-        dx = torch.empty_like(gx)
-        epi = _hip.Epilogue(None, None, None, _hip.ptr(gx), None, 1.0, 0.2, 1.0, -1.0, 0, 0)
-        fh, fw = f.shape
-        _hip.check(_hip.lib().sg2_upfirdn2d_fused(
-            _hip.ptr(dx), _hip.ptr(gy), _hip.ptr(f), _hip.dtype_code(gy), _hip.i64arr(gy.shape),
-            _hip.i64arr(gy.stride()), _hip.i64arr(dx.shape), _hip.i64arr(dx.stride()), fw, fh, aup[0], aup[1],
-            adown[0], adown[1], p[0], p[1], p[2], p[3], int(bool(aflip)), 1.0, ctypes.byref(epi),
-            _hip.stream_ptr(gy.device)), 'sg2_upfirdn2d_fused')
-        return dx, None, None, None
+        return fork_adjoint(gx, gy, f, down, padding, xs), None, None, None
+
+
+def fork_adjoint(gx, gy, f, down, padding, xs):
+    aup, adown, p, aflip = adjoint_params(f, (xs[2], xs[3]), (gy.shape[2], gy.shape[3]), [1, 1], [down, down],
+                                          list(padding), False)
+    if torch.is_grad_enabled() or gx is None:
+        dx = _upfirdn2d_fn(up=aup, down=adown, padding=p, flip_filter=aflip).apply(gy, f)
+        return dx + gx if gx is not None else dx
+    cl = torch.channels_last
+    gy = gy.contiguous(memory_format=cl)
+    gx = gx.to(gy.dtype).contiguous(memory_format=cl)
+    dx = torch.empty_like(gx)
+    epi = _hip.Epilogue(None, None, None, _hip.ptr(gx), None, 1.0, 0.2, 1.0, -1.0, 0, 0)
+    fh, fw = f.shape
+    _hip.check(_hip.lib().sg2_upfirdn2d_fused(
+        _hip.ptr(dx), _hip.ptr(gy), _hip.ptr(f), _hip.dtype_code(gy), _hip.i64arr(gy.shape),
+        _hip.i64arr(gy.stride()), _hip.i64arr(dx.shape), _hip.i64arr(dx.stride()), fw, fh, aup[0], aup[1],
+        adown[0], adown[1], p[0], p[1], p[2], p[3], int(bool(aflip)), 1.0, ctypes.byref(epi),
+        _hip.stream_ptr(gy.device)), 'sg2_upfirdn2d_fused')
+    return dx
+
+
+def fir_actgrad_ok(ys, want_db=False, fork=None):
+    c = ys.shape[1]
+    mode = os.environ.get('SG2_FIR_ACTGRAD', '1')
+    db_exact = (fork is not None and tuple(fork[0].shape) == (4, 4) and fork[1] == 2 and
+                not os.environ.get('SG2_UPF_UP2_OFF'))
+    return (mode != '0' and (mode == '2' or not want_db or db_exact) and _hip.det_active() and ys.is_cuda and ys.ndim == 4 and
+            ys.dtype in (torch.float16, torch.bfloat16) and c % 8 == 0 and 256 % (c // 8) == 0 and
+            ys.is_contiguous(memory_format=torch.channels_last) and ys.data_ptr() % 16 == 0)
+
+
+def fir_actgrad(x, f2, ys, up=1, down=1, padding=0, flip_filter=False, act=1, alpha=0.2, gain=1.0, clamp=-1.0,
+                residual=None, want_v=False, want_db=True):
+    upx, upy = _parse_scaling(up)
+    downx, downy = _parse_scaling(down)
+    px0, px1, py0, py1 = _parse_padding(padding)
+    cl = torch.channels_last
+    x = x.to(ys.dtype).contiguous(memory_format=cl)
+    fh, fw = f2.shape
+    assert tuple(ys.shape) == (x.shape[0], x.shape[1], (x.shape[2] * upy + py0 + py1 - fh + downy) // downy,
+                               (x.shape[3] * upx + px0 + px1 - fw + downx) // downx)
+    dc = torch.empty_like(ys)
+    if residual is not None:
+        residual = residual.to(ys.dtype).contiguous(memory_format=cl)
+    v = torch.empty_like(ys) if (want_v or residual is not None) else None
+    db = torch.empty([ys.shape[1]], dtype=torch.float32, device=ys.device) if want_db else None
+    _hip.check(_hip.lib().sg2_upfirdn2d_actgrad(
+        _hip.ptr(dc), _hip.ptr(db), _hip.ptr(v), _hip.ptr(x), _hip.ptr(ys), _hip.ptr(residual), _hip.ptr(f2),
+        _hip.dtype_code(ys), _hip.i64arr(x.shape), _hip.i64arr(x.stride()), _hip.i64arr(ys.shape), fw, fh, upx, upy,
+        downx, downy, px0, px1, py0, py1, int(bool(flip_filter)), 1.0, int(act), float(alpha), float(gain),
+        float(clamp), _hip.stream_ptr(ys.device)), 'sg2_upfirdn2d_actgrad')
+    return dc, db, v
 
 
 def fork_fir(x, f, down, padding):
diff --git a/gan-track_amd/training/networks_stylegan2.py b/gan-track_amd/training/networks_stylegan2.py
--- a/gan-track_amd/training/networks_stylegan2.py
+++ b/gan-track_amd/training/networks_stylegan2.py
@@ -314,10 +314,14 @@
             else:
                 self.bias = None
 
-    def forward(self, x, gain=1, residual=None, prefiltered=False):
+    def fused_ok(self, x):
+        return self.activation in ('lrelu', 'linear') and self.up == 1 and modconv.supported_generic(x, self.weight)
+
+    def forward(self, x, gain=1, residual=None, prefiltered=False, fir_next=None, fork=None):
         clamp = self.conv_clamp * gain if self.conv_clamp is not None else None
         kh = self.weight.shape[2]
-        if self.activation in ('lrelu', 'linear') and self.up == 1 and modconv.supported_generic(x, self.weight):
+        assert (fir_next is None and fork is None and (not prefiltered or kh == 1)) or self.fused_ok(x)
+        if self.fused_ok(x):
             stride, pad = 1, self.padding
             if self.down > 1:
                 x0, x1, y0, y1 = conv2d_resample._frame_padding(self.padding, self.resample_filter, 1, self.down)
@@ -325,9 +329,19 @@
                     if not prefiltered:
                         x = upfirdn2d.upfirdn2d(x, self.resample_filter, down=self.down, padding=[x0, x1, y0, y1])
                 else:
-                    x = upfirdn2d.upfirdn2d(x, self.resample_filter, padding=[x0, x1, y0, y1])
+                    if not prefiltered:
+                        x = upfirdn2d.upfirdn2d(x, self.resample_filter, padding=[x0, x1, y0, y1])
                     stride = self.down
                 pad = 0
+            alpha = bias_act.activation_funcs[self.activation].def_alpha or 0.2
+            if fir_next is not None:
+                assert residual is None and fork is None and stride == 1
+                return modconv.fused_conv_fir(x, self.weight, self.bias, fir_next[0], fir_next[1], pad, self.activation,
+                                              alpha, self.act_gain * gain, clamp, self.weight_gain)
+            if fork is not None:
+                return modconv.fused_conv_fork(x, self.weight, self.bias, residual, fork[0], fork[1], fork[2], stride,
+                                               pad, self.activation, alpha, self.act_gain * gain, clamp,
+                                               self.weight_gain)
             return modconv.fused_conv(x, self.weight, bias=self.bias, residual=residual, stride=stride, padding=pad,
                                       act=self.activation, alpha=bias_act.activation_funcs[self.activation].def_alpha or 0.2,
                                       gain=self.act_gain * gain, clamp=clamp, wgain=self.weight_gain)
@@ -676,32 +690,64 @@
             self.skip = Conv2dLayer(tmp_channels, out_channels, kernel_size=1, bias=False, down=2,
                                     trainable=next_trainable(), resample_filter=resample_filter)
 
-    def forward(self, x, img, force_fp32=False):
+    def skip_fork(self, x):
+        if self.architecture != 'resnet':
+            return None
+        sk = self.skip
+        if not (sk.down > 1 and sk.weight.shape[2] == 1 and upfirdn2d.fork_fir_ok(x, sk.resample_filter)):
+            return None
+        return sk.resample_filter, sk.down, conv2d_resample._frame_padding(sk.padding, sk.resample_filter, 1, sk.down)
+
+    def forward(self, x, img, force_fp32=False, xd=None, fork_next=None):
         dtype = self.fp16_dtype if self.use_fp16 and not force_fp32 else torch.float32
+        x_in = x
         if x is not None:
             misc.assert_shape(x, [None, self.in_channels, self.resolution, self.resolution])
             x = x.to(dtype=dtype, memory_format=_CL)
         if self.in_channels == 0 or self.architecture == 'skip':
             misc.assert_shape(img, [None, self.img_channels, self.resolution, self.resolution])
             img = img.to(dtype=dtype, memory_format=_CL)
-            y = self.fromrgb(img)
-            x = x + y if x is not None else y
+            own = self.skip_fork(torch.empty([0, self.fromrgb.out_channels, 1, 1], dtype=dtype, device=img.device,
+                                             memory_format=_CL)) if x is None and dtype != torch.float32 else None
+            if own is not None and self.fromrgb.fused_ok(img):
+                x, xd = self.fromrgb(img, fork=own)
+            else:
+                y = self.fromrgb(img)
+                x = x + y if x is not None else y
             img = upfirdn2d.downsample2d(img, self.resample_filter) if self.architecture == 'skip' else None
+        if xd is not None and (x is not x_in and x_in is not None):
+            xd = None
+        c0, c1 = self.conv0, self.conv1
+        fir1 = None
+        if (c1.down > 1 and c1.weight.shape[2] == 3 and c0.down == 1 and c0.weight.shape[2] == 3 and
+                dtype != torch.float32 and upfirdn2d.fork_fir_ok(x, c1.resample_filter) and c0.fused_ok(x) and
+                c0.out_channels % 8 == 0):
+            fir1 = (c1.resample_filter, conv2d_resample._frame_padding(c1.padding, c1.resample_filter, 1, c1.down))
+        fk = None
+        if isinstance(fork_next, DiscriminatorBlock) and fork_next.in_channels == c1.out_channels and \
+                (fork_next.fp16_dtype if fork_next.use_fp16 and not force_fp32 else torch.float32) == dtype and \
+                dtype != torch.float32 and c1.fused_ok(x):
+            fk = fork_next.skip_fork(torch.empty([0, c1.out_channels, 1, 1], dtype=dtype, device=x.device,
+                                                 memory_format=_CL))
         if self.architecture == 'resnet':
             sk = self.skip
-            if sk.down > 1 and sk.weight.shape[2] == 1 and upfirdn2d.fork_fir_ok(x, sk.resample_filter):
-                pad = conv2d_resample._frame_padding(sk.padding, sk.resample_filter, 1, sk.down)
-                x, xd = upfirdn2d.fork_fir(x, sk.resample_filter, sk.down, pad)
+            fx = self.skip_fork(x)
+            if fx is not None:
+                if xd is None:
+                    x, xd = upfirdn2d.fork_fir(x, fx[0], fx[1], fx[2])
                 y = sk(xd, gain=np.sqrt(0.5), prefiltered=True)
             else:
                 y = self.skip(x, gain=np.sqrt(0.5))
-            x = self.conv0(x)
-            x = self.conv1(x, gain=np.sqrt(0.5), residual=y)
+            x = c0(x, fir_next=fir1)
+            x = c1(x, gain=np.sqrt(0.5), residual=y, prefiltered=fir1 is not None, fork=fk)
         else:
-            x = self.conv0(x)
-            x = self.conv1(x)
+            x = c0(x, fir_next=fir1)
+            x = c1(x, prefiltered=fir1 is not None, fork=fk)
+        xd_next = None
+        if fk is not None:
+            x, xd_next = x
         assert x.dtype == dtype
-        return x, img
+        return (x, img, xd_next) if fork_next is not None else (x, img)
 
     def extra_repr(self):
         return f'resolution={self.resolution:d}, architecture={self.architecture:s}'
@@ -807,9 +853,10 @@
         self.b4 = DiscriminatorEpilogue(channels[4], cmap_dim=cmap_dim, resolution=4, **epilogue_kwargs, **common)
 
     def forward(self, img, c, update_emas=False, **block_kwargs):
-        x = None
-        for r in self.block_resolutions:
-            x, img = getattr(self, f'b{r}')(x, img, **block_kwargs)
+        x = xd = None
+        blocks = [getattr(self, f'b{r}') for r in self.block_resolutions]
+        for blk, nxt in zip(blocks, blocks[1:] + [self.b4]):
+            x, img, xd = blk(x, img, xd=xd, fork_next=nxt, **block_kwargs)
         cmap = self.mapping(None, c) if self.c_dim > 0 else None
         return self.b4(x, img, cmap)
 
diff --git a/include/sg2hip.h b/include/sg2hip.h
--- a/include/sg2hip.h
+++ b/include/sg2hip.h
@@ -36,6 +36,12 @@
                         const int64_t* in_stride, const int64_t* out_size, const int64_t* out_stride, int fw, int fh,
                         int upx, int upy, int downx, int downy, int padx0, int padx1, int pady0, int pady1, int flip,
                         float gain, const sg2_epilogue* epi, void* stream);
+
+int sg2_upfirdn2d_actgrad(void* dc, float* db, void* v, const void* x, const void* ys, const void* residual,
+                          const float* f, int dtype, const int64_t* in_size, const int64_t* in_stride,
+                          const int64_t* out_size, int fw, int fh, int upx, int upy, int downx, int downy, int padx0,
+                          int padx1, int pady0, int pady1, int flip, float fgain, int act, float alpha, float gain,
+                          float clamp, void* stream);
 
 int sg2_conv2d(void* y, const void* x, const void* w, int dtype, int N, int Cin, int H, int W, int Cout,
                int OH, int OW, int KH, int KW, int stride, int pad_y, int pad_x, int transpose,
```

Result: no change. 793.3 imgs/s (median of 6 runs) (+0.6%).
